# BaratiLab/GAMD

Hardware: AMD Instinct MI355X
Metric: atom-steps/sec (force eval + integrate), 10k-atom LJ box (higher is better)
Workload: dtype f32; 1 GPU; C2: 10 000-atom LJ box, rho*=0.5, L=92.29 A, cutoff 3.0 sigma=10.2 A, fp32, 4 conv layers x 128, random-init weights (seed 0), 1 box per GPU; n_atoms=10000, boxes=1, launch=single process

## Files before the change

gamd_amd/csrc/gamd_api.hip:

```cpp
#include "gamd_host.h"

#include <algorithm>
#include <cmath>
#include <cstddef>
#include <cstdlib>
#include <cstring>
#include <deque>

static_assert(sizeof(gamd_config) == 96 && offsetof(gamd_config, n_boxes) == 88 && offsetof(gamd_config, edge_capacity) == 40,
              "gamd_config layout is part of the C ABI (gamd_amd/_lib.py mirrors it)");

namespace {

bool small_path(const gamd_handle* h) { return h->use_small; }

int fill_com(gamd_handle* h, int enabled, MdCom* c) {
    c->enabled = enabled ? 1 : 0;
    c->blocks = std::max(1, std::min(16, (h->n_per_box + 1023) / 1024));
    c->partial = nullptr;
    if (!c->enabled) return 0;
    if (h->com_partial.ensure(sizeof(double) * 4 * (size_t)c->blocks * (size_t)h->n_boxes, true)) return fail(-12, "allocation failed");
    c->partial = h->com_partial.as<double>();
    return 0;
}
// ... 127 lines not shown
        a.cand_stride = (int)std::max<long long>(1, std::min<long long>(h->cand_cap / h->n, 1 << 20));
    }
    return a;
}

void pack128(const float* W, float* out, int ld = 128) {
    for (int tp = 0; tp < 4; ++tp)
        for (int t = 0; t < 4; ++t)
            for (int q = 0; q < 4; ++q)
                for (int lane = 0; lane < 64; ++lane)
                    for (int j = 0; j < 4; ++j) {
                        const int n = 32 * tp + (lane & 31), k = 32 * t + 8 * q + 4 * (lane >> 5) + j;
                        out[((((tp * 4 + t) * 4 + q) * 64 + lane) * 4) + j] = W[(size_t)n * ld + k];
                    }
}
void pack16(const float* W, float* out, int ld = 128) {
    for (int ob = 0; ob < 8; ++ob)
        for (int blk = 0; blk < 8; ++blk)
            for (int lane = 0; lane < 64; ++lane)
                for (int r = 0; r < 4; ++r)
                    out[(((ob * 8 + blk) * 64 + lane) * 4) + r] = W[(size_t)(16 * ob + (lane & 15)) * ld + 16 * blk + 4 * (lane >> 4) + r];
}
void split_f16(float w, uint16_t* hi, uint16_t* lo);
void pack16_f16x3(const float* W, uint16_t* out) {
    for (int ob = 0; ob < 8; ++ob)
        for (int m = 0; m < 4; ++m)
            for (int lane = 0; lane < 64; ++lane)
                for (int j = 0; j < 8; ++j) {
                    const int k = 32 * m + 16 * (j >> 2) + 4 * (lane >> 4) + (j & 3);
                    const size_t hi = ((((size_t)(ob * 4 + m) * 2 + 0) * 64 + lane) * 8) + j, lo = ((((size_t)(ob * 4 + m) * 2 + 1) * 64 + lane) * 8) + j;
                    split_f16(W[(size_t)(16 * ob + (lane & 15)) * 128 + k], out + hi, out + lo);
                }
}
void pack_enc1(const float* W, int n_feat, float* out) {
    for (int tp = 0; tp < 4; ++tp)
        for (int g = 0; g < 6; ++g)
            for (int lane = 0; lane < 64; ++lane)
                for (int j = 0; j < 4; ++j) {
                    const int n = 32 * tp + (lane & 31), k = 2 * (4 * g + j) + (lane >> 5);
                    out[(((tp * 6 + g) * 64 + lane) * 4) + j] = k < n_feat ? W[n * n_feat + k] : 0.f;
                }
}

int kfeat16x(int m, int g) { return 32 * (m >> 3) + 8 * ((m >> 1) & 3) + 4 * (g & 1) + (g >> 1) + 2 * (m & 1); }
void pack16x(const float* W, float* out, int ld, bool chained) {
    for (int ob = 0; ob < 8; ++ob)
        for (int m4 = 0; m4 < 8; ++m4)
            for (int lane = 0; lane < 64; ++lane) {
                const int i = lane & 15, g = lane >> 4;
                const int row = chained ? kfeat16x(4 * ob + (i & 3), i >> 2) : 64 * (ob >> 2) + 4 * i + (ob & 3);
                for (int c = 0; c < 4; ++c)
                    out[(((size_t)ob * 8 + m4) * 64 + lane) * 4 + c] = W[(size_t)row * ld + kfeat16x(4 * m4 + c, g)];
            }
}

uint16_t f2bf(float x) {
    uint32_t u; memcpy(&u, &x, 4);
    if ((u & 0x7f800000u) == 0x7f800000u) return (uint16_t)(u >> 16);
    u += 0x7fffu + ((u >> 16) & 1u);
    return (uint16_t)(u >> 16);
}
void pack128_bf16(const float* W, uint16_t* out, int ld = 128) {
    for (int tp = 0; tp < 4; ++tp)
        for (int t = 0; t < 4; ++t)
            for (int u = 0; u < 2; ++u)
                for (int lane = 0; lane < 64; ++lane)
                    for (int j = 0; j < 8; ++j) {
                        const int r = 8 * u + j, half = lane >> 5;
                        const int n = 32 * tp + (lane & 31), k = 32 * t + (r & 3) + 8 * (r >> 2) + 4 * half;
                        out[((((tp * 4 + t) * 2 + u) * 64 + lane) * 8) + j] = f2bf(W[(size_t)n * ld + k]);
                    }
}
void pack_enc1_bf16(const float* W, int n_feat, uint16_t* out) {
    for (int tp = 0; tp < 4; ++tp)
        for (int s = 0; s < 3; ++s)
            for (int lane = 0; lane < 64; ++lane)
                for (int j = 0; j < 8; ++j) {
                    const int n = 32 * tp + (lane & 31), k = 16 * s + 8 * (lane >> 5) + j;
                    out[(((tp * 3 + s) * 64 + lane) * 8) + j] = k < n_feat ? f2bf(W[n * n_feat + k]) : (uint16_t)0;
                }
}

void split_f16(float w, uint16_t* hi, uint16_t* lo) {
    const _Float16 h = (_Float16)w;
    const _Float16 l = (_Float16)(w - (float)h);
    memcpy(hi, &h, 2); memcpy(lo, &l, 2);
}
void pack128_f16x3(const float* W, uint16_t* out, int ld = 128) {
    for (int tp = 0; tp < 4; ++tp)
        for (int t = 0; t < 4; ++t)
            for (int u = 0; u < 2; ++u)
                for (int lane = 0; lane < 64; ++lane)
                    for (int j = 0; j < 8; ++j) {
                        const int r = 8 * u + j, half = lane >> 5;
                        const int n = 32 * tp + (lane & 31), k = 32 * t + (r & 3) + 8 * (r >> 2) + 4 * half;
                        const size_t at = ((((tp * 4 + t) * 2 + u) * 64 + lane) * 8) + j;
                        split_f16(W[(size_t)n * ld + k], out + at, out + 16384 + at);
                    }
}
void pack_enc1_f16x3(const float* W, int n_feat, uint16_t* out) {
    for (int tp = 0; tp < 4; ++tp)
        for (int s = 0; s < 3; ++s)
            for (int lane = 0; lane < 64; ++lane)
                for (int j = 0; j < 8; ++j) {
                    const int n = 32 * tp + (lane & 31), k = 16 * s + 8 * (lane >> 5) + j;
                    const size_t at = (((tp * 3 + s) * 64 + lane) * 8) + j;
                    split_f16(k < n_feat ? W[n * n_feat + k] : 0.f, out + at, out + 6144 + at);
                }
}

struct BlobBuilder {
    std::vector<float> host;
    size_t add(size_t n_floats) {
        const size_t off = host.size();
        host.resize(off + ((n_floats + 63) & ~(size_t)63), 0.f);
        return off;
    }
};

const HostTensor* find_w(gamd_handle* h, const std::string& name, std::initializer_list<int64_t> shape) {
    auto it = h->host_w.find(name);
    if (it == h->host_w.end()) { fail(-2, "missing weight '%s'", name.c_str()); return nullptr; }
    if (it->second.shape != std::vector<int64_t>(shape)) {
        std::string got;
        for (auto d : it->second.shape) got += std::to_string(d) + ",";
        std::string want;
        for (auto d : shape) want += std::to_string(d) + ",";
        fail(-22, "weight '%s' has shape (%s), expected (%s) for this configuration", name.c_str(), got.c_str(),
             want.c_str());
        return nullptr;
    }
    return &it->second;
}

struct EdgeList { const int* centre; const int* neigh; long long n; };

int fill_rigid(const gamd_handle* h, int rigid_water, float mass_o, float mass_h, float r_oh, float r_hh,
               int* use_rigid, RigidWater* g) {
    *use_rigid = 0;
    if (!rigid_water) return 0;
    if (h->n_per_box % 3 != 0) return fail(-22, "rigid_water needs O,H,H triples: n_atoms = %d is not a multiple of 3", h->n_per_box);
    if (!(mass_h > 0.f) || !(mass_o > 0.f)) return fail(-22, "rigid_water needs mass_amu (O) and mass_h_amu (H)");
    if (!(r_oh > 0.f) || !(r_hh > 0.f) || !(r_hh < 2.f * r_oh)) return fail(-22, "rigid_water needs 0 < r_hh < 2 r_oh");
    const double rc = 0.5 * (double)r_hh, t = std::sqrt((double)r_oh * r_oh - rc * rc);
    const double ra = t * 2.0 * mass_h / ((double)mass_o + 2.0 * mass_h);
    g->m_o = mass_o; g->m_h = mass_h;
    g->rc = (float)rc; g->ra = (float)ra; g->rb = (float)(t - ra);
    *use_rigid = 1;
    return 0;
}

int enqueue_forward(gamd_handle* h, const float* pos_dev, const uint8_t* species_dev, float* out_norm_dev,
                    float* out_denorm_dev, hipStream_t st, hipEvent_t* evs, int* n_ev, std::vector<std::string>* labels,
                    const EdgeList* el = nullptr, const MdFuse* fuse = nullptr, bool copy_counters = true, bool l0_reuse = false) {
    auto mark = [&](const char* label) {
        if (evs) { (void)hipEventRecord(evs[*n_ev], st); ++*n_ev; labels->push_back(label); }
    };
    int r;
    mark("begin");
    const bool pingpong = !el && h->skin > 0.f;
    int* counters_next = nullptr;
    if (pingpong) {
        h->cnt_parity ^= 1;
        h->cur_counters = h->cnt2.as<int>() + h->cnt_parity * CNT_COUNT;
        counters_next = h->cnt2.as<int>() + (1 - h->cnt_parity) * CNT_COUNT;
    } else {
        h->cur_counters = h->counters.as<int>();
    }
    NbrArgs na = nbr_args(h, pos_dev, species_dev);
    na.counters_next = counters_next;
    if (el) {
        if ((r = launch_csr_from_edges(na, el->centre, el->neigh, el->n, h->tmp_eid.as<int>(), st)))
            return fail(-1, "edge-list CSR launch failed (%d)", r);
        h->cand_valid = false;
    } else if (h->skin > 0.f) {
        na.ref_pos = h->ref_pos.as<float4>();
        na.force_rebuild = h->cand_valid ? 0 : 1;
        ++h->skin_calls;
        na.cells_one_wg = (h->skin_calls < 32 || 6ll * h->sticky_host[STICKY_REBUILDS] < h->skin_calls) ? 1 : 0;
        if (fuse && !pingpong) return fail(-1, "internal: integrator halves can only be fused into the skin path");
        if ((r = launch_neighbor_skin(na, st, fuse))) return fail(-1, "neighbor (skin) launch failed (%d)", r);
        h->cand_valid = true;
    } else if ((r = launch_neighbor_build(na, st))) return fail(-1, "neighbor build launch failed (%d)", r);
    mark("neighbor_build");

    EncArgs ea{};
    ea.counters = h->cur_counters;
    ea.devflags = h->devflags.as<int>();
    ea.pos_s = h->pos_s.as<float4>();
    ea.col = h->col.as<int>();
    ea.erow = h->erow.as<int>();
    ea.bond_nbr = h->has_bonds ? h->bond_nbr.as<int>() : nullptr;
    ea.perm = h->perm.as<int>();
    ea.row_ptr = h->row_ptr.as<int>();
    ea.self_loop = na.self_loop;
    ea.zero_row = h->n;
    for (int d = 0; d < 3; ++d) { ea.box[d] = h->box[d]; ea.half[d] = 0.5f * h->box[d]; }
    ea.bx = box_ref(h);
    ea.length_mean = h->length_mean;
    ea.length_std = h->length_std;
    ea.gamma = (float)(1.0 / 0.025);
    ea.ln_inv_width = 1.0f / (float)h->Eh_true;
    ea.ln_n_pad = (float)(h->Eh - h->Eh_true);
    ea.n_feat = h->n_feat;
    ea.n_ksteps = (h->n_feat + 1) / 2;
    ea.centers = h->centers;
    ea.rbf = h->rbf;
    ea.w1p = h->enc_w1p; ea.w2p = h->enc_w2p; ea.w3p = h->enc_w3p;
    ea.b1 = h->enc_b1; ea.b2 = h->enc_b2; ea.b3 = h->enc_b3;
    ea.ln_g = h->enc_lng; ea.ln_b = h->enc_lnb;
    ea.e_format = !h->wide_enc ? 0 : h->cfg.edge_dtype == GAMD_EDGE_F16X3 ? 2 : h->cfg.edge_dtype == GAMD_EDGE_BF16 ? 1 : 0;
    ea.e_frag = h->e_frag.as<float>();
    ea.e_cap = h->e_cap;
    ea.sticky = h->sticky_dev;
    ea.feat_dbg = h->cfg.keep_stages ? h->feat_dbg.as<float>() : nullptr;
    int small_tiles = 0;
    if (h->cfg.edge_dtype == GAMD_EDGE_F32) {
        const long long e_est = el ? el->n + (na.self_loop ? h->n : 0)
                                   : (h->counters_host[CNT_E] > 0 ? (long long)h->counters_host[CNT_E] : (long long)((double)h->e_cap / 1.5));
        const long long tiles = (e_est + GAMD_TILE - 1) / GAMD_TILE;
        if (tiles <= h->small_tile_limit) small_tiles = (int)std::max<long long>(1, std::min<long long>(tiles + tiles / 8 + 1, 4096));
    }
    const bool half_quantum = h->wide_conv && h->cfg.edge_dtype == GAMD_EDGE_F32 && (h->cfg.kernel_select & GAMD_KSEL_FORCE_HALF_QUANTUM) != 0;
    bool tev_full = false;
    auto tev_begin = [&](int kind) -> int {
        if (!h->timing) return 0;
        if (h->tev_used + 2 > h->tev.size()) {
            if (h->tev.size() >= 8 * gamd_handle::EVENT_POOL_CAP) { tev_full = true; return 0; }
            for (int k = 0; k < 256; ++k) { hipEvent_t e; HIP_TRY(hipEventCreate(&e)); h->tev.push_back(e); h->tev_kind.push_back(0); }
        }
        h->tev_kind[h->tev_used] = kind;
        HIP_TRY(hipEventRecord(h->tev[h->tev_used], st));
        return 0;
    };
    auto tev_end = [&]() -> int {
        if (!h->timing || tev_full) return 0;
        HIP_TRY(hipEventRecord(h->tev[h->tev_used + 1], st));
        h->tev_used += 2;
        return 0;
    };
    if ((r = tev_begin(100))) return r;
    r = h->DT > 1 ? launch_edge_encode_wide_d(ea, h->EHT, h->DT, h->n_cu, st)
        : h->wide_enc ? launch_edge_encode_wide(ea, h->EHT, h->n_cu, st)
        : h->cfg.edge_dtype == GAMD_EDGE_BF16 ? launch_edge_encode_bf16(ea, h->n_cu, st)
        : h->cfg.edge_dtype == GAMD_EDGE_F16X3 ? launch_edge_encode_f16x3(ea, h->n_cu, st)
        : small_tiles > 0 ? launch_edge_encode_small(ea, small_tiles, st) : launch_edge_encode(ea, h->n_cu, st);
    if (r) return fail(-1, "edge encode launch failed (%d)", r);
    if ((r = tev_end())) return r;
    mark("edge_encode");

    const size_t nh = (size_t)h->n * (size_t)h->H;
    auto node = [&](const NodeArgs& na_) {
        return h->DT > 1 ? launch_node_wide_d(na_, h->HT, h->DT, st) : h->wide_conv ? launch_node_wide(na_, h->HT, st) : launch_node(na_, st);
    };
    auto hptr = [&](int l) { return h->hbuf.as<float>() + (h->cfg.keep_stages ? (size_t)l * nh : (size_t)(l & 1) * nh); };

    NodeArgs no{};
#ifdef GAMD_PROFILING
    { static const bool node_time = getenv("GAMD_NODE_TIME") != nullptr; if (node_time) no.tdbg = h->tdbg.as<long long>(); }
#endif
    no.counters = h->cur_counters;
    no.devflags = h->devflags.as<int>();
    no.sticky = h->sticky_dev;
    no.n = h->n;
    no.pos_s = h->pos_s.as<float4>();
    no.node_emb = h->node_emb; no.enc_w = h->nenc_w; no.enc_b = h->nenc_b;
    no.row_ptr = h->row_ptr.as<int>(); no.na_excl = h->na_excl.as<int>(); no.deg = h->deg.as<int>();
    no.col = (h->l0_hoist && h->n_boxes > 1) ? h->col.as<int>() : nullptr;
    no.partial = h->partial.as<float>();
    no.piece_cap = h->piece_cap;
    no.P_in = h->P.as<float>();
    no.hn_perm = (!h->wide_conv && h->cfg.edge_dtype == GAMD_EDGE_F16X3) ? 1 : 0;
    no.tab16 = (!h->wide_conv && h->cfg.edge_dtype == GAMD_EDGE_BF16) ? 1 : 0;
    no.hn_out = h->hn.as<float>(); no.S_out = h->S.as<float>(); no.D_out = h->D.as<float>(); no.P_out = h->P.as<float>();
    no.dec_w1p = h->dec_w1p; no.dec_b1 = h->dec_b1; no.dec_w2 = h->dec_w2; no.dec_b2 = h->dec_b2;
    no.ln_inv_width = 1.0f / (float)h->H_true;
    no.ln_n_pad = (float)(h->H - h->H_true);
    no.norm_bn = h->norm_bn;
    no.f16x3 = h->node_f16 ? 1 : 0;
    no.scale = (float)std::sqrt(h->scaler_var);
    no.shift = (float)h->scaler_mean;
    no.perm = h->perm.as<int>();
    no.forces_norm = out_norm_dev ? out_norm_dev : h->f_norm.as<float>();
    no.forces = out_denorm_dev;

    const bool l0 = h->skin > 0.f && !el;
    float* const h0 = (l0 && !h->cfg.keep_stages) ? h->l0_h.as<float>() : hptr(0);
    no.mode = 0;
    no.pre = h->layers[0].node;
    no.h_out = h0;
    if (l0) { no.hn_out = h->l0_hn.as<float>(); no.S_out = h->l0_S.as<float>(); no.D_out = h->l0_D.as<float>(); no.P_out = h->l0_P.as<float>(); }
    no.l0_gate = (l0 && l0_reuse) ? 1 : 0;
    if ((r = node(no))) return fail(-1, "node(0) launch failed (%d)", r);
    no.l0_gate = 0;
    no.hn_out = h->hn.as<float>(); no.S_out = h->S.as<float>(); no.D_out = h->D.as<float>(); no.P_out = h->P.as<float>();
    mark("node_first");


    for (int l = 0; l < h->L; ++l) {
        ConvEdgeArgs ca{};
        ca.counters = h->cur_counters;
        ca.devflags = h->devflags.as<int>();
        ca.col = h->col.as<int>(); ca.erow = h->erow.as<int>();
        ca.chunk_piece = h->chunk_piece.as<int>(); ca.chunk_mask = h->chunk_mask.as<unsigned>();
        ca.e_frag = (h->update_edge && l > 0) ? h->e_frag2.as<float>() : h->e_frag.as<float>();
        ca.emb_out = (h->update_edge && l + 1 < h->L) ? h->e_emb.as<float>() : nullptr;
        ca.hn = h->hn.as<float>(); ca.S = h->S.as<float>(); ca.D = h->D.as<float>();
        if (l0 && l == 0) { ca.hn = h->l0_hn.as<float>(); ca.S = h->l0_S.as<float>(); ca.D = h->l0_D.as<float>(); }
        const LayerDev& ld = h->layers[l];
        ca.w1p = ld.w1p; ca.w2p = ld.w2p; ca.w3p = ld.w3p; ca.w4p = ld.w4p; ca.w16p = ld.w16p;
        ca.b1 = ld.b1; ca.b3 = ld.b3; ca.b4 = ld.b4;
        const bool hoist = l == 0 && h->l0_hoist;
        if (hoist) { ca.w3p = ld.w3p_l0; ca.b3 = ld.b3_l0; }
        ca.partial = h->partial.as<float>();
        ca.piece_cap = h->piece_cap;
        ca.sticky = h->sticky_dev;
        ca.e_cap = h->e_cap;
        ca.zero_row = h->n;
#ifdef GAMD_CHECKED
        { static const bool inject = getenv("GAMD_CHK_INJECT") != nullptr; if (inject) ca.zero_row = 0; }
#endif
        ca.tdbg = h->tdbg.as<long long>();
        if ((r = tev_begin(l))) return r;
        r = h->DT > 1 ? launch_conv_edge_wide_d(ca, h->EHT, h->HT, h->DT, h->n_cu, st)
            : h->wide_conv ? (h->cfg.edge_dtype == GAMD_EDGE_F16X3 ? launch_conv_edge_f16x3_wide(ca, h->EHT, h->HT, h->n_cu, st)
                            : h->cfg.edge_dtype == GAMD_EDGE_BF16 ? launch_conv_edge_bf16_wide(ca, h->EHT, h->HT, h->n_cu, st)
                            : (half_quantum && ca.w16p && !ca.emb_out) ? launch_conv_edge_wide16(ca, h->EHT, h->HT, h->n_cu, st)
                            : small_tiles > 0 ? launch_conv_edge_small_wide(ca, h->EHT, h->HT, small_tiles, st)
                                              : launch_conv_edge_wide(ca, h->EHT, h->HT, h->n_cu, st))
            : h->cfg.edge_dtype == GAMD_EDGE_BF16 ? launch_conv_edge_bf16(ca, h->n_cu, st)
            : h->cfg.edge_dtype == GAMD_EDGE_F16X3 ? launch_conv_edge_f16x3(ca, h->n_cu, st)
            : hoist ? (small_tiles > 0 ? launch_conv_edge_small_l0(ca, small_tiles, st) : launch_conv_edge_l0(ca, h->n_cu, st))
            : small_tiles > 0 ? launch_conv_edge_small(ca, small_tiles, st) : launch_conv_edge(ca, h->n_cu, st);
        if (r) return fail(-1, "conv edge launch failed (%d)", r);
        if ((r = tev_end())) return r;
        mark("conv_edge");
        if (ca.emb_out) {
            EdgeUpdateArgs ua{};
            ua.counters = h->cur_counters; ua.devflags = h->devflags.as<int>(); ua.e_cap = h->e_cap;
            ua.emb = ca.emb_out; ua.ln_g = ld.e_ln_g; ua.ln_b = ld.e_ln_b;
            ua.ln_inv_width = 1.0f / (float)h->Eh_true;
            ua.ln_n_pad = (float)(h->Eh - h->Eh_true);
            ua.e_frag_out = h->e_frag2.as<float>();
            if ((r = launch_edge_update(ua, h->HT, small_tiles > 0 ? std::max(1, small_tiles / 4) : 2 * h->n_cu, st)))
                return fail(-1, "edge update launch failed (%d)", r);
            mark("edge_update");
        }

        no.mode = (l == h->L - 1) ? 2 : 1;
        no.post = ld.node;
        if (l + 1 < h->L) no.pre = h->layers[l + 1].node;
        no.h_in = l == 0 ? h0 : hptr(l);
        no.P_in = (l0 && l == 0) ? h->l0_P.as<float>() : h->P.as<float>();
        no.h_out = hptr(l + 1);
        if ((r = node(no))) return fail(-1, "node launch failed (%d)", r);
        mark(no.mode == 2 ? "node_last_decode" : "node_mid");
    }
    if (copy_counters)
        HIP_TRY(hipMemcpyAsync(h->counters_host, h->cur_counters, sizeof(int) * CNT_COUNT, hipMemcpyDeviceToHost, st));
    return 0;
}

int check_ready(gamd_handle* h) {
    if (!h) return fail(-22, "null handle");
    if (!h->finalized) return fail(-22, "weights not finalized (call gamd_finalize_weights)");
    return 0;
}

int check_model_inputs(gamd_handle* h, const uint8_t* species_dev) {
    if (h->cfg.kind == GAMD_KIND_WATER && !species_dev && !h->feat_dev)
        return fail(-22, "water model needs species (or gamd_set_node_features)");
    if (h->cfg.use_bond && !h->has_bonds) return fail(-22, "use_bond set but no bonds given (gamd_set_bonds)");
    return 0;
}

int check_rigid_layout(gamd_handle* h, const uint8_t* species_dev, hipStream_t st) {
    if (!species_dev) return fail(-22, "rigid_water needs species (O = 1, H = 0, atoms ordered O,H,H)");
    if (h->rigid_checked == species_dev) return 0;
    std::vector<uint8_t> sp((size_t)h->n);
    HIP_TRY(hipMemcpyAsync(sp.data(), species_dev, sp.size(), hipMemcpyDeviceToHost, st));
    HIP_TRY(hipStreamSynchronize(st));
    for (int i = 0; i < h->n; ++i)
        if ((sp[(size_t)i] != 0) != (i % 3 == 0))
            return fail(-22, "rigid_water needs atoms ordered O,H,H per molecule: species[%d] = %d", i, (int)sp[(size_t)i]);
    h->rigid_checked = species_dev;
    return 0;
}

int clear_devflags(gamd_handle* h) {
    const int init[2] = {0, -1};
    HIP_TRY(init_upload(h->devflags.p, init, sizeof(init)));
    return 0;
}

int step_event(gamd_handle* h, hipStream_t st, bool closes = false) {
    if (!h->timing) return 0;
    if (h->sev_used == h->sev.size()) {
        if (h->sev.size() >= gamd_handle::EVENT_POOL_CAP) return 0;
        for (int k = 0; k < 256; ++k) { hipEvent_t e; HIP_TRY(hipEventCreate(&e)); h->sev.push_back(e); h->sev_closes.push_back(0); }
    }
    h->sev_closes[h->sev_used] = closes ? 1 : 0;
    HIP_TRY(hipEventRecord(h->sev[h->sev_used++], st));
    return 0;
}

int enqueue_md_steps(gamd_handle* h, long long s_begin, bool skip_first) {
    MdPending& p = h->pending;
    int r;
    if (p.kind == 0 && h->skin > 0.f) {
        for (long long s = s_begin; s < p.n_steps; ++s) {
            if ((r = step_event(h, p.st))) return r;
            p.m.step = p.first_step + (unsigned long long)s;
            p.m.step_index = (int)s;
            int do_second = (s > s_begin && !observers_sampled(h, s - 1)) ? 1 : 0;
            const int do_first = (skip_first && s == s_begin) ? 0 : 1;
            if (p.m.com.enabled) {
                if (do_second && do_first) {
                    MdArgs prev = p.m;
                    prev.step_index = (int)(s - 1);
                    if ((r = launch_baoab_second_com(prev, p.st))) return fail(-1, "integrator launch failed (%d)", r);
                    do_second = 0;
                } else {
                    if (do_second) {
                        MdArgs prev = p.m;
                        prev.step_index = (int)(s - 1);
                        if ((r = launch_baoab_second(prev, p.st))) return fail(-1, "integrator launch failed (%d)", r);
                        do_second = 0;
                    }
                    if (do_first && (r = launch_com_partial(p.m.com, p.m.v, p.m.species, p.m.inv_mass, p.m.inv_mass_h, p.m.n, p.m.bx,
                                                            p.m.devflags, p.m.use_rigid, p.st)))
                        return fail(-1, "integrator launch failed (%d)", r);
                }
            }
            const MdFuse fuse{&p.m, do_second, do_first};
            if ((r = enqueue_forward(h, p.x, p.species, nullptr, p.f, p.st, nullptr, nullptr, nullptr, nullptr, &fuse,
                                     s + 1 == p.n_steps, s > s_begin)))
                return r;
            if (s + 1 < p.n_steps && observers_sampled(h, s)) {
                if ((r = launch_baoab_second(p.m, p.st))) return fail(-1, "integrator launch failed (%d)", r);
                if ((r = observers_enqueue(h, s))) return r;
            }
        }
        if (p.n_steps > s_begin) {
            p.m.step_index = (int)(p.n_steps - 1);
            if ((r = launch_baoab_second(p.m, p.st))) return fail(-1, "integrator launch failed (%d)", r);
            if ((r = observers_enqueue(h, p.n_steps - 1))) return r;
        }
        return step_event(h, p.st, true);
    }
    for (long long s = s_begin; s < p.n_steps; ++s) {
        if ((r = step_event(h, p.st))) return r;
        const bool first = !(skip_first && s == s_begin);
        const bool last = s + 1 == p.n_steps;
        if (p.kind == 0) {
            p.m.step = p.first_step + (unsigned long long)s;
            p.m.step_index = (int)s;
            if (first && (r = launch_baoab_first(p.m, p.st))) return fail(-1, "integrator launch failed (%d)", r);
            if ((r = enqueue_forward(h, p.x, p.species, nullptr, p.f, p.st, nullptr, nullptr, nullptr, nullptr, nullptr, last, s > s_begin))) return r;
            if ((r = launch_baoab_second(p.m, p.st))) return fail(-1, "integrator launch failed (%d)", r);
        } else {
            p.a.step_index = (int)s;
            if (first && (r = launch_nhc_first(p.a, p.st))) return fail(-1, "integrator launch failed (%d)", r);
            if ((r = enqueue_forward(h, p.x, p.species, nullptr, p.f, p.st, nullptr, nullptr, nullptr, nullptr, nullptr, last, s > s_begin))) return r;
            if ((r = launch_nhc_second(p.a, p.st))) return fail(-1, "integrator launch failed (%d)", r);
        }
        if ((r = observers_enqueue(h, s))) return r;
    }
    return step_event(h, p.st, true);
}

template <typename Params, typename Args>
int fill_run_args(gamd_handle* h, const Params* p, const float* box, const uint8_t* species_dev, hipStream_t st, Args* a) {
    int r;
    a->n = h->n; a->species = species_dev; a->dt = p->dt_ps;
    a->len = p->length_per_nm > 0.f ? p->length_per_nm : 10.0f;
    if ((r = fill_rigid(h, p->rigid_water, p->mass_amu, p->mass_h_amu, p->r_oh, p->r_hh, &a->use_rigid, &a->rigid))) return r;
    if (a->use_rigid && (r = check_rigid_layout(h, species_dev, st))) return r;
    for (int d = 0; d < 3; ++d) a->box[d] = box[d];
    a->bx = box_ref(h);
    if ((r = fill_com(h, p->remove_cm_motion, &a->com))) return r;
    a->devflags = h->devflags.as<int>();
    return 0;
}

int start_run(gamd_handle* h, float* x_dev, float* f_dev, const uint8_t* species_dev, const float* box, long long n_steps, hipStream_t st) {
    MdPending& pd = h->pending;
    pd.active = true; pd.n_steps = n_steps;
    pd.x = x_dev; pd.f = f_dev; pd.species = species_dev; pd.st = st;
    observers_begin_run(h, box, species_dev, n_steps);
    return enqueue_md_steps(h, 0, false);
}

}

extern "C" {

#ifdef GAMD_CHECKED
const char* gamd_version(void) { return "gamd_hip 0.1 (gfx950) checked"; }
#else
const char* gamd_version(void) { return "gamd_hip 0.1 (gfx950)"; }
#endif
const char* gamd_last_error(void) { return g_err; }

int32_t gamd_create(const gamd_config* cfg, gamd_handle** out) {
    if (!cfg || !out) return fail(-22, "null argument");
    if (cfg->n_atoms <= 0) return fail(-22, "n_atoms must be positive");
    if (cfg->n_boxes < 0 || cfg->n_boxes > (1 << 20)) return fail(-22, "n_boxes out of range");
    const int n_boxes = cfg->n_boxes > 1 ? cfg->n_boxes : 1;
    if ((long long)cfg->n_atoms * n_boxes >= (1 << 23) - 1)
        return fail(-22, "n_atoms x n_boxes = %lld: at most %d atoms per handle", (long long)cfg->n_atoms * n_boxes, (1 << 23) - 2);
    if (cfg->n_layers <= 0 || cfg->n_layers > 16) return fail(-22, "n_layers out of range");
    if (!(cfg->cutoff > 0.f)) return fail(-22, "cutoff must be positive");
    if (cfg->edge_dtype != GAMD_EDGE_F32 && cfg->edge_dtype != GAMD_EDGE_BF16 && cfg->edge_dtype != GAMD_EDGE_F16X3)
        return fail(-22, "unknown edge_dtype");
    if (!(cfg->neighbor_skin >= 0.f)) return fail(-22, "neighbor_skin must be >= 0");
    if (cfg->self_loop_mode != GAMD_SELF_LOOP_DGL07_NOOP && cfg->self_loop_mode != GAMD_SELF_LOOP_APPEND_ZERO_FEATURE)
        return fail(-22, "unknown self_loop_mode %d", cfg->self_loop_mode);
    if (cfg->self_loop_mode != GAMD_SELF_LOOP_DGL07_NOOP && cfg->edge_dtype != GAMD_EDGE_F32)
        return fail(-22, "self_loop_mode 1 is built for the fp32 edge dtype only");
    if (cfg->kernel_select & ~(GAMD_KSEL_FORCE_GENERIC_WIDTH | GAMD_KSEL_FORCE_HALF_QUANTUM | GAMD_KSEL_NO_LAYER0_HOIST))
        return fail(-22, "unknown kernel_select bits 0x%x", cfg->kernel_select);
    int ndev = 0;
    if (hipGetDeviceCount(&ndev) != hipSuccess || ndev <= 0)
        return fail(-19, "no HIP device available: libgamd_hip has no CPU fallback");
    if (cfg->device < 0 || cfg->device >= ndev) return fail(-22, "device %d out of range (%d visible)", cfg->device, ndev);
    DeviceGuard guard(cfg->device);
    hipDeviceProp_t prop;
    HIP_TRY(hipGetDeviceProperties(&prop, cfg->device));
    const int H_true = cfg->encoding_size ? cfg->encoding_size : 128, Eh_true = cfg->edge_embedding_dim ? cfg->edge_embedding_dim : 128;
    const int D_true = cfg->hidden_dim ? cfg->hidden_dim : 128;
    if (H_true < 1 || H_true > 256 || Eh_true < 1 || Eh_true > 256)
        return fail(-22, "encoding_size and edge_embedding_dim must be in [1, 256] (got %d, %d)", H_true, Eh_true);
    if (D_true < 1 || D_true > 256) return fail(-22, "hidden_dim must be in [1, 256] (got %d)", D_true);
    const int Dp = D_true <= 128 ? 128 : 256;
    if (Dp > 128 && cfg->edge_dtype != GAMD_EDGE_F32)
        return fail(-22, "hidden_dim above 128 is built for edge_dtype f32 only (got hidden_dim %d)", D_true);
    const int H = H_true <= 128 ? 128 : 256, Eh = Eh_true <= 128 ? 128 : 256;
    const bool exact128 = H_true == 128 && Eh_true == 128 && D_true == 128;
    const bool generic = H != 128 || Eh != 128 || cfg->no_expand_edge;
    if (cfg->edge_dtype != GAMD_EDGE_F32 && H == 256 && (long long)cfg->n_atoms * n_boxes > (1ll << 22) - 2)
        return fail(-22, "bf16 / split-fp16 with encoding_size > 128: at most 2^22 - 2 atoms per handle (32-bit byte offsets into hn)");
    gamd_handle* h = new gamd_handle();
    h->obs = observers_new();
    h->cfg = *cfg;
    h->dev = cfg->device;
    if (hipStreamCreateWithFlags(&h->init_stream, hipStreamNonBlocking) != hipSuccess) {
        h->init_stream = nullptr;
        gamd_destroy(h);
        return fail(-12, "stream creation failed");
    }
    InitStream init(h->init_stream);
    h->n_boxes = n_boxes;
    h->n_per_box = cfg->n_atoms;
    h->n = cfg->n_atoms * n_boxes;
    h->L = cfg->n_layers;
    h->H = H; h->Eh = Eh; h->HT = H / 128; h->EHT = Eh / 128;
    h->H_true = H_true; h->Eh_true = Eh_true; h->D_true = D_true;
    h->Dp = Dp; h->DT = Dp / 128;
    h->skin = cfg->neighbor_skin;
    if (cfg->small_tile_limit != 0) h->small_tile_limit = cfg->small_tile_limit < 0 ? -1 : cfg->small_tile_limit;
    const bool forced = (cfg->kernel_select & GAMD_KSEL_FORCE_GENERIC_WIDTH) && cfg->edge_dtype == GAMD_EDGE_F32;
    const bool lp_generic = cfg->edge_dtype != GAMD_EDGE_F32 && (generic || !exact128);
    h->wide_enc = generic || forced || lp_generic || Dp > 128;
    h->wide_conv = H != 128 || Eh != 128 || forced || lp_generic || Dp > 128;
    h->n_feat = (cfg->no_expand_edge ? 4 : 44) + (cfg->use_bond ? 1 : 0);
    h->n_cu = prop.multiProcessorCount > 0 ? prop.multiProcessorCount : 256;
    const size_t n = (size_t)h->n;
    int r = 0;
    r |= h->pos_w.ensure(sizeof(float4) * n, true);
    r |= h->pos_s.ensure(sizeof(float4) * (n + 1), true);
    r |= h->cell_of.ensure(sizeof(int) * n, true);
    r |= h->perm.ensure(sizeof(int) * (n + 1), true);
    if (n_boxes > 1) {
        r |= h->boxes_dev.ensure(sizeof(float) * 12 * (size_t)n_boxes, true);
        r |= h->box_shift.ensure(sizeof(int) * ((size_t)n_boxes + 2), true);
    }
    r |= h->inv_perm.ensure(sizeof(int) * n, true);
    r |= h->deg.ensure(sizeof(int) * n, true);
    r |= h->row_ptr.ensure(sizeof(int) * (n + 1), true);
    r |= h->na_excl.ensure(sizeof(int) * (n + 1), true);
    const size_t nh = n * (size_t)H * sizeof(float), nd = n * (size_t)Dp * sizeof(float), zd = (size_t)Dp * sizeof(float);
    r |= h->hbuf.ensure(nh * (cfg->keep_stages ? (size_t)h->L + 1 : 2), true);
    r |= h->hn.ensure(nh + (size_t)H * sizeof(float), true);
    r |= h->S.ensure(nd + zd, true);
    r |= h->D.ensure(nd + zd, true);
    r |= h->P.ensure(nd, true);
    if (cfg->neighbor_skin > 0.f) {
        r |= h->l0_hn.ensure(nh + (size_t)H * sizeof(float), true);
        r |= h->l0_S.ensure(nd + zd, true);
        r |= h->l0_D.ensure(nd + zd, true);
        r |= h->l0_P.ensure(nd, true);
        if (!cfg->keep_stages) r |= h->l0_h.ensure(nh, true);
    }
    r |= h->f_norm.ensure(sizeof(float) * 3 * n, true);
    r |= h->f_den.ensure(sizeof(float) * 3 * n, true);
    r |= h->tdbg.ensure(sizeof(long long) * 16 * 8 * 1024, true);
    r |= h->devflags.ensure(sizeof(int) * DEVFLAG_COUNT, true);
    r |= h->cnt2.ensure(sizeof(int) * 2 * CNT_COUNT, true);
    if (r) { gamd_destroy(h); return fail(-12, "device allocation failed"); }
    {
        const int no_atom = -2;
        if (init_upload(h->perm.as<int>() + n, &no_atom, sizeof(int)) != hipSuccess) {
            gamd_destroy(h);
            return fail(-1, "device copy failed");
        }
    }
    if ((r = clear_devflags(h))) { gamd_destroy(h); return r; }
    if (hipHostMalloc((void**)&h->counters_host, sizeof(int) * CNT_COUNT) != hipSuccess) {
        gamd_destroy(h);
        return fail(-12, "pinned allocation failed");
    }
    memset(h->counters_host, 0, sizeof(int) * CNT_COUNT);
    if (hipHostMalloc((void**)&h->sticky_host, sizeof(int) * STICKY_COUNT, hipHostMallocMapped) != hipSuccess ||
        hipHostGetDevicePointer((void**)&h->sticky_dev, h->sticky_host, 0) != hipSuccess) {
        gamd_destroy(h);
        return fail(-12, "mapped host allocation failed");
    }
    memset(h->sticky_host, 0, sizeof(int) * STICKY_COUNT);
    if (h->skin > 0.f) {
        int rr = 0;
        rr |= h->ref_pos.ensure(sizeof(float4) * n, true);
        rr |= h->cand_deg.ensure(sizeof(int) * n, true);
        rr |= h->cand_ptr.ensure(sizeof(int) * (n + 1), true);
        if (rr) { gamd_destroy(h); return fail(-12, "device allocation failed"); }
    }
    {
        std::vector<float> all((size_t)n_boxes * 3);
        for (int b = 0; b < n_boxes; ++b)
            for (int d = 0; d < 3; ++d) all[(size_t)3 * b + d] = cfg->box[d];
        if ((r = set_box(h, all.data()))) { gamd_destroy(h); return r; }
    }
    {
        const double per_atom = std::min<double>(h->n, 27.0 * h->n / std::max(1, h->ncell));
        h->use_small = h->n <= 1024 && n_boxes <= 1 && (double)h->n * per_atom <= 3.0e5 && h->ncell <= 4096;
    }
    long long ecap = cfg->edge_capacity;
    if (ecap <= 0) {
        const double vol = (double)cfg->box[0] * cfg->box[1] * cfg->box[2];
        const double per_atom = 4.18879 * std::pow((double)cfg->cutoff, 3) * (double)h->n_per_box / vol + 1.0;
        ecap = (long long)(1.5 * per_atom * (double)h->n) + 1024 + 16ll * n_boxes;
    }
    if (cfg->self_loop_mode) ecap += h->n;
    if ((r = alloc_edges(h, ecap))) { gamd_destroy(h); return r; }
    if (hipStreamSynchronize(h->init_stream) != hipSuccess) { gamd_destroy(h); return fail(-1, "device synchronisation failed"); }
    *out = h;
    return 0;
}

int32_t gamd_destroy(gamd_handle* h) {
    if (!h) return 0;
    DeviceGuard guard(h->dev);
    InitStream init(h->init_stream);
    h->devflags.release();
    h->cnt2.release();
    DevBuf* bufs[] = {&h->boxes_dev, &h->box_shift, &h->wblob, &h->pos_w, &h->pos_s, &h->cell_of, &h->perm, &h->inv_perm, &h->deg, &h->row_ptr,
                      &h->na_excl, &h->bond_nbr, &h->hbuf, &h->hn, &h->S, &h->D, &h->P, &h->l0_h, &h->l0_hn, &h->l0_S, &h->l0_D, &h->l0_P, &h->f_norm, &h->f_den,
                      &h->cell_cnt, &h->cell_fill, &h->cell_start, &h->col, &h->erow, &h->chunk_piece,
                      &h->chunk_mask, &h->e_frag, &h->e_emb, &h->e_frag2, &h->partial, &h->feat_dbg, &h->counters, &h->tdbg, &h->tmp_eid, &h->ke_partial, &h->com_partial,
                      &h->ref_pos, &h->cand_deg, &h->cand_ptr, &h->cand_col};
    for (DevBuf* b : bufs) b->release();
    observers_free(h);
    h->pos_in.release();
    if (h->host_in) (void)hipHostFree(h->host_in);
    if (h->host_out) (void)hipHostFree(h->host_out);
    if (h->counters_host) (void)hipHostFree(h->counters_host);
    if (h->sticky_host) (void)hipHostFree(h->sticky_host);
    for (hipEvent_t e : h->tev) (void)hipEventDestroy(e);
    for (hipEvent_t e : h->sev) (void)hipEventDestroy(e);
    if (h->init_stream) (void)hipStreamDestroy(h->init_stream);
    delete h;
    return 0;
}

int32_t gamd_load_weight(gamd_handle* h, const char* name, const float* data, const int64_t* shape, int32_t ndim) {
    if (!h || !name || !data || !shape || ndim < 1 || ndim > 2) return fail(-22, "bad argument to gamd_load_weight");
    HostTensor t;
    size_t cnt = 1;
    for (int i = 0; i < ndim; ++i) { t.shape.push_back(shape[i]); cnt *= (size_t)shape[i]; }
    t.data.assign(data, data + cnt);
    h->host_w[name] = std::move(t);
    h->finalized = false;
    return 0;
}

int32_t gamd_finalize_weights(gamd_handle* h) {
    if (!h) return fail(-22, "null handle");
    DeviceGuard guard(h->dev);
    InitStream init(h->init_stream);
    const int F = h->n_feat, L = h->L;
    const int64_t H = h->H, Eh = h->Eh, HT = h->HT, EHT = h->EHT;
    const int64_t Ht = h->H_true, Et = h->Eh_true, Dt = h->D_true;
    const int64_t Dp = h->Dp, DT = h->DT;
    const bool expand = !h->cfg.no_expand_edge;
    BlobBuilder bb;
    struct Off { size_t w1p, w2p, w3p, w4p, w16p = 0, b1, b3, b4, elng = 0, elnb = 0, lng, lnb, wsp, wdp, wpdp, bS, bP, wpep, wphip, bphi;
                 size_t w3p_l0 = 0, b3_l0 = 0, m0 = 0, c0 = 0; };
    std::vector<Off> lo(L);
    std::deque<HostTensor> padded;
    auto get = [&](const std::string& nm, std::initializer_list<int64_t> shp, std::initializer_list<int64_t> pad) -> const HostTensor* {
        const HostTensor* t = find_w(h, nm, shp);
        if (!t) return nullptr;
        const std::vector<int64_t> ps(pad);
        if (t->shape == ps) return t;
        HostTensor o;
        o.shape = ps;
        const int64_t r = ps.size() == 2 ? t->shape[0] : 1, c = ps.size() == 2 ? t->shape[1] : t->shape[0];
        const int64_t cp = ps.size() == 2 ? ps[1] : ps[0], rp = ps.size() == 2 ? ps[0] : 1;
        o.data.assign((size_t)(rp * cp), 0.f);
        for (int64_t i = 0; i < r; ++i) std::copy(t->data.begin() + i * c, t->data.begin() + (i + 1) * c, o.data.begin() + i * cp);
        padded.push_back(std::move(o));
        return &padded.back();
    };
    auto put_vec = [&](const HostTensor* t) { size_t o = bb.add(t->data.size()); std::copy(t->data.begin(), t->data.end(), bb.host.begin() + o); return o; };
    auto put_blocks = [&](const HostTensor* t, int OB, int KB) {
        size_t o = bb.add((size_t)OB * KB * GAMD_WFRAG_FLOATS);
        for (int ob = 0; ob < OB; ++ob)
            for (int kb = 0; kb < KB; ++kb)
                pack128(t->data.data() + (size_t)128 * ob * 128 * KB + 128 * kb,
                        bb.host.data() + o + (size_t)(ob * KB + kb) * GAMD_WFRAG_FLOATS, 128 * KB);
        return o;
    };
    auto put_blocks_f16x3_fn = [&](const HostTensor* t, int OB, int KB) {
        size_t o = bb.add((size_t)OB * KB * GAMD_WFRAG_FLOATS);
        for (int ob = 0; ob < OB; ++ob)
            for (int kb = 0; kb < KB; ++kb)
                pack128_f16x3(t->data.data() + (size_t)128 * ob * 128 * KB + 128 * kb,
                              reinterpret_cast<uint16_t*>(bb.host.data() + o + (size_t)(ob * KB + kb) * GAMD_WFRAG_FLOATS), 128 * KB);
        return o;
    };
    h->node_f16 = h->cfg.edge_dtype != GAMD_EDGE_F32;
    auto put_node = [&](const HostTensor* t, int OB, int KB) {
        if (h->wide_conv) return h->node_f16 ? put_blocks_f16x3_fn(t, OB, KB) : put_blocks(t, OB, KB);
        size_t o = bb.add(GAMD_WFRAG_FLOATS);
        if (h->node_f16) pack16_f16x3(t->data.data(), reinterpret_cast<uint16_t*>(bb.host.data() + o));
        else pack16(t->data.data(), bb.host.data() + o);
        return o;
    };
    const bool bf16_edges = h->cfg.edge_dtype == GAMD_EDGE_BF16 && !h->wide_conv;
    const bool bf16_wide = h->cfg.edge_dtype == GAMD_EDGE_BF16 && h->wide_conv;
    const bool f16x3_edges = h->cfg.edge_dtype == GAMD_EDGE_F16X3 && !h->wide_conv;
    const bool f16x3_wide = h->cfg.edge_dtype == GAMD_EDGE_F16X3 && h->wide_conv;
    auto put_edge_f16x3 = [&](const HostTensor* t) {
        size_t o = bb.add(GAMD_WFRAG_FLOATS);
        pack128_f16x3(t->data.data(), reinterpret_cast<uint16_t*>(bb.host.data() + o));
        return o;
    };
    auto put_blocks_f16x3 = put_blocks_f16x3_fn;
    auto put_edge_bf16 = [&](const HostTensor* t) {
        size_t o = bb.add(GAMD_WFRAG_FLOATS / 2);
        pack128_bf16(t->data.data(), reinterpret_cast<uint16_t*>(bb.host.data() + o));
        return o;
    };

    const bool update_edge = h->host_w.count("graph_conv.conv.0.edge_layer_norm.weight") != 0;
    if (update_edge) {
        if (Ht != Et)
            return fail(-22, "update_edge_emb needs encoding_size == edge_embedding_dim (got %d, %d)", (int)Ht, (int)Et);
        if (h->cfg.edge_dtype != GAMD_EDGE_F32 || h->cfg.self_loop_mode)
            return fail(-22, "update_edge_emb is built for the fp32 edge MLP without appended self loops");
        h->wide_enc = h->wide_conv = true;
    }
    if (update_edge != h->update_edge) {
        h->update_edge = update_edge;
        if (alloc_edges(h, h->e_cap)) return -12;
    }
    const bool norm_bn = h->host_w.count("graph_conv.norm_layers.0.running_mean") != 0;
    h->norm_bn = norm_bn ? 1 : 0;
    h->l0_hoist = h->cfg.kind == GAMD_KIND_LJ && h->cfg.edge_dtype == GAMD_EDGE_F32 && !h->wide_conv && DT == 1 && !update_edge &&
                  !(h->cfg.kernel_select & GAMD_KSEL_NO_LAYER0_HOIST);
    const HostTensor* emb0 = h->l0_hoist ? get("node_emb", {1, Ht}, {1, H}) : nullptr;
    if (h->l0_hoist && !emb0) return -2;
    auto permute_f2 = [](const HostTensor& w, const HostTensor& b, HostTensor& wo, HostTensor& bo) {
        wo = w;
        bo = b;
        for (int q = 0; q < 4; ++q)
            for (int s = 0; s < 32; ++s) {
                std::copy(w.data.begin() + (size_t)(4 * s + q) * 128, w.data.begin() + (size_t)(4 * s + q + 1) * 128,
                          wo.data.begin() + (size_t)(32 * q + s) * 128);
                bo.data[32 * q + s] = b.data[4 * s + q];
            }
    };
    for (int l = 0; l < L; ++l) {
        const std::string p = "graph_conv.conv." + std::to_string(l);
        const HostTensor *ea0w = get(p + ".edge_affine.mlp_layer.0.weight", {128, Et}, {128, Eh}), *ea0b = get(p + ".edge_affine.mlp_layer.0.bias", {128}, {128});
        const HostTensor *ea2w = get(p + ".edge_affine.mlp_layer.2.weight", {Dt, 128}, {Dp, 128}), *ea2b = get(p + ".edge_affine.mlp_layer.2.bias", {Dt}, {Dp});
        const HostTensor *sw = get(p + ".src_affine.weight", {Dt, Ht}, {Dp, H}), *sb = get(p + ".src_affine.bias", {Dt}, {Dp});
        const HostTensor *dw = get(p + ".dst_affine.weight", {Dt, Ht}, {Dp, H}), *db = get(p + ".dst_affine.bias", {Dt}, {Dp});
        const HostTensor *t1w = get(p + ".theta_edge.mlp_layer.1.weight", {Dt, Dt}, {Dp, Dp}), *t1b = get(p + ".theta_edge.mlp_layer.1.bias", {Dt}, {Dp});
        const HostTensor *t3w = get(p + ".theta_edge.mlp_layer.3.weight", {Ht, Dt}, {H, Dp}), *t3b = get(p + ".theta_edge.mlp_layer.3.bias", {Ht}, {H});
        const HostTensor *pdw = get(p + ".phi_dst.weight", {Dt, Ht}, {Dp, H}), *pdb = get(p + ".phi_dst.bias", {Dt}, {Dp});
        const HostTensor *pew = get(p + ".phi_edge.weight", {Dt, Ht}, {Dp, H}), *peb = get(p + ".phi_edge.bias", {Dt}, {Dp});
        const HostTensor *phw = get(p + ".phi.mlp_layer.1.weight", {Ht, Dt}, {H, Dp}), *phb = get(p + ".phi.mlp_layer.1.bias", {Ht}, {H});
        const HostTensor *ng = get("graph_conv.norm_layers." + std::to_string(l) + ".weight", {Ht}, {H});
        const HostTensor *nb = get("graph_conv.norm_layers." + std::to_string(l) + ".bias", {Ht}, {H});
        if (!ea0w || !ea0b || !ea2w || !ea2b || !sw || !sb || !dw || !db || !t1w || !t1b || !t3w || !t3b || !pdw ||
            !pdb || !pew || !peb || !phw || !phb || !ng || !nb)
            return -2;
        if (norm_bn) {
            const std::string np_ = "graph_conv.norm_layers." + std::to_string(l);
            const HostTensor *rm = get(np_ + ".running_mean", {Ht}, {H}), *rv = get(np_ + ".running_var", {Ht}, {H});
            if (!rm || !rv) return -2;
            HostTensor al, be;
            al.shape = be.shape = {H};
            al.data.assign((size_t)H, 0.f);
            be.data.assign((size_t)H, 0.f);
            for (int64_t i = 0; i < Ht; ++i) {
                const float invstd = 1.0f / std::sqrt(rv->data[i] + 1e-5f);
                al.data[i] = ng->data[i] * invstd;
                be.data[i] = nb->data[i] - rm->data[i] * al.data[i];
            }
            padded.push_back(std::move(al)); ng = &padded.back();
            padded.push_back(std::move(be)); nb = &padded.back();
        }
        if (bf16_edges) {
            auto scaled = [&](const HostTensor* t, double f) -> const HostTensor* {
                HostTensor o = *t;
                for (float& v : o.data) v = (float)((double)v * f);
                padded.push_back(std::move(o));
                return &padded.back();
            };
            const double LOG2E = 1.4426950408889634, LN2 = 0.6931471805599453;
            ea0w = scaled(ea0w, LOG2E); ea0b = scaled(ea0b, LOG2E); t1b = scaled(t1b, LOG2E); t3w = scaled(t3w, LN2);
            sw = scaled(sw, LOG2E); dw = scaled(dw, LOG2E);
            sb = scaled(sb, LOG2E); db = scaled(db, LOG2E); ea2b = scaled(ea2b, LOG2E);
        }
        Off& o = lo[l];
        if (l == 0 && h->l0_hoist) {
            std::vector<double> hn0((size_t)H, 0.0);
            if (norm_bn) {
                for (int64_t i = 0; i < H; ++i) hn0[i] = (double)emb0->data[i] * ng->data[i] + nb->data[i];
            } else {
                double mean = 0.0, var = 0.0;
                for (int64_t i = 0; i < Ht; ++i) mean += emb0->data[i];
                mean /= (double)Ht;
                for (int64_t i = 0; i < Ht; ++i) var += ((double)emb0->data[i] - mean) * ((double)emb0->data[i] - mean);
                var /= (double)Ht;
                const double rstd = 1.0 / std::sqrt(var + 1e-5);
                for (int64_t i = 0; i < Ht; ++i) hn0[i] = ((double)emb0->data[i] - mean) * rstd * ng->data[i] + nb->data[i];
            }
            HostTensor m0, c0;
            m0.shape = {Dp, Dp};
            m0.data.assign((size_t)(Dp * Dp), 0.f);
// ... 620 lines not shown
```

gamd_amd/csrc/gamd_host.h:

```cpp
#pragma once
#include "../../include/gamd_hip.h"
#include "gamd_common.h"
#include "gamd_internal.h"

#include <cstdarg>
#include <cstdio>
#include <map>
#include <string>
#include <vector>

#pragma GCC visibility push(hidden)

inline thread_local char g_err[512] = "";

inline int fail(int code, const char* fmt, ...) {
    va_list ap;
    va_start(ap, fmt);
    vsnprintf(g_err, sizeof(g_err), fmt, ap);
    va_end(ap);
    return code;
}

#define HIP_TRY(expr)                                                                              \
    do {                                                                                           \
        hipError_t e__ = (expr);                                                                   \
        if (e__ != hipSuccess) return fail(-1000 - (int)e__, "%s: %s", #expr, hipGetErrorString(e__)); \
    } while (0)

struct HostTensor {
    std::vector<int64_t> shape;
    std::vector<float> data;
};

inline thread_local hipStream_t tl_init_stream = nullptr;
struct InitStream {
    hipStream_t prev;
    explicit InitStream(hipStream_t st) : prev(tl_init_stream) { tl_init_stream = st; }
    ~InitStream() { tl_init_stream = prev; }
    InitStream(const InitStream&) = delete;
    InitStream& operator=(const InitStream&) = delete;
};
inline hipError_t init_upload(void* dst, const void* src, size_t bytes) {
    hipError_t e = hipMemcpyAsync(dst, src, bytes, hipMemcpyHostToDevice, tl_init_stream);
    return e != hipSuccess ? e : hipStreamSynchronize(tl_init_stream);
}

struct DevBuf {
    void* p = nullptr;
    size_t bytes = 0;
    int ensure(size_t want, bool zero) {
        if (want <= bytes && p) return 0;
        if (p) { hipError_t e = hipFree(p); if (e != hipSuccess) return (int)e; p = nullptr; bytes = 0; }
        hipError_t e = hipMalloc(&p, want);
        if (e != hipSuccess) return (int)e;
        bytes = want;
        if (zero) {
            e = hipMemsetAsync(p, 0, want, tl_init_stream);
            if (e == hipSuccess) e = hipStreamSynchronize(tl_init_stream);
            if (e != hipSuccess) return (int)e;
        }
        return 0;
    }
    void release() { if (p) (void)hipFree(p); p = nullptr; bytes = 0; }
    template <typename T> T* as() const { return reinterpret_cast<T*>(p); }
};

struct LayerDev {
    const float *w1p, *w2p, *w3p, *w4p, *b1, *b3, *b4;
    const float *w16p = nullptr;
    const float *e_ln_g = nullptr, *e_ln_b = nullptr;
    const float *w3p_l0 = nullptr, *b3_l0 = nullptr;
    NodeLayerW node;
};

struct DeviceGuard {
    int prev = -1;
    bool changed = false;
    explicit DeviceGuard(int dev) {
        if (hipGetDevice(&prev) == hipSuccess && prev != dev) changed = hipSetDevice(dev) == hipSuccess;
    }
    ~DeviceGuard() { if (changed) (void)hipSetDevice(prev); }
    DeviceGuard(const DeviceGuard&) = delete;
    DeviceGuard& operator=(const DeviceGuard&) = delete;
};

struct MdPending {
    bool active = false;
    int kind = 0;
    MdArgs m{};
    NhcArgs a{};
    unsigned long long first_step = 0;
    float mass = 0.f, mass_h = 0.f;
    long long n_steps = 0;
    float* x = nullptr;
    float* f = nullptr;
    const uint8_t* species = nullptr;
    hipStream_t st = nullptr;
};

struct Observers;
Observers* observers_new();
void observers_free(gamd_handle* h);
int observers_check_run(gamd_handle* h, const float* box, const uint8_t* species_dev);
void observers_begin_run(gamd_handle* h, const float* box, const uint8_t* species_dev, long long n_steps);
bool observers_sampled(const gamd_handle* h, long long s);
int observers_enqueue(gamd_handle* h, long long s);

struct gamd_handle {
    gamd_config cfg{};
    int dev = 0;
    int n = 0, L = 0, n_feat = 44, n_cu = 256;
    int n_boxes = 1, n_per_box = 0;
    bool use_small = false;
    DevBuf boxes_dev, box_shift;
    std::vector<float> boxes_host;
    int H = 128, Eh = 128, HT = 1, EHT = 1;
    int H_true = 128, Eh_true = 128, D_true = 128;
    int Dp = 128, DT = 1;
    int norm_bn = 0;
    bool update_edge = false;
    bool node_f16 = false;
    bool wide_enc = false, wide_conv = false;
    bool l0_hoist = false;
    long long small_tile_limit = 512;
    std::map<std::string, HostTensor> host_w;
    bool finalized = false;
    double scaler_mean = 0.0, scaler_var = 1.0;

    DevBuf wblob;
    std::vector<LayerDev> layers;
    const float *enc_w1p = nullptr, *enc_w2p = nullptr, *enc_w3p = nullptr, *enc_b1 = nullptr, *enc_b2 = nullptr,
                *enc_b3 = nullptr, *enc_lng = nullptr, *enc_lnb = nullptr, *centers = nullptr;
    const float *node_emb = nullptr, *nenc_w = nullptr, *nenc_b = nullptr;
    const float *dec_w1p = nullptr, *dec_b1 = nullptr, *dec_w2 = nullptr, *dec_b2 = nullptr;
    float length_mean = 0.f, length_std = 1.f;
    RbfGrid rbf{};

    DevBuf pos_w, pos_s, cell_of, perm, inv_perm, deg, row_ptr, na_excl, bond_nbr;
    DevBuf hbuf, hn, S, D, P, f_norm, f_den;
    DevBuf l0_h, l0_hn, l0_S, l0_D, l0_P;
    DevBuf cell_cnt, cell_fill, cell_start;
    int ncell_cap = 0;
    long long e_cap = 0;
    long long piece_cap = 0;
    DevBuf col, erow, chunk_piece, chunk_mask, e_frag, partial, feat_dbg, e_emb, e_frag2;
    DevBuf counters, tdbg, tmp_eid, ke_partial, com_partial;
    DevBuf cnt2;
    int cnt_parity = 0;
    long long skin_calls = 0;
    int* cur_counters = nullptr;
    int* counters_host = nullptr;
    float* host_in = nullptr;
    float* host_out = nullptr;
    DevBuf pos_in;
    int* sticky_host = nullptr;
    int* sticky_dev = nullptr;
    hipStream_t init_stream = nullptr;
    DevBuf devflags;
    const float* feat_dev = nullptr;
    const uint8_t* rigid_checked = nullptr;
    MdPending pending;
    Observers* obs = nullptr;
    bool has_bonds = false;

    float skin = 0.f;
    DevBuf ref_pos, cand_deg, cand_ptr, cand_col;
    long long cand_cap = 0;
    bool cand_valid = false;

    float box[3] = {0, 0, 0};
    int nc[3] = {1, 1, 1};
    int ncell = 1;

    bool timing = false;
    std::vector<hipEvent_t> tev;
    std::vector<int> tev_kind;
    size_t tev_used = 0;
    std::vector<hipEvent_t> sev;
    std::vector<uint8_t> sev_closes;
    size_t sev_used = 0;
    static constexpr size_t EVENT_POOL_CAP = 1u << 16;
};

inline BoxRef box_ref(const gamd_handle* h) {
    BoxRef r{};
    r.n_boxes = h->n_boxes;
    r.n_per_box = h->n_per_box;
    r.inv_npb = 1.0f / (float)h->n_per_box;
    r.boxes = h->n_boxes > 1 ? h->boxes_dev.as<float4>() : nullptr;
    return r;
}

inline int check_traps(gamd_handle* h) {
    const int code = h->sticky_host[STICKY_CHECK_CODE];
    if (!code) return 0;
    const int value = h->sticky_host[STICKY_CHECK_VALUE], line = h->sticky_host[STICKY_CHECK_LINE];
    h->sticky_host[STICKY_CHECK_CODE] = 0;
    return fail(-35, "checked build: device-side range check %d failed (value %d, source line %d)", code, value, line);
}

#pragma GCC visibility pop
```

gamd_amd/csrc/gamd_internal.h:

```cpp
#pragma once
#include <hip/hip_runtime.h>
#include <stdint.h>
#include <atomic>
#include "gamd_common.h"

enum { CNT_E = 0, CNT_PIECES = 1, CNT_OVERFLOW = 2, CNT_TILES = 3, CNT_REBUILD = 4, CNT_NCAND = 5,
       CNT_CAND_MAX = 6,
       CNT_COUNT = 8 };
enum { STICKY_EDGE_OVERFLOW = 0, STICKY_CAND_OVERFLOW = 1, STICKY_REBUILDS = 2, STICKY_NCAND = 3,
       STICKY_NONFINITE = 4,
       STICKY_CHECK_CODE = 5, STICKY_CHECK_VALUE = 6, STICKY_CHECK_LINE = 7,
       STICKY_COUNT = 8 };
enum { GAMD_CHK_CELL = 101, GAMD_CHK_CAND = 102, GAMD_CHK_EDGE_POS = 103, GAMD_CHK_PERM = 104, GAMD_CHK_ENC_SRC = 111, GAMD_CHK_ENC_DST = 112,
       GAMD_CHK_CONV_SRC = 121, GAMD_CHK_CONV_DST = 122, GAMD_CHK_PIECE = 123, GAMD_CHK_NODE_PIECES = 131, GAMD_CHK_INJECTED = 199 };
#ifdef GAMD_CHECKED
template <typename T>
__device__ __forceinline__ T gamd_chk_range(int* sticky, T v, long long lo, long long hi, int code, int line) {
    if ((long long)v >= lo && (long long)v <= hi) return v;
    if (sticky && sticky[STICKY_CHECK_CODE] == 0) {
        sticky[STICKY_CHECK_VALUE] = (int)v;
        sticky[STICKY_CHECK_LINE] = line;
        __threadfence_system();
        sticky[STICKY_CHECK_CODE] = code;
    }
    return (T)lo;
}
#define GAMD_CHK_RANGE(sticky, v, lo, hi, code) gamd_chk_range((sticky), (v), (long long)(lo), (long long)(hi), (code), __LINE__)
#else
#define GAMD_CHK_RANGE(sticky, v, lo, hi, code) (v)
#endif
enum { DEVFLAG_FROZEN = 0, DEVFLAG_FROZEN_AT = 1, DEVFLAG_REBUILDS = 2, DEVFLAG_COUNT = 4 };

constexpr int GAMD_MAX_DEVICES = 64;
struct PerDeviceOnce { std::atomic<bool> done[GAMD_MAX_DEVICES] = {}; };
template <typename... Fn>
inline int gamd_allow_dynamic_lds(PerDeviceOnce& once, int bytes, Fn... fns) {
    int dev = 0;
    hipError_t e = hipGetDevice(&dev);
    if (e != hipSuccess) return (int)e;
    if (dev >= 0 && dev < GAMD_MAX_DEVICES && once.done[dev].load(std::memory_order_relaxed)) return 0;
    const void* list[] = {(const void*)fns...};
    for (const void* fn : list) {
        e = hipFuncSetAttribute(fn, hipFuncAttributeMaxDynamicSharedMemorySize, bytes);
        if (e != hipSuccess) return (int)e;
    }
    if (dev >= 0 && dev < GAMD_MAX_DEVICES) once.done[dev].store(true, std::memory_order_relaxed);
    return 0;
}

struct BoxRef {
    int n_boxes, n_per_box;
    float inv_npb;
    const float4* boxes;
};
__device__ __forceinline__ int gamd_box_of(const BoxRef& r, int i) {
    int q = (int)(((float)i + 0.5f) * r.inv_npb);
    const int rem = i - q * r.n_per_box;
    q += rem >= r.n_per_box ? 1 : (rem < 0 ? -1 : 0);
    return q;
}
struct BoxDims { float bx, by, bz, hx, hy, hz; };
__device__ __forceinline__ BoxDims gamd_box_dims(const BoxRef& r, const float (&box)[3], const float (&half)[3], int box_id) {
    if (r.n_boxes <= 1) return BoxDims{box[0], box[1], box[2], half[0], half[1], half[2]};
    const float4 b = r.boxes[3 * box_id], h = r.boxes[3 * box_id + 1];
    return BoxDims{b.x, b.y, b.z, h.x, h.y, h.z};
}

constexpr int GAMD_HIST_MAX_BINS = 1024;
constexpr int GAMD_HIST_MAX_PAIRS = 3;
__device__ __forceinline__ void gamd_hist_add(unsigned* bins, float4 p, float4 q, const BoxDims& B, float r_max, float bin_scale,
                                              int n_bins, int n_pairs, int accept_all, unsigned inc) {
    float r;
    {
#pragma clang fp contract(off)
        const float rx = gamd_min_image_wrapped(p.x - q.x, B.bx, B.hx);
        const float ry = gamd_min_image_wrapped(p.y - q.y, B.by, B.hy);
        const float rz = gamd_min_image_wrapped(p.z - q.z, B.bz, B.hz);
        r = sqrtf((rx * rx + ry * ry) + rz * rz);
    }
    if (!(accept_all || r < r_max)) return;
    int bin = (int)(r * bin_scale / r_max);
    bin = bin < n_bins - 1 ? bin : n_bins - 1;
    bin = bin < 0 ? 0 : bin;
    int pair = 0;
    if (n_pairs == 3) {
        const bool po = p.w != 0.f, qo = q.w != 0.f;
        pair = (po && qo) ? 0 : ((po || qo) ? 1 : 2);
    }
    atomicAdd(&bins[pair * n_bins + bin], inc);
}
__device__ __forceinline__ void gamd_hist_zero(unsigned* bins, int n_slots) { for (int k = threadIdx.x; k < n_slots; k += blockDim.x) bins[k] = 0u; }
__device__ __forceinline__ void gamd_hist_flush(const unsigned* bins, unsigned long long* out, int n_slots) {
    for (int k = threadIdx.x; k < n_slots; k += blockDim.x) {
        const unsigned c = bins[k];
        if (c) atomicAdd(&out[k], (unsigned long long)c);
    }
}

struct NbrArgs {
    int n;
    BoxRef bx;
    int* box_shift;
    int flavour;
    float box[3], half[3];
    float rc, rc2;
    int nc[3], ncell;
    int ncell_cap;
    long long e_cap;
    const float* pos;
    const uint8_t* species;
    const float* feat;
    int self_loop;
    int* devflags;
    float4* pos_w;
    float4* pos_s;
    int* cell_of;
    int* cell_cnt;
    int* cell_fill;
    int* cell_start;
    int* perm;
    int* inv_perm;
    int* deg;
    int* row_ptr;
    int* na_excl;
    int* col;
    int* erow;
    int* chunk_piece;
    unsigned* chunk_mask;
    int* counters;
    int* counters_next;
    int* sticky;
    const int* gate;
    float skin_half2;
    int force_rebuild;
    float4* ref_pos;
    int* cand_deg;
    int* cand_ptr;
    int* cand_col;
    long long cand_cap;
    int cand_stride;
    int use_small;
    int cells_one_wg;
    float rc_build, rc2_build;
};
struct MdArgs;
struct MdFuse { const MdArgs* md; int do_second, do_first; };
int launch_neighbor_build(const NbrArgs& a, hipStream_t st);
int launch_neighbor_skin(const NbrArgs& a, hipStream_t st, const MdFuse* fuse = nullptr);
int launch_csr_from_edges(const NbrArgs& a, const int* centre, const int* neigh, long long n_edges, int* tmp_eid,
                          hipStream_t st);

struct EncArgs {
    const int* counters;
    const int* devflags;
    const float4* pos_s;
    const int* col;
    const int* erow;
    const int* bond_nbr;
    const int* perm;
    const int* row_ptr;
    int self_loop;
    int zero_row;
    float box[3], half[3];
    BoxRef bx;
    float length_mean, length_std, gamma;
    float ln_inv_width, ln_n_pad;
    int n_feat;
    int n_ksteps;
    const float* centers;
    RbfGrid rbf;
    const float* w1p;
    const float* w2p;
    const float* w3p;
    const float* b1; const float* b2; const float* b3;
    const float* ln_g; const float* ln_b;
    float* e_frag;
    long long e_cap;
    float* feat_dbg;
    int* sticky;
    int e_format;
};
__device__ __forceinline__ bool gamd_is_appended_loop(const EncArgs& a, long long x, int src, int dst) {
    if (!a.self_loop || src == a.zero_row) return false;
    const long long row_end = a.row_ptr[dst + 1];
    return x == row_end - 1 || (x + 1 < row_end && a.col[x + 1] == a.zero_row);
}

__device__ __forceinline__ BoxDims gamd_edge_box(const EncArgs& a, int dst) {
    return gamd_box_dims(a.bx, a.box, a.half, a.bx.n_boxes > 1 ? gamd_box_of(a.bx, dst) : 0);
}
int launch_edge_encode(const EncArgs& a, int n_blocks, hipStream_t st);
int launch_edge_encode_small(const EncArgs& a, int n_blocks, hipStream_t st);
int launch_edge_encode_bf16(const EncArgs& a, int n_blocks, hipStream_t st);
int launch_edge_encode_f16x3(const EncArgs& a, int n_blocks, hipStream_t st);
int launch_edge_encode_wide(const EncArgs& a, int eht, int n_blocks, hipStream_t st);
int launch_edge_encode_wide_d(const EncArgs& a, int eht, int dt, int n_blocks, hipStream_t st);

struct ConvEdgeArgs {
    const int* counters;
    const int* devflags;
    const int* col;
    const int* erow;
    const int* chunk_piece;
    const unsigned* chunk_mask;
    const float* e_frag;
    const float* hn;
    const float* S;
    const float* D;
    const float* w1p; const float* w2p; const float* w3p; const float* w4p;
    const float* w16p;
    const float* b1; const float* b3; const float* b4;
    float* partial;
    long long e_cap;
    int zero_row;
    long long* tdbg;
    int* sticky;
    long long piece_cap;
    float* emb_out;
};
int launch_conv_edge(const ConvEdgeArgs& a, int n_blocks, hipStream_t st);
int launch_conv_edge_l0(const ConvEdgeArgs& a, int n_blocks, hipStream_t st);
int launch_conv_edge_bf16(const ConvEdgeArgs& a, int n_blocks, hipStream_t st);
int launch_conv_edge_small(const ConvEdgeArgs& a, int n_blocks, hipStream_t st);
int launch_conv_edge_small_l0(const ConvEdgeArgs& a, int n_blocks, hipStream_t st);
int launch_conv_edge_small_wide(const ConvEdgeArgs& a, int eht, int ht, int n_blocks, hipStream_t st);
int launch_conv_edge_f16x3(const ConvEdgeArgs& a, int n_blocks, hipStream_t st);
int launch_conv_edge_wide(const ConvEdgeArgs& a, int eht, int ht, int n_blocks, hipStream_t st);
int launch_conv_edge_wide16(const ConvEdgeArgs& a, int eht, int ht, int n_blocks, hipStream_t st);
int launch_conv_edge_wide_d(const ConvEdgeArgs& a, int eht, int ht, int dt, int n_blocks, hipStream_t st);
int launch_conv_edge_f16x3_wide(const ConvEdgeArgs& a, int eht, int ht, int n_blocks, hipStream_t st);
int launch_conv_edge_bf16_wide(const ConvEdgeArgs& a, int eht, int ht, int n_blocks, hipStream_t st);

struct EdgeUpdateArgs {
    const int* counters;
    const int* devflags;
    long long e_cap;
    const float* emb;
    const float* ln_g; const float* ln_b;
    float ln_inv_width, ln_n_pad;
    float* e_frag_out;
};
int launch_edge_update(const EdgeUpdateArgs& a, int ht, int n_blocks, hipStream_t st);

struct NodeLayerW {
    const float* ln_g; const float* ln_b;
    const float* wsp; const float* wdp; const float* wpdp;
    const float* bS;
    const float* bP;
    const float* wpep;
    const float* c0;
    const float* wphip;
    const float* bphi;
};
struct NodeArgs {
    const int* counters;
    const int* devflags;
    int* sticky;
    int n;
    int mode;
    int l0_gate;
    const float4* pos_s;
    const float* node_emb;
    const float* enc_w; const float* enc_b;
    const int* row_ptr; const int* na_excl; const int* deg;
    const int* col;
    const float* partial;
    long long piece_cap;
    const float* h_in;
    const float* P_in;
    NodeLayerW post;
    NodeLayerW pre;
    const float* dec_w1p; const float* dec_b1; const float* dec_w2; const float* dec_b2;
    float scale, shift;
    float ln_inv_width, ln_n_pad;
    int norm_bn;
    int f16x3;
    const int* perm;
    float* h_out;
    float* hn_out; float* S_out; float* D_out; float* P_out;
    int hn_perm;
    int tab16;
    float* forces_norm;
    float* forces;
    long long* tdbg;
};
int launch_node(const NodeArgs& a, hipStream_t st);
int launch_node_wide(const NodeArgs& a, int ht, hipStream_t st);
int launch_node_wide_d(const NodeArgs& a, int ht, int dt, hipStream_t st);

struct RigidWater { float m_o, m_h, ra, rb, rc; };
struct MdCom {
    int enabled;
    int blocks;
    double* partial;
};
struct MdArgs {
    int n;
    float* x; float* v;
    const float* f;
    const uint8_t* species;
    float inv_mass, inv_mass_h;
    float len;
    float dt;
    float a, b_len_kT;
    float box[3];
    BoxRef bx;
    int use_rigid;
    RigidWater rigid;
    unsigned long long seed; unsigned long long step;
    int* devflags;
    int step_index;
    MdCom com;
};
int launch_baoab_first(const MdArgs& a, hipStream_t st);
int launch_baoab_second(const MdArgs& a, hipStream_t st);
int launch_baoab_second_com(const MdArgs& a, hipStream_t st);

struct NhcArgs {
    int n;
    float* x; float* v;
    const float* f;
    const uint8_t* species;
    float mass, mass_h;
    float len;
    float dt;
    float box[3];
    BoxRef bx;
    int use_rigid;
    RigidWater rigid;
    double kT, freq, ndf;
    int M, n_c, n_ys;
    double w[5];
    double* state;
    double* partial;
    int n_blocks;
    int* devflags;
    int step_index;
    MdCom com;
};
int launch_com_partial(const MdCom& com, const float* v, const uint8_t* species, float inv_mass, float inv_mass_h, int n,
                       const BoxRef& bx, const int* devflags, int by_molecule, hipStream_t st);
int launch_nhc_first(const NhcArgs& a, hipStream_t st);
int launch_nhc_second(const NhcArgs& a, hipStream_t st);

enum { GAMD_CHK_REPORT_SRC = 141, GAMD_CHK_REPORT_DST = 142, GAMD_CHK_REPORT_PERM = 143, GAMD_CHK_REPORT_ROW = 144 };
struct ReportArgs {
    int n;
    BoxRef bx;
    const int* devflags;
    int* sticky;
    const float* v;
    const uint8_t* species;
    double mass, mass_h;
    double len;
    double* partial;
    int blocks;
    long long* steps;
    double* ke;
    long long slot;
    long long g;
    const int* counters;
    const float4* pos_s;
    const int* col; const int* erow; const int* row_ptr; const int* perm;
    long long e_cap;
    float box[3], half[3];
    int n_bins, n_pairs;
    float r_max, bin_scale;
    int all_edges;
    int exclude_same_molecule;
    unsigned long long* counts;
    int rdf_blocks;
};
int launch_report_ke(const ReportArgs& a, hipStream_t st);
int launch_report_rdf(const ReportArgs& a, hipStream_t st);

struct TrajArgs {
    int n;
    BoxRef bx;
    float box[3];
    const int* devflags;
    const float* x; const float* v; const float* f;
    const uint8_t* species;
    double mass, mass_h;
    long long q;
    long long g;
    long long frame;
    long long* steps;
    float* fx; float* fv; float* ff; int* fimg;
    float* x_prev;
    int* image;
    unsigned long long* ambiguous;
    int n_lags;
    int slot;
    int active;
    int classes;
    int subtract_com;
    float* ring_x; int* ring_img; float* ring_v;
    double* ring_com;
    double* com_partial;
    int com_blocks;
    double* corr_partial;
    int corr_blocks;
    double* msd; double* vacf;
    long long* class_atoms;
};
int launch_traj_sample(const TrajArgs& a, hipStream_t st);

enum { GAMD_CHK_STRUCT_PERM_I = 145, GAMD_CHK_STRUCT_PERM_J = 146 };
struct StructArgs {
    int n;
    BoxRef bx;
    const int* devflags;
    int* sticky;
    float box[3], half[3];
    const float4* pos_s;
    const int* perm;
    int n_bins, n_pairs;
    float r_max, bin_scale;
    int exclude_same_molecule;
    int tiles;
    unsigned long long* counts;
    const float* x;
    const uint8_t* species;
    int n_k;
    const int* kvec;
    int classes;
    int rho_blocks;
    double* rho_partial;
    double* sk_sum;
};
int launch_struct_pairs(const StructArgs& a, hipStream_t st);
int launch_struct_sk(const StructArgs& a, hipStream_t st);
```

gamd_amd/csrc/gamd_md_dev.h:

```cpp
#pragma once
#include "gamd_common.h"
#include "gamd_internal.h"

#pragma clang fp contract(off)

__device__ __forceinline__ void philox_round(uint32_t (&c)[4], uint32_t k0, uint32_t k1) {
    const uint32_t M0 = 0xD2511F53u, M1 = 0xCD9E8D57u;
    const uint32_t hi0 = __umulhi(M0, c[0]), lo0 = M0 * c[0];
    const uint32_t hi1 = __umulhi(M1, c[2]), lo1 = M1 * c[2];
    const uint32_t n0 = hi1 ^ c[1] ^ k0, n2 = hi0 ^ c[3] ^ k1;
    c[0] = n0; c[1] = lo1; c[2] = n2; c[3] = lo0;
}

__device__ __forceinline__ void philox4x32_10(uint32_t (&c)[4], uint32_t k0, uint32_t k1) {
#pragma unroll
    for (int i = 0; i < 10; ++i) {
        philox_round(c, k0, k1);
        k0 += 0x9E3779B9u; k1 += 0xBB67AE85u;
    }
}

__device__ __forceinline__ float u01(uint32_t x) { return ((float)(x >> 8) + 0.5f) * (1.0f / 16777216.0f); }

__device__ __forceinline__ void atom_noise(unsigned long long seed, unsigned long long step, int i, float (&xi)[3]) {
// ... 28 lines not shown
    out[0] = (float)(px * inv); out[1] = (float)(py * inv); out[2] = (float)(pz * inv);
}

__device__ __forceinline__ void d_baoab_first_atom(const MdArgs& a, int i) {
    float xi[3], box[3], com[3] = {0.f, 0.f, 0.f};
    const BoxAtom ba = md_box_atom(a.bx, i);
    md_box(a.bx, a.box, ba.box, box);
    if (a.com.enabled) md_com_velocity(a.com, ba.box, com);
    atom_noise(a.seed + (unsigned long long)ba.box, a.step, ba.local, xi);
    const float w = atom_inv_mass(a.species, a.inv_mass, a.inv_mass_h, i);
    const float hdt = 0.5f * a.dt, kick = hdt * a.len * w, bs = a.b_len_kT * sqrtf(w);
#pragma unroll
    for (int d = 0; d < 3; ++d) {
        float v = a.v[3 * i + d] - com[d], x = a.x[3 * i + d];
        v += kick * a.f[3 * i + d];
        x += hdt * v;
        v = a.a * v + bs * xi[d];
        x += hdt * v;
        a.v[3 * i + d] = v;
        a.x[3 * i + d] = gamd_remainder(x, box[d]);
    }
}

__device__ __forceinline__ void d_baoab_second_dof(const MdArgs& a, int i) {
    a.v[i] += 0.5f * a.dt * a.len * atom_inv_mass(a.species, a.inv_mass, a.inv_mass_h, i / 3) * a.f[i];
}

namespace gamd_md {

struct Vec3 { float x, y, z; };
__device__ __forceinline__ Vec3 operator+(Vec3 a, Vec3 b) { return {a.x + b.x, a.y + b.y, a.z + b.z}; }
__device__ __forceinline__ Vec3 operator-(Vec3 a, Vec3 b) { return {a.x - b.x, a.y - b.y, a.z - b.z}; }
__device__ __forceinline__ Vec3 operator*(float s, Vec3 a) { return {s * a.x, s * a.y, s * a.z}; }
__device__ __forceinline__ float dot(Vec3 a, Vec3 b) { return (a.x * b.x + a.y * b.y) + a.z * b.z; }
__device__ __forceinline__ Vec3 cross(Vec3 a, Vec3 b) { return {a.y * b.z - a.z * b.y, a.z * b.x - a.x * b.z, a.x * b.y - a.y * b.x}; }
__device__ __forceinline__ Vec3 unit(Vec3 a) { return (1.0f / sqrtf(dot(a, a))) * a; }

__device__ __forceinline__ void settle_positions(const Vec3 (&x0)[3], Vec3 (&x1)[3], const RigidWater& g) {
    const Vec3 b0 = x0[1] - x0[0], c0 = x0[2] - x0[0];
    const Vec3 A1 = x1[0] - x0[0], B1 = x1[1] - x0[0], C1 = x1[2] - x0[0];
    const float inv_m = 1.0f / (g.m_o + 2.0f * g.m_h);
    const Vec3 d0 = inv_m * ((g.m_o * A1) + (g.m_h * (B1 + C1)));
    const Vec3 a1 = A1 - d0, b1 = B1 - d0, c1 = C1 - d0;
    Vec3 n0 = cross(b0, c0), n1 = cross(a1, n0), n2 = cross(n0, n1);
    n0 = unit(n0); n1 = unit(n1); n2 = unit(n2);
    const float b0x = dot(b0, n1), b0y = dot(b0, n2), c0x = dot(c0, n1), c0y = dot(c0, n2);
    const float a1z = dot(a1, n0);
    const float b1x = dot(b1, n1), b1y = dot(b1, n2), b1z = dot(b1, n0);
    const float c1x = dot(c1, n1), c1y = dot(c1, n2), c1z = dot(c1, n0);
    const float sinphi = a1z / g.ra, cosphi = sqrtf(1.0f - sinphi * sinphi);
    const float sinpsi = (b1z - c1z) / (2.0f * g.rc * cosphi), cospsi = sqrtf(1.0f - sinpsi * sinpsi);
    const float a2y = g.ra * cosphi, a2z = g.ra * sinphi;
    const float b2x = -g.rc * cospsi, b2y = -g.rb * cosphi - g.rc * sinpsi * sinphi, b2z = -g.rb * sinphi + g.rc * sinpsi * cosphi;
    const float c2x = g.rc * cospsi, c2y = -g.rb * cosphi + g.rc * sinpsi * sinphi, c2z = -g.rb * sinphi - g.rc * sinpsi * cosphi;
    const float alpha = b2x * (b0x - c0x) + b0y * b2y + c0y * c2y;
    const float beta = b2x * (c0y - b0y) + b0x * b2y + c0x * c2y;
    const float gamma = (b0x * b1y - b1x * b0y) + (c0x * c1y - c1x * c0y);
    const float a2b2 = alpha * alpha + beta * beta;
    const float sint = (alpha * gamma - beta * sqrtf(a2b2 - gamma * gamma)) / a2b2, cost = sqrtf(1.0f - sint * sint);
    const float a3x = -a2y * sint, a3y = a2y * cost;
    const float b3x = b2x * cost - b2y * sint, b3y = b2x * sint + b2y * cost;
    const float c3x = c2x * cost - c2y * sint, c3y = c2x * sint + c2y * cost;
    const Vec3 base = x0[0] + d0;
    x1[0] = base + ((a3x * n1) + (a3y * n2)) + (a2z * n0);
    x1[1] = base + ((b3x * n1) + (b3y * n2)) + (b2z * n0);
    x1[2] = base + ((c3x * n1) + (c3y * n2)) + (c2z * n0);
}

__device__ __forceinline__ void settle_velocities(const Vec3 (&x)[3], Vec3 (&v)[3], const RigidWater& g) {
    const float wo = 1.0f / g.m_o, wh = 1.0f / g.m_h;
    const Vec3 r0 = x[0] - x[1], r1 = x[0] - x[2], r2 = x[1] - x[2];
    const float y0 = -dot(r0, v[0] - v[1]), y1 = -dot(r1, v[0] - v[2]), y2 = -dot(r2, v[1] - v[2]);
    const float a00 = (wo + wh) * dot(r0, r0), a01 = wo * dot(r0, r1), a02 = -wh * dot(r0, r2);
    const float a11 = (wo + wh) * dot(r1, r1), a12 = wh * dot(r1, r2), a22 = 2.0f * wh * dot(r2, r2);
    const float c00 = a11 * a22 - a12 * a12, c01 = a02 * a12 - a01 * a22, c02 = a01 * a12 - a02 * a11;
    const float c11 = a00 * a22 - a02 * a02, c12 = a01 * a02 - a00 * a12, c22 = a00 * a11 - a01 * a01;
    const float inv_det = 1.0f / ((a00 * c00 + a01 * c01) + a02 * c02);
    const float g0 = ((c00 * y0 + c01 * y1) + c02 * y2) * inv_det;
    const float g1 = ((c01 * y0 + c11 * y1) + c12 * y2) * inv_det;
    const float g2 = ((c02 * y0 + c12 * y1) + c22 * y2) * inv_det;
    v[0] = v[0] + (wo * ((g0 * r0) + (g1 * r1)));
    v[1] = v[1] + (wh * ((g2 * r2) - (g0 * r0)));
    v[2] = v[2] - (wh * ((g1 * r1) + (g2 * r2)));
}

__device__ __forceinline__ void load_mol(const float* p, int m, Vec3 (&o)[3]) {
#pragma unroll
    for (int k = 0; k < 3; ++k) o[k] = {p[9 * m + 3 * k], p[9 * m + 3 * k + 1], p[9 * m + 3 * k + 2]};
}
__device__ __forceinline__ void store_mol(float* p, int m, const Vec3 (&o)[3]) {
#pragma unroll
    for (int k = 0; k < 3; ++k) { p[9 * m + 3 * k] = o[k].x; p[9 * m + 3 * k + 1] = o[k].y; p[9 * m + 3 * k + 2] = o[k].z; }
}
__device__ __forceinline__ void wrap_mol(Vec3 (&x)[3], const float (&box)[3]) {
    const Vec3 s = {floorf(x[0].x / box[0]) * box[0], floorf(x[0].y / box[1]) * box[1], floorf(x[0].z / box[2]) * box[2]};
#pragma unroll
    for (int k = 0; k < 3; ++k) x[k] = x[k] - s;
}

__device__ __forceinline__ void d_baoab_first_mol(const MdArgs& a, int m) {
    Vec3 x[3], v[3], f[3];
    load_mol(a.x, m, x); load_mol(a.v, m, v); load_mol(a.f, m, f);
    const float w[3] = {1.0f / a.rigid.m_o, 1.0f / a.rigid.m_h, 1.0f / a.rigid.m_h};
    const float hdt = 0.5f * a.dt;
    const BoxAtom ba = md_box_atom(a.bx, 3 * m);
    float box[3];
    md_box(a.bx, a.box, ba.box, box);
    if (a.com.enabled) {
        float com[3];
        md_com_velocity(a.com, ba.box, com);
#pragma unroll
        for (int k = 0; k < 3; ++k) v[k] = v[k] - Vec3{com[0], com[1], com[2]};
    }
#pragma unroll
    for (int k = 0; k < 3; ++k) v[k] = v[k] + ((hdt * a.len * w[k]) * f[k]);
    settle_velocities(x, v, a.rigid);
#pragma unroll
    for (int stage = 0; stage < 2; ++stage) {
        Vec3 x1[3], xc[3];
#pragma unroll
        for (int k = 0; k < 3; ++k) { x1[k] = x[k] + (hdt * v[k]); xc[k] = x1[k]; }
        settle_positions(x, xc, a.rigid);
#pragma unroll
        for (int k = 0; k < 3; ++k) { v[k] = v[k] + ((1.0f / hdt) * (xc[k] - x1[k])); x[k] = xc[k]; }
        settle_velocities(x, v, a.rigid);
        if (stage == 0) {
#pragma unroll
            for (int k = 0; k < 3; ++k) {
                float xi[3];
                atom_noise(a.seed + (unsigned long long)ba.box, a.step, ba.local + k, xi);
                const float bs = a.b_len_kT * sqrtf(w[k]);
                v[k] = (a.a * v[k]) + Vec3{bs * xi[0], bs * xi[1], bs * xi[2]};
            }
            settle_velocities(x, v, a.rigid);
        }
    }
    wrap_mol(x, box);
    store_mol(a.x, m, x); store_mol(a.v, m, v);
}

__device__ __forceinline__ void d_baoab_second_mol(const MdArgs& a, int m) {
    Vec3 x[3], v[3], f[3];
    load_mol(a.x, m, x); load_mol(a.v, m, v); load_mol(a.f, m, f);
    const float w[3] = {1.0f / a.rigid.m_o, 1.0f / a.rigid.m_h, 1.0f / a.rigid.m_h};
#pragma unroll
    for (int k = 0; k < 3; ++k) v[k] = v[k] + ((0.5f * a.dt * a.len * w[k]) * f[k]);
    settle_velocities(x, v, a.rigid);
    store_mol(a.v, m, v);
}

}

#pragma clang fp contract(fast)
```

gamd_amd/csrc/neighbor.hip:

```cpp
#include "gamd_common.h"
#include "gamd_internal.h"
#include "gamd_md_dev.h"

namespace {

__device__ __forceinline__ int cell_coord(float p, float box, int nc) {
    int c = (int)floorf(p * ((float)nc / box));
    return c < 0 ? 0 : (c >= nc ? nc - 1 : c);
}

#define GAMD_GATE() do { if (a.gate && *a.gate == 0) return; } while (0)

__device__ __forceinline__ float node_feature(const NbrArgs& a, int v) {
    return a.feat ? a.feat[v] : (a.species ? (float)a.species[v] : 0.f);
}

__device__ __forceinline__ int box_id(const NbrArgs& a, int i) { return a.bx.n_boxes > 1 ? gamd_box_of(a.bx, i) : 0; }
__device__ __forceinline__ BoxDims box_dims(const NbrArgs& a, int b) {
    if (a.bx.n_boxes <= 1) {
        float bx = a.box[0], by = a.box[1], bz = a.box[2], hx = a.half[0], hy = a.half[1], hz = a.half[2];
        asm volatile("" : "+r"(bx), "+r"(by), "+r"(bz), "+r"(hx), "+r"(hy), "+r"(hz));
        return BoxDims{bx, by, bz, hx, hy, hz};
    }
    const float4 B = a.bx.boxes[3 * b], H = a.bx.boxes[3 * b + 1];
    return BoxDims{B.x, B.y, B.z, H.x, H.y, H.z};
}
struct BoxCells { int nx, ny, nz, base; };
__device__ __forceinline__ BoxCells box_cells(const NbrArgs& a, int b) {
    if (a.bx.n_boxes <= 1) {
        int nx = a.nc[0], ny = a.nc[1], nz = a.nc[2];
        asm volatile("" : "+r"(nx), "+r"(ny), "+r"(nz));
        return BoxCells{nx, ny, nz, 0};
    }
    const int4 c = reinterpret_cast<const int4*>(a.bx.boxes)[3 * b + 2];
    return BoxCells{c.x, c.y, c.z, c.w};
}

__device__ __forceinline__ void d_bin(const NbrArgs& a, int i) {
    const int bi = box_id(a, i);
    const BoxDims B = box_dims(a, bi);
    float4 p;
    p.x = gamd_remainder(a.pos[3 * i + 0], B.bx);
    p.y = gamd_remainder(a.pos[3 * i + 1], B.by);
    p.z = gamd_remainder(a.pos[3 * i + 2], B.bz);
    p.w = 0.f;
    a.pos_w[i] = p;
    if (a.ref_pos) a.ref_pos[i] = p;
    const BoxCells G = box_cells(a, bi);
    const int c = G.base + (cell_coord(p.x, B.bx, G.nx) * G.ny + cell_coord(p.y, B.by, G.ny)) * G.nz + cell_coord(p.z, B.bz, G.nz);
    (void)GAMD_CHK_RANGE(a.sticky, c, 0, a.ncell - 1, GAMD_CHK_CELL);
    a.cell_of[i] = c;
    atomicAdd(&a.cell_cnt[c], 1);
}

__global__ void k_bin(NbrArgs a) {
    GAMD_GATE();
    const int i = blockIdx.x * blockDim.x + threadIdx.x;
    if (i < a.n) d_bin(a, i);
}

template <typename F>
__device__ __forceinline__ void block_exclusive_scan(int n, F load, int* __restrict__ out) {
    constexpr int IPT = 4;
    __shared__ int wave_tot[16];
    __shared__ int carry_s;
    const int tid = threadIdx.x, lane = tid & 63, wv = tid >> 6;
    if (tid == 0) carry_s = 0;
    __syncthreads();
    for (int base = 0; base < n; base += 1024 * IPT) {
        const int i0 = base + tid * IPT;
        int v[IPT];
        int mine = 0;
#pragma unroll
        for (int k = 0; k < IPT; ++k) { v[k] = (i0 + k < n) ? load(i0 + k) : 0; mine += v[k]; }
        int x = mine;
#pragma unroll
        for (int d = 1; d < 64; d <<= 1) {
            const int y = __shfl_up(x, d, 64);
            if (lane >= d) x += y;
        }
        if (lane == 63) wave_tot[wv] = x;
        __syncthreads();
        int woff = 0;
        for (int w = 0; w < wv; ++w) woff += wave_tot[w];
        const int carry = carry_s;
        int run = carry + woff + x - mine;
#pragma unroll
        for (int k = 0; k < IPT; ++k) {
            if (i0 + k < n) out[i0 + k] = run;
            run += v[k];
        }
        __syncthreads();
        if (tid == 1023) carry_s = run;
        __syncthreads();
    }
    if (tid == 0) out[n] = carry_s;
}

__global__ void __launch_bounds__(1024) k_scan_cells(NbrArgs a) {
    GAMD_GATE();
    block_exclusive_scan(a.ncell, [&](int i) { return a.cell_cnt[i]; }, a.cell_start);
}

__device__ __forceinline__ void d_fill_cells(const NbrArgs& a, int i) {
    const int c = GAMD_CHK_RANGE(a.sticky, a.cell_of[i], 0, a.ncell - 1, GAMD_CHK_CELL);
    const int s = atomicAdd(&a.cell_fill[c], 1);
    a.perm[GAMD_CHK_RANGE(a.sticky, a.cell_start[c] + s, 0, a.n - 1, GAMD_CHK_PERM)] = i;
}

__global__ void k_fill_cells(NbrArgs a) {
    GAMD_GATE();
    const int i = blockIdx.x * blockDim.x + threadIdx.x;
    if (i < a.n) d_fill_cells(a, i);
}

__device__ __forceinline__ void d_sort_gather(const NbrArgs& a, int c, int lane) {
    const int s = a.cell_start[c], e = a.cell_start[c + 1], cnt = e - s;
    if (cnt <= 64) {
        const int v = lane < cnt ? a.perm[s + lane] : 0x7fffffff;
        int rank = 0;
        for (int j = 0; j < cnt; ++j) rank += (__shfl(v, j, 64) < v) ? 1 : 0;
        if (lane < cnt) {
            a.perm[s + rank] = v;
            float4 p = a.pos_w[v];
            p.w = node_feature(a, v);
            a.pos_s[s + rank] = p;
            a.inv_perm[v] = s + rank;
        }
    } else {
        if (lane == 0) {
            for (int i = s + 1; i < e; ++i) {
                const int v = a.perm[i];
                int j = i - 1;
                while (j >= s && a.perm[j] > v) { a.perm[j + 1] = a.perm[j]; --j; }
                a.perm[j + 1] = v;
            }
        }
        __builtin_amdgcn_fence(__ATOMIC_RELEASE, "workgroup");
        __builtin_amdgcn_wave_barrier();
        __builtin_amdgcn_fence(__ATOMIC_ACQUIRE, "workgroup");
        for (int i = s + lane; i < e; i += 64) {
            const int v = ((volatile int*)a.perm)[i];
            float4 p = a.pos_w[v];
            p.w = node_feature(a, v);
            a.pos_s[i] = p;
            a.inv_perm[v] = i;
        }
    }
}

__global__ void __launch_bounds__(256) k_sort_gather(NbrArgs a) {
    GAMD_GATE();
    const int c = (blockIdx.x * blockDim.x + threadIdx.x) >> 6;
    if (c < a.ncell) d_sort_gather(a, c, threadIdx.x & 63);
}

__device__ __forceinline__ float gamd_mask_d2(const float4& pc, const float4& pb, const BoxDims& B) {
#pragma clang fp contract(off)
    const float rx = gamd_min_image_wrapped(pc.x - pb.x, B.bx, B.hx);
    const float ry = gamd_min_image_wrapped(pc.y - pb.y, B.by, B.hy);
    const float rz = gamd_min_image_wrapped(pc.z - pb.z, B.bz, B.hz);
    const float xx = rx * rx, yy = ry * ry, zz = rz * rz;
    return (xx + yy) + zz;
}

typedef __attribute__((address_space(3))) const f32x4* LdsPos;
typedef __attribute__((address_space(3))) const int* LdsCells;
__device__ __forceinline__ float4 pos_at(const float4* p, int i) { return p[i]; }
__device__ __forceinline__ float4 pos_at(LdsPos p, int i) { const f32x4 v = p[i]; return make_float4(v[0], v[1], v[2], v[3]); }

template <typename V, typename PosPtr, typename CellPtr>
__device__ __forceinline__ void sweep_d2(const NbrArgs& a, int ctr, int l, V visit, PosPtr pos_s, CellPtr cell_start) {
    const float4 pc = pos_at(pos_s, ctr);
    const int bi = box_id(a, ctr);
    const BoxDims B = box_dims(a, bi);
    const BoxCells G = box_cells(a, bi);
    const int cx = cell_coord(pc.x, B.bx, G.nx);
    const int cy = cell_coord(pc.y, B.by, G.ny);
    const int cz = cell_coord(pc.z, B.bz, G.nz);
    const int lx = G.nx >= 3 ? -1 : -cx, hx = G.nx >= 3 ? 1 : G.nx - 1 - cx;
    const int ly = G.ny >= 3 ? -1 : -cy, hy = G.ny >= 3 ? 1 : G.ny - 1 - cy;
    const int lz = G.nz >= 3 ? -1 : -cz, hz = G.nz >= 3 ? 1 : G.nz - 1 - cz;
    for (int dx = lx; dx <= hx; ++dx) {
        int x = cx + dx; x += x < 0 ? G.nx : 0; x -= x >= G.nx ? G.nx : 0;
        for (int dy = ly; dy <= hy; ++dy) {
            int y = cy + dy; y += y < 0 ? G.ny : 0; y -= y >= G.ny ? G.ny : 0;
            for (int dz = lz; dz <= hz; ++dz) {
                int z = cz + dz; z += z < 0 ? G.nz : 0; z -= z >= G.nz ? G.nz : 0;
                const int c = G.base + (x * G.ny + y) * G.nz + z;
                const int s = cell_start[c], e = cell_start[c + 1];
                for (int b0 = s; b0 < e; b0 += 32) {
                    const int b = b0 + l;
                    float d2 = 0.f;
                    if (b < e) { const float4 pb = pos_at(pos_s, b); d2 = gamd_mask_d2(pc, pb, B); }
                    visit(b < e, d2, b);
                }
            }
        }
    }
}
template <typename V>
__device__ __forceinline__ void sweep_d2(const NbrArgs& a, int ctr, int l, V visit) { sweep_d2(a, ctr, l, visit, a.pos_s, a.cell_start); }
__device__ __forceinline__ bool in_range(int flavour, float d2, float rc, float rc2, bool is_self) {
    return flavour == 0 ? d2 < rc2
                        : (sqrtf(d2) <= rc) && !is_self;
}
template <typename V, typename PosPtr, typename CellPtr>
__device__ __forceinline__ void sweep(const NbrArgs& a, int ctr, int l, V visit, PosPtr pos_s, CellPtr cell_start) {
// ... 232 lines not shown
template <typename PosPtr, typename CellPtr>
__device__ __forceinline__ void d_fill(const NbrArgs& a, int ctr, int l, PosPtr pos_s, CellPtr cell_start) {
    const bool live = ctr < a.n;
    const int c = live ? ctr : a.n - 1;
    long long w = a.row_ptr[c];
    sweep(a, c, l, [&](bool ok, int b) {
        const unsigned m = half_ballot(ok);
        if (ok && live) {
            const long long at = w + __popc(m & ((1u << l) - 1u));
            if (at < a.e_cap) { a.col[at] = b; if (a.erow) a.erow[at] = c; }
        }
        w += __popc(m);
    }, pos_s, cell_start);
    if (a.self_loop && live && l == 0 && w < a.e_cap) { a.col[w] = c; if (a.erow) a.erow[w] = c; }
    if (live) d_fill_padding(a, c, l, w + (a.self_loop ? 1 : 0));
}
__device__ __forceinline__ void d_fill(const NbrArgs& a, int ctr, int l) { d_fill(a, ctr, l, a.pos_s, a.cell_start); }

__global__ void __launch_bounds__(256) k_fill(NbrArgs a) {
    GAMD_GATE();
    d_fill(a, (blockIdx.x * blockDim.x + threadIdx.x) >> 5, threadIdx.x & 31);
    for (int k = blockIdx.x * blockDim.x + threadIdx.x; k < a.ncell; k += gridDim.x * blockDim.x) { a.cell_cnt[k] = 0; a.cell_fill[k] = 0; }
}

__global__ void k_chunk_meta(NbrArgs a) {
    const int c = blockIdx.x * blockDim.x + threadIdx.x;
    long long E = a.counters[CNT_E];
    if (E > a.e_cap) E = a.e_cap;
    const long long x0 = (long long)c * GAMD_CHUNK;
    if (x0 >= E) {
        if (x0 < a.e_cap + GAMD_TILE) { a.chunk_piece[c] = 0; a.chunk_mask[c] = 0; }
        return;
    }
    const int first_atom = a.erow[x0];
    const int na_incl = a.na_excl[first_atom] +
                        ((a.deg[first_atom] > 0 && (a.row_ptr[first_atom] % GAMD_CHUNK) != 0) ? 1 : 0);
    a.chunk_piece[c] = c + na_incl;
    unsigned mask = 0;
    int prev = first_atom;
    for (int r = 0; r < GAMD_CHUNK; ++r) {
        const long long x = x0 + r;
        if (x >= E) break;
        const int nxt = (x + 1 < E) ? a.erow[x + 1] : -1;
        if (nxt != prev) mask |= 1u << r;
        prev = nxt;
    }
    a.chunk_mask[c] = mask;
}

__device__ __forceinline__ NbrArgs cand_args(const NbrArgs& a) {
    NbrArgs c = a;
    c.rc = a.rc_build; c.rc2 = a.rc2_build;
    c.deg = a.cand_deg; c.row_ptr = a.cand_ptr; c.col = a.cand_col; c.erow = nullptr; c.e_cap = a.cand_cap;
    c.self_loop = 0;
    c.gate = nullptr;
    return c;
}

constexpr int CELL_BATCH = 8;

__device__ void d_bin_batch(const NbrArgs& a, int tid) {
    for (int base = tid; base < a.n; base += 1024 * CELL_BATCH) {
        float px[CELL_BATCH], py[CELL_BATCH], pz[CELL_BATCH];
#pragma unroll
        for (int b = 0; b < CELL_BATCH; ++b) {
            const int i = base + 1024 * b;
            if (i < a.n) { px[b] = a.pos[3 * i + 0]; py[b] = a.pos[3 * i + 1]; pz[b] = a.pos[3 * i + 2]; }
        }
#pragma unroll
        for (int b = 0; b < CELL_BATCH; ++b) {
            const int i = base + 1024 * b;
            if (i < a.n) {
                const int bi = box_id(a, i);
                const BoxDims B = box_dims(a, bi);
                float4 p;
                p.x = gamd_remainder(px[b], B.bx);
                p.y = gamd_remainder(py[b], B.by);
                p.z = gamd_remainder(pz[b], B.bz);
                p.w = 0.f;
                a.pos_w[i] = p;
                if (a.ref_pos) a.ref_pos[i] = p;
                const BoxCells G = box_cells(a, bi);
                const int c = G.base + (cell_coord(p.x, B.bx, G.nx) * G.ny + cell_coord(p.y, B.by, G.ny)) * G.nz + cell_coord(p.z, B.bz, G.nz);
                a.cell_of[i] = c;
                atomicAdd(&a.cell_cnt[c], 1);
            }
        }
    }
}

__device__ void d_fill_cells_batch(const NbrArgs& a, int tid) {
    for (int base = tid; base < a.n; base += 1024 * CELL_BATCH) {
        int c[CELL_BATCH], s[CELL_BATCH], st[CELL_BATCH];
#pragma unroll
        for (int b = 0; b < CELL_BATCH; ++b) { const int i = base + 1024 * b; c[b] = i < a.n ? a.cell_of[i] : -1; }
#pragma unroll
        for (int b = 0; b < CELL_BATCH; ++b)
            if (c[b] >= 0) { s[b] = atomicAdd(&a.cell_fill[c[b]], 1); st[b] = a.cell_start[c[b]]; }
#pragma unroll
        for (int b = 0; b < CELL_BATCH; ++b)
            if (c[b] >= 0) a.perm[st[b] + s[b]] = base + 1024 * b;
    }
}

__device__ void d_sort_gather_batch(const NbrArgs& a, int wave, int lane, int c_begin, int c_end) {
    for (int k0 = c_begin + wave; k0 < c_end; k0 += 16 * CELL_BATCH) {
        int s[CELL_BATCH], cnt[CELL_BATCH], v[CELL_BATCH], rank[CELL_BATCH];
#pragma unroll
        for (int b = 0; b < CELL_BATCH; ++b) {
            const int k = k0 + 16 * b;
            s[b] = k < c_end ? a.cell_start[k] : 0;
            cnt[b] = k < c_end ? a.cell_start[k + 1] - s[b] : 0;
        }
#pragma unroll
        for (int b = 0; b < CELL_BATCH; ++b) v[b] = (cnt[b] <= 64 && lane < cnt[b]) ? a.perm[s[b] + lane] : 0x7fffffff;
        int maxc = 0;
#pragma unroll
        for (int b = 0; b < CELL_BATCH; ++b) { rank[b] = 0; if (cnt[b] <= 64 && cnt[b] > maxc) maxc = cnt[b]; }
        for (int j = 0; j < maxc; ++j) {
#pragma unroll
            for (int b = 0; b < CELL_BATCH; ++b) rank[b] += (__shfl(v[b], j, 64) < v[b]) ? 1 : 0;
        }
        float4 p[CELL_BATCH];
        float f[CELL_BATCH];
#pragma unroll
        for (int b = 0; b < CELL_BATCH; ++b)
            if (cnt[b] <= 64 && lane < cnt[b]) { p[b] = a.pos_w[v[b]]; f[b] = node_feature(a, v[b]); }
#pragma unroll
        for (int b = 0; b < CELL_BATCH; ++b)
            if (cnt[b] <= 64 && lane < cnt[b]) {
                a.perm[s[b] + rank[b]] = v[b];
                a.pos_s[s[b] + rank[b]] = make_float4(p[b].x, p[b].y, p[b].z, f[b]);
                a.inv_perm[v[b]] = s[b] + rank[b];
            }
        unsigned over = 0;
#pragma unroll
        for (int b = 0; b < CELL_BATCH; ++b) over |= cnt[b] > 64 ? 1u << b : 0u;
        for (int b = 0; over >> b; ++b)
            if ((over >> b) & 1u) d_sort_gather(a, k0 + 16 * b, lane);
    }
}

__device__ void d_cells_one_wg(const NbrArgs& c) {
    const int tid = threadIdx.x;
    d_bin_batch(c, tid);
    __syncthreads();
    block_exclusive_scan(c.ncell, [&](int i) { return c.cell_cnt[i]; }, c.cell_start);
    __syncthreads();
    d_fill_cells_batch(c, tid);
    __syncthreads();
    d_sort_gather_batch(c, tid >> 6, tid & 63, 0, c.ncell);
}

__device__ __forceinline__ bool d_moved_beyond(const float4& p, const float4& r, const BoxDims& B, float skin_half2) {
#pragma clang fp contract(off)
    const float dx = gamd_min_image_wrapped(p.x - r.x, B.bx, B.hx);
    const float dy = gamd_min_image_wrapped(p.y - r.y, B.by, B.hy);
    const float dz = gamd_min_image_wrapped(p.z - r.z, B.bz, B.hz);
    return !(((dx * dx + dy * dy) + dz * dz) <= skin_half2);
}

__device__ __forceinline__ bool d_skin_check(const NbrArgs& a, int i) {
    const BoxDims B = box_dims(a, box_id(a, i));
    float4 p;
    p.x = gamd_remainder(a.pos[3 * i + 0], B.bx);
    p.y = gamd_remainder(a.pos[3 * i + 1], B.by);
    p.z = gamd_remainder(a.pos[3 * i + 2], B.bz);
    p.w = 0.f;
    a.pos_w[i] = p;
    bool moved = a.force_rebuild != 0;
    if (!moved) {
        moved = d_moved_beyond(p, a.ref_pos[i], B, a.skin_half2);
    }
    p.w = node_feature(a, i);
    a.pos_s[a.inv_perm[i]] = p;
    return moved;
}

__device__ __forceinline__ bool d_skin_check_mol(const NbrArgs& a, int i0) {
    float px[3][3];
    float4 r[3];
    int ip[3];
    float w[3];
#pragma unroll
    for (int k = 0; k < 3; ++k) {
        const int i = i0 + k < a.n ? i0 + k : a.n - 1;
        px[k][0] = a.pos[3 * i + 0]; px[k][1] = a.pos[3 * i + 1]; px[k][2] = a.pos[3 * i + 2];
        r[k] = a.ref_pos[i];
        ip[k] = a.inv_perm[i];
        w[k] = node_feature(a, i);
    }
    bool moved = a.force_rebuild != 0;
#pragma unroll
    for (int k = 0; k < 3; ++k) {
        const int i = i0 + k;
        if (i < a.n) {
            const BoxDims B = box_dims(a, box_id(a, i));
            float4 p;
            p.x = gamd_remainder(px[k][0], B.bx);
            p.y = gamd_remainder(px[k][1], B.by);
            p.z = gamd_remainder(px[k][2], B.bz);
            p.w = 0.f;
            a.pos_w[i] = p;
            if (!a.force_rebuild) moved |= d_moved_beyond(p, r[k], B, a.skin_half2);
            p.w = w[k];
            a.pos_s[ip[k]] = p;
        }
    }
    return moved;
}

__global__ void k_skin_check(NbrArgs a, MdArgs md, int do_second, int do_first) {
    const int i = blockIdx.x * blockDim.x + threadIdx.x;
    if (a.counters_next && i < CNT_COUNT) a.counters_next[i] = 0;
    if (do_second | do_first) {
        if (md.devflags[DEVFLAG_FROZEN]) {
            if (i == 0 && md.devflags[DEVFLAG_FROZEN_AT] < 0)
                md.devflags[DEVFLAG_FROZEN_AT] = do_second ? 2 * (md.step_index - 1) + 1 : 2 * md.step_index;
        } else if (md.use_rigid) {
            if (3 * i < a.n) {
                if (do_second) gamd_md::d_baoab_second_mol(md, i);
                if (do_first) gamd_md::d_baoab_first_mol(md, i);
            }
        } else if (i < a.n) {
            if (do_second) {
#pragma unroll
                for (int d = 0; d < 3; ++d) d_baoab_second_dof(md, 3 * i + d);
            }
            if (do_first) d_baoab_first_atom(md, i);
        }
    }
    bool moved = false;
    if ((do_second | do_first) && md.use_rigid) {
        if (3 * i < a.n) moved = d_skin_check_mol(a, 3 * i);
    } else if (i < a.n) {
        moved = d_skin_check(a, i);
    }
    if (moved) a.counters[CNT_REBUILD] = 1;
}

__global__ void __launch_bounds__(1024) k_cells_one_wg(NbrArgs a) {
    if (a.counters[CNT_REBUILD] == 0) return;
    d_cells_one_wg(cand_args(a));
}

constexpr int CELLS_SL_MAXCELL = 4096;
constexpr int CELLS_SL_WGS = 32;

struct BinOut { float4 p; int c; };
__device__ __forceinline__ BinOut d_wrap_cell(const NbrArgs& a, int i, float px, float py, float pz) {
    const int bi = box_id(a, i);
    const BoxDims B = box_dims(a, bi);
    BinOut o;
    o.p.x = gamd_remainder(px, B.bx);
    o.p.y = gamd_remainder(py, B.by);
    o.p.z = gamd_remainder(pz, B.bz);
    o.p.w = 0.f;
    const BoxCells G = box_cells(a, bi);
    o.c = G.base + (cell_coord(o.p.x, B.bx, G.nx) * G.ny + cell_coord(o.p.y, B.by, G.ny)) * G.nz + cell_coord(o.p.z, B.bz, G.nz);
    return o;
}

__global__ void __launch_bounds__(1024) k_cells_sliced(NbrArgs a0) {
    if (a0.counters[CNT_REBUILD] == 0) return;
    __shared__ int s_cnt[CELLS_SL_MAXCELL];
    __shared__ int s_start[CELLS_SL_MAXCELL + 1];
    __shared__ int s_range[2];
    const NbrArgs a = cand_args(a0);
    const int tid = threadIdx.x, w = blockIdx.x, nwg = gridDim.x;
    for (int k = tid; k < a.ncell; k += 1024) s_cnt[k] = 0;
    __syncthreads();
    for (int base = tid; base < a.n; base += 1024 * CELL_BATCH) {
        float px[CELL_BATCH], py[CELL_BATCH], pz[CELL_BATCH];
#pragma unroll
        for (int b = 0; b < CELL_BATCH; ++b) {
            const int i = base + 1024 * b;
            if (i < a.n) { px[b] = a.pos[3 * i + 0]; py[b] = a.pos[3 * i + 1]; pz[b] = a.pos[3 * i + 2]; }
        }
#pragma unroll
        for (int b = 0; b < CELL_BATCH; ++b) {
            const int i = base + 1024 * b;
            if (i < a.n) atomicAdd(&s_cnt[d_wrap_cell(a, i, px[b], py[b], pz[b]).c], 1);
        }
    }
    __syncthreads();
    block_exclusive_scan(a.ncell, [&](int i) { return s_cnt[i]; }, s_start);
    __syncthreads();
    if (tid < 2) {
        const int which = w + tid;
        int c;
        if (which == 0) c = 0;
        else if (which >= nwg) c = a.ncell;
        else {
            const int chunk = (a.n + nwg - 1) / nwg;
            const int target = which * chunk < a.n ? which * chunk : a.n;
            int lo = 0, hi = a.ncell;
            while (lo < hi) { const int mid = (lo + hi) >> 1; if (s_start[mid] >= target) hi = mid; else lo = mid + 1; }
            c = lo;
        }
        s_range[tid] = c;
    }
    for (int k = tid; k < a.ncell; k += 1024) s_cnt[k] = 0;
    __syncthreads();
    const int c0 = s_range[0], c1 = s_range[1];
    for (int k = c0 + tid; k <= c1; k += 1024) a.cell_start[k] = s_start[k];
    for (int base = tid; base < a.n; base += 1024 * CELL_BATCH) {
        float px[CELL_BATCH], py[CELL_BATCH], pz[CELL_BATCH];
#pragma unroll
        for (int b = 0; b < CELL_BATCH; ++b) {
            const int i = base + 1024 * b;
            if (i < a.n) { px[b] = a.pos[3 * i + 0]; py[b] = a.pos[3 * i + 1]; pz[b] = a.pos[3 * i + 2]; }
        }
#pragma unroll
        for (int b = 0; b < CELL_BATCH; ++b) {
            const int i = base + 1024 * b;
            if (i < a.n) {
                const BinOut o = d_wrap_cell(a, i, px[b], py[b], pz[b]);
                if (o.c >= c0 && o.c < c1) {
                    a.pos_w[i] = o.p;
                    if (a.ref_pos) a.ref_pos[i] = o.p;
                    a.cell_of[i] = o.c;
                    a.perm[s_start[o.c] + atomicAdd(&s_cnt[o.c], 1)] = i;
                }
            }
        }
    }
    __syncthreads();
    d_sort_gather_batch(a, tid >> 6, tid & 63, c0, c1);
}

__global__ void __launch_bounds__(1024) k_step_small(NbrArgs a, MdArgs md, int do_second, int do_first) {
    const int tid = threadIdx.x;
    if (do_second | do_first) {
        if (md.devflags[DEVFLAG_FROZEN]) {
            if (tid == 0 && md.devflags[DEVFLAG_FROZEN_AT] < 0)
                md.devflags[DEVFLAG_FROZEN_AT] = do_second ? 2 * (md.step_index - 1) + 1 : 2 * md.step_index;
        } else if (md.use_rigid) {
            if (3 * tid < a.n) {
                if (do_second) gamd_md::d_baoab_second_mol(md, tid);
                if (do_first) gamd_md::d_baoab_first_mol(md, tid);
            }
        } else if (tid < a.n) {
            if (do_second) {
#pragma unroll
                for (int d = 0; d < 3; ++d) d_baoab_second_dof(md, 3 * tid + d);
            }
            if (do_first) d_baoab_first_atom(md, tid);
        }
    }
    bool moved = false;
    if ((do_second | do_first) && md.use_rigid) {
        if (3 * tid < a.n) moved = d_skin_check_mol(a, 3 * tid);
    } else if (tid < a.n) {
        moved = d_skin_check(a, tid);
    }
    if (tid < CNT_COUNT) a.counters_next[tid] = 0;
    if (!__syncthreads_or(moved ? 1 : 0)) return;
    if (tid == 0) a.counters[CNT_REBUILD] = 1;
    NbrArgs c = cand_args(a);
    for (int k = tid; k < c.ncell; k += 1024) { c.cell_cnt[k] = 0; c.cell_fill[k] = 0; }
    __syncthreads();
    if (tid < c.n) d_bin(c, tid);
    __syncthreads();
    block_exclusive_scan(c.ncell, [&](int i) { return c.cell_cnt[i]; }, c.cell_start);
    __syncthreads();
    if (tid < c.n) d_fill_cells(c, tid);
    __syncthreads();
    for (int k = tid >> 6; k < c.ncell; k += 16) d_sort_gather(c, k, tid & 63);
    __syncthreads();
}

template <bool FILL, typename RowPtr>
__device__ __forceinline__ void d_filter(const NbrArgs& a, int ctr, int l, RowPtr row_ptr) {
    const bool live = ctr < a.n;
    const int c = live ? ctr : a.n - 1;
    const float4 pc = a.pos_s[c];
    const BoxDims B = box_dims(a, box_id(a, c));
    long long s, e;
    if (a.cand_stride > 0) {
        const int dgc = a.cand_deg[c];
        s = (long long)c * a.cand_stride;
        e = s + (dgc < a.cand_stride ? dgc : a.cand_stride);
    } else {
        s = a.cand_ptr[c]; e = a.cand_ptr[c + 1];
        if (e > a.cand_cap) e = a.cand_cap;
        if (s > e) s = e;
    }
    long long w = FILL ? (long long)row_ptr[c] : 0;
    int cnt = 0;
    for (long long b0 = s; b0 < e; b0 += 32) {
        bool ok = false;
        int b = 0;
        if (b0 + l < e) {
            b = GAMD_CHK_RANGE(a.sticky, a.cand_col[b0 + l], 0, a.n, GAMD_CHK_CAND);
            const float4 pb = a.pos_s[b];
            const float d2 = gamd_mask_d2(pc, pb, B);
            if (a.flavour == 0) ok = d2 < a.rc2;
            else ok = (sqrtf(d2) <= a.rc) && (b != c);
        }
        const unsigned m = half_ballot(ok);
        if (FILL) {
            if (ok && live) {
                const long long at = w + __popc(m & ((1u << l) - 1u));
                if (at < a.e_cap) { a.col[at] = b; a.erow[at] = c; }
            }
            w += __popc(m);
        } else {
            cnt += __popc(m);
        }
    }
    if (FILL && a.self_loop && live && l == 0 && w < a.e_cap) { a.col[w] = c; a.erow[w] = c; }
    if (FILL && live) d_fill_padding(a, c, l, w + (a.self_loop ? 1 : 0));
    if (!FILL && live && l == 0) a.deg[ctr] = cnt + (a.self_loop ? 1 : 0);
}

template <bool FILL>
// ... 196 lines not shown
#pragma unroll
    for (int k = 0; k < 4; ++k) {
        if (i0 + k <= a.n) s_na[i0 + k] = run2;
        run2 += f[k];
    }
    if (tid == 255 && a.n == 1024) s_na[1024] = run2;
    __syncthreads();
    const int E_all = s_rp[a.n];
    long long E = E_all;
    if (E > a.e_cap) E = a.e_cap;
    if (blockIdx.x == 0) {
        if (a.cand_stride > 0 && a.counters[CNT_REBUILD]) d_publish_candidates<256>(a);
        for (int i = tid; i <= a.n; i += 256) { a.row_ptr[i] = s_rp[i]; a.na_excl[i] = s_na[i]; }
        if (tid == 0) {
            a.counters[CNT_E] = E_all;
            a.counters[CNT_PIECES] = (E_all + GAMD_CHUNK - 1) / GAMD_CHUNK + s_na[a.n];
            if ((long long)E_all > a.e_cap) {
                a.counters[CNT_OVERFLOW] = 1; a.sticky[STICKY_EDGE_OVERFLOW] = 1; a.devflags[DEVFLAG_FROZEN] = 1;
            }
            a.counters[CNT_TILES] = (E_all + GAMD_TILE - 1) / GAMD_TILE;
        }
    }
    d_filter<true>(a, (blockIdx.x * 256 + tid) >> 5, tid & 31, s_rp);
    const int n_chunks = 2 * (int)((E + GAMD_TILE - 1) / GAMD_TILE);
    for (int c = blockIdx.x * 256 + tid; c < n_chunks; c += gridDim.x * 256) {
        const long long x0 = (long long)c * GAMD_CHUNK;
        if (x0 >= E) { a.chunk_piece[c] = 0; a.chunk_mask[c] = 0; continue; }
        int lo = 0, hi = a.n - 1;
        while (lo < hi) { const int mid = (lo + hi + 1) >> 1; if (s_rp[mid] <= x0) lo = mid; else hi = mid - 1; }
        int at = lo;
        while (s_rp[at + 1] <= x0) ++at;
        const int na_incl = s_na[at] + ((s_rp[at + 1] > s_rp[at] && (s_rp[at] % GAMD_CHUNK) != 0) ? 1 : 0);
        a.chunk_piece[c] = c + na_incl;
        unsigned mask = 0;
        for (int r = 0; r < GAMD_CHUNK; ++r) {
            const long long xe = x0 + r;
            if (xe >= E) break;
            while (s_rp[at + 1] <= xe) ++at;
            if (xe == (long long)s_rp[at + 1] - 1 || xe == E - 1) mask |= 1u << r;
        }
        a.chunk_mask[c] = mask;
    }
}

__global__ void k_identity_sort(NbrArgs a) {
    const int i = blockIdx.x * blockDim.x + threadIdx.x;
    if (i >= a.n) return;
    const BoxDims B = box_dims(a, box_id(a, i));
    float4 p;
    p.x = gamd_remainder(a.pos[3 * i + 0], B.bx);
    p.y = gamd_remainder(a.pos[3 * i + 1], B.by);
    p.z = gamd_remainder(a.pos[3 * i + 2], B.bz);
    p.w = node_feature(a, i);
    a.pos_w[i] = p;
    a.pos_s[i] = p;
    a.perm[i] = i;
    a.inv_perm[i] = i;
    a.deg[i] = a.self_loop ? 1 : 0;
}

__global__ void k_edges_count(NbrArgs a, const int* __restrict__ centre, const int* __restrict__ neigh, long long ne) {
    const long long e = (long long)blockIdx.x * blockDim.x + threadIdx.x;
    if (e >= ne) return;
    const int c = centre[e], j = neigh[e];
    if (c >= 0 && c < a.n && j >= 0 && j < a.n) atomicAdd(&a.deg[c], 1);
    else a.counters[CNT_OVERFLOW] = 2;
}

__global__ void k_edges_fill(NbrArgs a, const int* __restrict__ centre, const int* __restrict__ neigh, long long ne,
                             int* __restrict__ tmp_eid) {
    const long long e = (long long)blockIdx.x * blockDim.x + threadIdx.x;
    if (e >= ne) return;
    const int c = centre[e], j = neigh[e];
    if (c < 0 || c >= a.n || j < 0 || j >= a.n) return;
    const int s = atomicAdd(&a.cell_of[c], 1);
    const long long at = (long long)a.row_ptr[c] + s;
    if (at < a.e_cap) tmp_eid[at] = (int)e;
}

__global__ void __launch_bounds__(256) k_edges_sort_rows(NbrArgs a, const int* __restrict__ neigh,
                                                         const int* __restrict__ tmp_eid) {
    const int row = (blockIdx.x * blockDim.x + threadIdx.x) >> 6;
    const int lane = threadIdx.x & 63;
    if (row >= a.n) return;
    const long long s = a.row_ptr[row];
    long long e = a.row_ptr[row + 1];
    if (e > a.e_cap) e = a.e_cap;
    const int total = (int)(e - s);
    int cnt = a.cell_of[row];
    if (cnt > total) cnt = total;
    int behind = cnt;
    if (a.self_loop && behind < total) {
        if (lane == 0) { a.col[s + behind] = row; a.erow[s + behind] = row; }
        ++behind;
    }
    for (int x = behind + lane; x < total; x += 64) { a.col[s + x] = a.n; a.erow[s + x] = row; }
    if (cnt <= 0) return;
    if (cnt <= 64) {
        const int v = lane < cnt ? tmp_eid[s + lane] : 0x7fffffff;
        int rank = 0;
        for (int j = 0; j < cnt; ++j) rank += (__shfl(v, j, 64) < v) ? 1 : 0;
        if (lane < cnt) { a.col[s + rank] = neigh[v]; a.erow[s + rank] = row; }
    } else {
        for (int i = lane; i < cnt; i += 64) {
            const int v = tmp_eid[s + i];
            int rank = 0;
            for (int j = 0; j < cnt; ++j) rank += (tmp_eid[s + j] < v) ? 1 : 0;
            a.col[s + rank] = neigh[v];
            a.erow[s + rank] = row;
        }
    }
}

}

int launch_csr_from_edges(const NbrArgs& a, const int* centre, const int* neigh, long long n_edges, int* tmp_eid,
                          hipStream_t st) {
    hipError_t e;
    e = hipMemsetAsync(a.counters, 0, sizeof(int) * CNT_COUNT, st); if (e) return (int)e;
    e = hipMemsetAsync(a.cell_of, 0, sizeof(int) * (size_t)a.n, st); if (e) return (int)e;
    const int tb = 256, gb = (a.n + tb - 1) / tb;
    hipLaunchKernelGGL(k_identity_sort, dim3(gb), dim3(tb), 0, st, a); GAMD_CHECK_LAUNCH();
    if (n_edges > 0) {
        const unsigned ge = (unsigned)((n_edges + tb - 1) / tb);
        hipLaunchKernelGGL(k_edges_count, dim3(ge), dim3(tb), 0, st, a, centre, neigh, n_edges); GAMD_CHECK_LAUNCH();
        hipLaunchKernelGGL(k_scan_deg, dim3(1), dim3(1024), 0, st, a); GAMD_CHECK_LAUNCH();
        hipLaunchKernelGGL(k_edges_fill, dim3(ge), dim3(tb), 0, st, a, centre, neigh, n_edges, tmp_eid); GAMD_CHECK_LAUNCH();
        hipLaunchKernelGGL(k_edges_sort_rows, dim3((a.n + 3) / 4), dim3(256), 0, st, a, neigh, tmp_eid); GAMD_CHECK_LAUNCH();
    } else {
        hipLaunchKernelGGL(k_scan_deg, dim3(1), dim3(1024), 0, st, a); GAMD_CHECK_LAUNCH();
    }
    const long long nchunk_cap = (a.e_cap + GAMD_TILE) / GAMD_CHUNK;
    hipLaunchKernelGGL(k_chunk_meta, dim3((unsigned)((nchunk_cap + 255) / 256)), dim3(256), 0, st, a);
    GAMD_CHECK_LAUNCH();
    return 0;
}

int launch_neighbor_skin(const NbrArgs& a, hipStream_t st, const MdFuse* fuse) {
    hipError_t e;
    const int tb = 256, gb = (a.n + tb - 1) / tb, ga = (a.n + 7) / 8;
    if (a.counters_next && a.use_small) {
        if (a.n > 1024) return -22;
        MdArgs md{};
        if (fuse) md = *fuse->md;
        hipLaunchKernelGGL(k_step_small, dim3(1), dim3(1024), 0, st, a, md, fuse ? fuse->do_second : 0, fuse ? fuse->do_first : 0);
        GAMD_CHECK_LAUNCH();
        NbrArgs x = a;
        x.ref_pos = nullptr;
        hipLaunchKernelGGL(k_filter_count, dim3(ga), dim3(256), 0, st, x); GAMD_CHECK_LAUNCH();
        hipLaunchKernelGGL(k_filter_fill_small, dim3(ga), dim3(256), 0, st, x); GAMD_CHECK_LAUNCH();
        return 0;
    }
    if (!a.counters_next) { e = hipMemsetAsync(a.counters, 0, sizeof(int) * CNT_COUNT, st); if (e) return (int)e; }
    {
        MdArgs md{};
        if (fuse) md = *fuse->md;
        hipLaunchKernelGGL(k_skin_check, dim3(gb), dim3(tb), 0, st, a, md, fuse ? fuse->do_second : 0, fuse ? fuse->do_first : 0);
        GAMD_CHECK_LAUNCH();
    }
    if (a.cells_one_wg && a.n <= 16 * 1024) {
        if (a.ncell <= CELLS_SL_MAXCELL) hipLaunchKernelGGL(k_cells_sliced, dim3(CELLS_SL_WGS), dim3(1024), 0, st, a);
        else hipLaunchKernelGGL(k_cells_one_wg, dim3(1), dim3(1024), 0, st, a);
        GAMD_CHECK_LAUNCH();
    } else {
        NbrArgs c = a;
        c.gate = a.counters + CNT_REBUILD;
        c.rc = a.rc_build; c.rc2 = a.rc2_build;
        c.deg = a.cand_deg; c.row_ptr = a.cand_ptr; c.col = a.cand_col; c.erow = nullptr; c.e_cap = a.cand_cap;
        c.self_loop = 0;
        hipLaunchKernelGGL(k_bin, dim3(gb), dim3(tb), 0, st, c); GAMD_CHECK_LAUNCH();
        hipLaunchKernelGGL(k_scan_cells, dim3(1), dim3(1024), 0, st, c); GAMD_CHECK_LAUNCH();
        hipLaunchKernelGGL(k_fill_cells, dim3(gb), dim3(tb), 0, st, c); GAMD_CHECK_LAUNCH();
        hipLaunchKernelGGL(k_sort_gather, dim3((a.ncell + 3) / 4), dim3(256), 0, st, c); GAMD_CHECK_LAUNCH();
    }
    NbrArgs x = a;
    x.ref_pos = nullptr;
    hipLaunchKernelGGL(k_filter_count, dim3(ga), dim3(256), 0, st, x); GAMD_CHECK_LAUNCH();
    if (a.bx.n_boxes <= 1 && a.n <= 16 * 1024 && a.cand_stride > 0) {
        hipLaunchKernelGGL(k_filter_fill_scan, dim3(ga), dim3(256), 0, st, x); GAMD_CHECK_LAUNCH();
        return 0;
    }
    hipLaunchKernelGGL(k_scan_deg, dim3(1), dim3(1024), 0, st, x); GAMD_CHECK_LAUNCH();
    hipLaunchKernelGGL(k_filter<true>, dim3(ga), dim3(256), 0, st, x); GAMD_CHECK_LAUNCH();
    return 0;
}

int launch_neighbor_build(const NbrArgs& a, hipStream_t st) {
    hipError_t e;
    e = hipMemsetAsync(a.counters, 0, sizeof(int) * (CNT_COUNT + 2 * (size_t)a.ncell_cap), st); if (e) return (int)e;
    const int tb = 256, gb = (a.n + tb - 1) / tb;
    hipLaunchKernelGGL(k_bin, dim3(gb), dim3(tb), 0, st, a); GAMD_CHECK_LAUNCH();
    hipLaunchKernelGGL(k_scan_cells, dim3(1), dim3(1024), 0, st, a); GAMD_CHECK_LAUNCH();
    hipLaunchKernelGGL(k_fill_cells, dim3(gb), dim3(tb), 0, st, a); GAMD_CHECK_LAUNCH();
    hipLaunchKernelGGL(k_sort_gather, dim3((a.ncell + 3) / 4), dim3(256), 0, st, a); GAMD_CHECK_LAUNCH();
    const int ga = (a.n + 7) / 8;
    hipLaunchKernelGGL(k_count, dim3(ga), dim3(256), 0, st, a); GAMD_CHECK_LAUNCH();
    hipLaunchKernelGGL(k_scan_deg, dim3(1), dim3(1024), 0, st, a); GAMD_CHECK_LAUNCH();
    hipLaunchKernelGGL(k_fill, dim3(ga), dim3(256), 0, st, a); GAMD_CHECK_LAUNCH();
    const long long nchunk_cap = (a.e_cap + GAMD_TILE) / GAMD_CHUNK;
    hipLaunchKernelGGL(k_chunk_meta, dim3((unsigned)((nchunk_cap + 255) / 256)), dim3(256), 0, st, a);
    GAMD_CHECK_LAUNCH();
    return 0;
}
```

gamd_amd/csrc/node.hip:

```cpp
#include "gamd_common.h"
#include "gamd_internal.h"

namespace {

typedef _Float16 nf16x8 __attribute__((ext_vector_type(8)));
typedef _Float16 nf16x2 __attribute__((ext_vector_type(2)));
typedef float nf32x2 __attribute__((ext_vector_type(2)));

constexpr int NT = 16;
constexpr int XLD = 136;

__device__ __forceinline__ f32x4 mfma16(float a, float b, f32x4 c) {
    return __builtin_amdgcn_mfma_f32_16x16x4f32(a, b, c, 0, 0, 0);
}

struct WHalf { f32x4 w[8]; };
__device__ __forceinline__ void load_whalf(const float* __restrict__ Wp, int w, int lane, int half, WHalf& h) {
    const f32x4* W = reinterpret_cast<const f32x4*>(Wp) + (size_t)w * 16 * 64 + lane;
#pragma unroll
    for (int o = 0; o < 2; ++o)
#pragma unroll
        for (int b = 0; b < 4; ++b) h.w[o * 4 + b] = W[(o * 8 + 4 * half + b) * 64];
}

__device__ __forceinline__ void gemm16_half(const WHalf& h, int half, const f32x4 (&XB)[8], f32x4 (&acc)[2]) {
#pragma unroll
    for (int b = 0; b < 4; ++b)
#pragma unroll
        for (int r = 0; r < 4; ++r) {
            acc[0] = mfma16(h.w[b][r], XB[4 * half + b][r], acc[0]);
            acc[1] = mfma16(h.w[4 + b][r], XB[4 * half + b][r], acc[1]);
        }
}

struct XSplit { nf16x8 h[4], l[4]; };
__device__ __forceinline__ void split16(const f32x4 (&XB)[8], XSplit& s) {
#pragma unroll
    for (int m = 0; m < 4; ++m)
#pragma unroll
        for (int j = 0; j < 8; j += 2) {
            const f32x4& q = XB[2 * m + (j >> 2)];
            const nf32x2 x = {q[j & 3], q[(j & 3) + 1]};
            const nf16x2 hi = __builtin_convertvector(x, nf16x2);
            const nf32x2 rem = x - __builtin_convertvector(hi, nf32x2);
            const nf16x2 lo = __builtin_convertvector(rem, nf16x2);
            s.h[m][j] = hi[0]; s.h[m][j + 1] = hi[1];
            s.l[m][j] = lo[0]; s.l[m][j + 1] = lo[1];
        }
}
__device__ __forceinline__ void gemm16_half_f16(const WHalf& h, int half, const XSplit& X, f32x4 (&acc)[2]) {
#pragma unroll
    for (int mm = 0; mm < 2; ++mm) {
        const int m = 2 * half + mm;
#pragma unroll
        for (int o = 0; o < 2; ++o) {
            const nf16x8 wh = __builtin_bit_cast(nf16x8, h.w[o * 4 + mm * 2]), wl = __builtin_bit_cast(nf16x8, h.w[o * 4 + mm * 2 + 1]);
            acc[o] = __builtin_amdgcn_mfma_f32_16x16x32_f16(wh, X.l[m], acc[o], 0, 0, 0);
            acc[o] = __builtin_amdgcn_mfma_f32_16x16x32_f16(wl, X.h[m], acc[o], 0, 0, 0);
            acc[o] = __builtin_amdgcn_mfma_f32_16x16x32_f16(wh, X.h[m], acc[o], 0, 0, 0);
        }
    }
}

template <bool NEXT, bool F16, typename XT>
__device__ __forceinline__ void gemm16(const float* W, const float* next, WHalf& wn, const XT& XB, f32x4 (&acc)[2], int w, int lane) {
    WHalf cur = wn;
    asm volatile("" ::: "memory");
    load_whalf(W, w, lane, 1, wn);
    asm volatile("" ::: "memory");
    if constexpr (F16) gemm16_half_f16(cur, 0, XB, acc); else gemm16_half(cur, 0, XB, acc);
    __builtin_amdgcn_sched_barrier(0);
    cur = wn;
    if (NEXT) {
        asm volatile("" ::: "memory");
        load_whalf(next, w, lane, 0, wn);
        asm volatile("" ::: "memory");
    }
    if constexpr (F16) gemm16_half_f16(cur, 1, XB, acc); else gemm16_half(cur, 1, XB, acc);
    __builtin_amdgcn_sched_barrier(0);
}

__device__ __forceinline__ void load16(const float* __restrict__ row, int w, int g, f32x4 (&v)[2]) {
    v[0] = *reinterpret_cast<const f32x4*>(row + 32 * w + 4 * g);
    v[1] = *reinterpret_cast<const f32x4*>(row + 32 * w + 16 + 4 * g);
}
__device__ __forceinline__ void store16(float* __restrict__ row, int w, int g, const f32x4 (&v)[2]) {
    *reinterpret_cast<f32x4*>(row + 32 * w + 4 * g) = v[0];
    *reinterpret_cast<f32x4*>(row + 32 * w + 16 + 4 * g) = v[1];
}

__device__ __forceinline__ void exchange16(float* xbuf, int w, int a, int g, const f32x4 (&mine)[2], f32x4 (&XB)[8]) {
    __syncthreads();
    store16(xbuf + a * XLD, w, g, mine);
    __syncthreads();
#pragma unroll
    for (int blk = 0; blk < 8; ++blk) XB[blk] = *reinterpret_cast<const f32x4*>(xbuf + a * XLD + 16 * blk + 4 * g);
}

typedef _Float16 nf16x4 __attribute__((ext_vector_type(4)));
__device__ __forceinline__ nf16x4 cvt16x4(const f32x4& v) {
    const nf16x2 lo = __builtin_convertvector(nf32x2{v[0], v[1]}, nf16x2), hi = __builtin_convertvector(nf32x2{v[2], v[3]}, nf16x2);
    return nf16x4{lo[0], lo[1], hi[0], hi[1]};
}
__device__ __forceinline__ void store16_h(_Float16* __restrict__ row, int w, int g, const f32x4 (&v)[2]) {
    *reinterpret_cast<nf16x4*>(row + 32 * w + 4 * g) = cvt16x4(v[0]);
    *reinterpret_cast<nf16x4*>(row + 32 * w + 16 + 4 * g) = cvt16x4(v[1]);
}
__device__ __forceinline__ void store16_tab(_Float16* __restrict__ row, int w, int g, const f32x4 (&v)[2]) {
    *reinterpret_cast<nf16x4*>(row + 32 * w + 8 * (g & 1) + 4 * (g >> 1)) = cvt16x4(v[0]);
    *reinterpret_cast<nf16x4*>(row + 32 * w + 16 + 8 * (g & 1) + 4 * (g >> 1)) = cvt16x4(v[1]);
}

__device__ __forceinline__ float group_sum(float v) {
    v += __shfl_xor(v, 16, 64);
    return v + __shfl_xor(v, 32, 64);
}

template <bool F16>
__global__ void __launch_bounds__(256, 3) k_node(NodeArgs a) {
    __shared__ __attribute__((aligned(16))) float xbuf[NT * XLD];
    __shared__ float obuf[4][NT][3];
    __shared__ float red[2][4][NT];

    if (a.counters[CNT_OVERFLOW] || a.devflags[DEVFLAG_FROZEN]) return;
    if (a.mode == 0 && a.l0_gate && a.counters[CNT_REBUILD] == 0) return;

    const int lane = threadIdx.x & 63, la = lane & 15, g = lane >> 4;
    const int w = __builtin_amdgcn_readfirstlane(threadIdx.x >> 6);
    const int atom_raw = blockIdx.x * NT + la;
    const bool valid = atom_raw < a.n;
    const int atom = valid ? atom_raw : a.n - 1;
    const size_t row = (size_t)atom * GAMD_H;

#ifdef GAMD_PROFILING
    long long tm[16] = {0, 0, 0, 0, 0, 0, 0, 0, 0, 0, 0, 0, 0, 0, 0, 0};
#define NMARK(I) do { if (a.tdbg) tm[I] = (long long)__builtin_readcyclecounter(); } while (0)
#else
#define NMARK(I) do { } while (0)
#endif
    NMARK(0);
    f32x4 XB[8];
    XSplit XS;
#define GEMM16(NEXT, W, NXT) do { if constexpr (F16) gemm16<NEXT, true>(W, NXT, wn, XS, mine, w, lane); \
                                  else gemm16<NEXT, false>(W, NXT, wn, XB, mine, w, lane); } while (0)
#define SPLIT16() do { if constexpr (F16) split16(XB, XS); } while (0)
    f32x4 mine[2];
    WHalf wn;

    if (a.mode == 0) {
        if (a.node_emb) {
            load16(a.node_emb, w, g, mine);
        } else {
            const float f = a.pos_s[atom].w;
            f32x4 ww[2];
            load16(a.enc_w, w, g, ww);
            load16(a.enc_b, w, g, mine);
#pragma unroll
            for (int o = 0; o < 2; ++o)
#pragma unroll
                for (int r = 0; r < 4; ++r) mine[o][r] = f * ww[o][r] + mine[o][r];
        }
        if (valid) store16(a.h_out + row, w, g, mine);
        load_whalf(a.pre.wsp, w, lane, 0, wn);
    } else {
        const int rp0 = a.row_ptr[atom], dg = a.deg[atom];
        const int na_incl = a.na_excl[atom] + ((dg > 0 && (rp0 % GAMD_CHUNK) != 0) ? 1 : 0);
        const int p0 = rp0 / GAMD_CHUNK + na_incl;
        const int np = dg > 0 ? ((rp0 + dg - 1) / GAMD_CHUNK - rp0 / GAMD_CHUNK + 1) : 0;
        (void)GAMD_CHK_RANGE(a.sticky, (long long)p0 + np, 0, a.piece_cap, GAMD_CHK_NODE_PIECES);
        float n_real = 0.f;
        if (a.post.c0) {
            float n_pad = 0.f;
            if (a.col) {
#pragma unroll
                for (int k = 0; k < 4; ++k) {
                    const int j = g + 4 * k;
                    if (j < dg && a.col[rp0 + dg - 1 - j] == a.n) n_pad += 1.f;
                }
                n_pad = group_sum(n_pad);
            }
            n_real = (float)dg - n_pad;
        }
        mine[0] = f32x4{0.f, 0.f, 0.f, 0.f};
        mine[1] = mine[0];
        f32x4 p_in[2], h_res[2];
        load16(a.P_in + row, w, g, p_in);
        for (int k0 = 0; __any(k0 < np); k0 += 8) {
            f32x4 pc[8][2];
#pragma unroll
            for (int k = 0; k < 8; ++k) {
                const int kk = (k0 + k < np) ? k0 + k : (np > 0 ? np - 1 : 0);
                load16(a.partial + (size_t)(np > 0 ? p0 + kk : 0) * GAMD_H, w, g, pc[k]);
            }
#pragma unroll
            for (int k = 0; k < 8; ++k)
                if (k0 + k < np) { mine[0] += pc[k][0]; mine[1] += pc[k][1]; }
        }
        NMARK(1);
        asm volatile("" ::: "memory");
        load_whalf(a.post.wpep, w, lane, 0, wn);
        exchange16(xbuf, w, la, g, mine, XB);
        SPLIT16();
        NMARK(2);
        mine[0] = p_in[0]; mine[1] = p_in[1];
        GEMM16(true, a.post.wpep, a.post.wphip);
        if (a.post.c0) {
            f32x4 c[2];
            load16(a.post.c0, w, g, c);
#pragma unroll
            for (int o = 0; o < 2; ++o)
#pragma unroll
                for (int r = 0; r < 4; ++r) mine[o][r] = fmaf(n_real, c[o][r], mine[o][r]);
        }
        NMARK(3);
#pragma unroll
        for (int o = 0; o < 2; ++o)
#pragma unroll
            for (int r = 0; r < 4; ++r) mine[o][r] = gamd_silu_hw(mine[o][r]);
        exchange16(xbuf, w, la, g, mine, XB);
        SPLIT16();
        NMARK(4);
        load16(a.post.bphi, w, g, mine);
        load16(a.h_in + row, w, g, h_res);
        GEMM16(true, a.post.wphip, a.mode != 2 ? a.pre.wsp : a.dec_w1p);
        mine[0] += h_res[0]; mine[1] += h_res[1];
        if (valid) store16(a.h_out + row, w, g, mine);
        NMARK(5);
    }

    if (a.mode != 2) {
        float mean = 0.f, rstd = 1.0f;
        if (!a.norm_bn) {
            float ps = 0.f;
#pragma unroll
            for (int o = 0; o < 2; ++o)
#pragma unroll
                for (int r = 0; r < 4; ++r) ps += mine[o][r];
            ps = group_sum(ps);
            if (g == 0) red[0][w][la] = ps;
            __syncthreads();
            mean = ((red[0][0][la] + red[0][1][la]) + (red[0][2][la] + red[0][3][la])) * a.ln_inv_width;
            float pv = 0.f;
#pragma unroll
            for (int o = 0; o < 2; ++o)
#pragma unroll
                for (int r = 0; r < 4; ++r) { const float d = mine[o][r] - mean; pv += d * d; }
            pv = group_sum(pv);
            if (g == 0) red[1][w][la] = pv;
            __syncthreads();
            const float var = (((red[1][0][la] + red[1][1][la]) + (red[1][2][la] + red[1][3][la])) - a.ln_n_pad * (mean * mean)) * a.ln_inv_width;
            rstd = 1.0f / sqrtf(var + 1e-5f);
        }
        {
            f32x4 gg[2], bb[2];
            load16(a.pre.ln_g, w, g, gg);
            load16(a.pre.ln_b, w, g, bb);
#pragma unroll
            for (int o = 0; o < 2; ++o)
#pragma unroll
                for (int r = 0; r < 4; ++r) mine[o][r] = (mine[o][r] - mean) * rstd * gg[o][r] + bb[o][r];
        }
        if (valid && a.tab16) store16_h(reinterpret_cast<_Float16*>(a.hn_out) + row, w, g, mine);
        else if (valid && !a.hn_perm) store16(a.hn_out + row, w, g, mine);
        exchange16(xbuf, w, la, g, mine, XB);
        SPLIT16();
        NMARK(6);
        if (a.hn_perm) {
#pragma unroll
            for (int k = 0; k < 2; ++k) {
                const int idx = k * 256 + threadIdx.x, at = idx >> 5, c = idx & 31;
                const float* xr = xbuf + at * XLD + c;
                const f32x4 v = {xr[0], xr[32], xr[64], xr[96]};
                const int atom_k = blockIdx.x * NT + at;
                if (atom_k < a.n) *reinterpret_cast<f32x4*>(a.hn_out + (size_t)atom_k * GAMD_H + 4 * c) = v;
            }
        }
        load16(a.pre.bS, w, g, mine);
        GEMM16(true, a.pre.wsp, a.pre.wdp);
        if (valid && a.tab16) store16_tab(reinterpret_cast<_Float16*>(a.S_out) + row, w, g, mine);
        else if (valid) store16(a.S_out + row, w, g, mine);
        NMARK(7);
        mine[0] = f32x4{0.f, 0.f, 0.f, 0.f};
        mine[1] = mine[0];
        GEMM16(true, a.pre.wdp, a.pre.wpdp);
        if (valid && a.tab16) store16_tab(reinterpret_cast<_Float16*>(a.D_out) + row, w, g, mine);
        else if (valid) store16(a.D_out + row, w, g, mine);
        NMARK(8);
        load16(a.pre.bP, w, g, mine);
        GEMM16(false, a.pre.wpdp, nullptr);
        if (valid) store16(a.P_out + row, w, g, mine);
        NMARK(9);
#ifdef GAMD_PROFILING
        if (a.tdbg && a.mode == 1 && lane == 0 && blockIdx.x < 512) {
            long long* o = a.tdbg + ((size_t)blockIdx.x * 4 + w) * 16;
            for (int i = 0; i < 16; ++i) o[i] = tm[i];
        }
#endif
    } else {
        exchange16(xbuf, w, la, g, mine, XB);
        SPLIT16();
        load16(a.dec_b1, w, g, mine);
        GEMM16(false, a.dec_w1p, nullptr);
        float o3[3] = {0.f, 0.f, 0.f};
#pragma unroll
        for (int o = 0; o < 2; ++o) {
            const int f0 = 32 * w + 16 * o + 4 * g;
            f32x4 gl;
#pragma unroll
            for (int r = 0; r < 4; ++r) gl[r] = gamd_gelu_hw(mine[o][r]);
#pragma unroll
            for (int c = 0; c < 3; ++c) {
                const f32x4 ww = *reinterpret_cast<const f32x4*>(a.dec_w2 + c * GAMD_H + f0);
#pragma unroll
                for (int r = 0; r < 4; ++r) o3[c] += ww[r] * gl[r];
            }
        }
#pragma unroll
        for (int c = 0; c < 3; ++c) o3[c] = group_sum(o3[c]);
        if (g == 0) {
#pragma unroll
            for (int c = 0; c < 3; ++c) obuf[w][la][c] = o3[c];
        }
        __syncthreads();
        if (w == 0 && g == 0 && valid) {
            const int orig = a.perm[atom];
#pragma unroll
            for (int c = 0; c < 3; ++c) {
                const float v = ((obuf[0][la][c] + obuf[1][la][c]) + (obuf[2][la][c] + obuf[3][la][c])) + a.dec_b2[c];
                a.forces_norm[3 * (size_t)orig + c] = v;
                if (a.forces) a.forces[3 * (size_t)orig + c] = v * a.scale + a.shift;
                if (!(fabsf(v) <= 3.0e38f)) a.sticky[STICKY_NONFINITE] = 1;
            }
        }
    }
}

#undef NMARK
#undef GEMM16
#undef SPLIT16

}

int launch_node(const NodeArgs& a, hipStream_t st) {
    const int nb = (a.n + NT - 1) / NT;
    if (a.f16x3) hipLaunchKernelGGL((k_node<true>), dim3(nb), dim3(256), 0, st, a);
    else hipLaunchKernelGGL((k_node<false>), dim3(nb), dim3(256), 0, st, a);
    GAMD_CHECK_LAUNCH();
    return 0;
}
```

gamd_amd/engine.py:

```python
from __future__ import annotations

import ctypes as C
import os
from typing import Dict, Optional, Sequence, Tuple, Union

import numpy as np
import torch

from . import _lib
from ._lib import GamdReportParams, GamdStructParams, GamdTrajParams, GamdConfig, GamdMdParams, GamdNhcParams, TRAJ_FIELDS, check
from .weights import ModelConfig, infer_config, validate_state_dict

ArrayLike = Union[np.ndarray, torch.Tensor]

KIND = {"lj": 0, "water": 1, "dynbox": 1}
FLAVOUR = {"jaxmd": 0, "torch": 1}
SELF_LOOP = {"dgl07_noop": 0, "append_zero_feature_loops": 1}
KSEL_FORCE_GENERIC_WIDTH = 1
KSEL_NO_LAYER0_HOIST = 4


def _box3(box) -> np.ndarray:
    b = np.asarray(box, dtype=np.float64).reshape(-1)
    if b.size == 1:
        b = np.repeat(b, 3)
    if b.size != 3:
        raise ValueError("box must be a scalar or 3 values")
    return b.astype(np.float32)


def _boxes(box, n_boxes: int) -> np.ndarray:
    b = np.asarray(box, dtype=np.float64)
    if b.ndim == 0 or b.size == 1 or (b.ndim == 1 and b.size == 3):
        return np.tile(_box3(b), (n_boxes, 1))
    if b.ndim == 2 and b.shape == (n_boxes, 3):
        return b.astype(np.float32)
    if (b.ndim == 1 and b.size == n_boxes) or (b.ndim == 2 and b.shape == (n_boxes, 1)):
        return np.repeat(b.reshape(-1).astype(np.float32)[:, None], 3, axis=1)
    raise ValueError(f"box must be a scalar, 3 values, [{n_boxes}, 1] or [{n_boxes}, 3] ({n_boxes} boxes)")


def _rdf_from_counts(counts, frames: int, r_max: float, n_by_class, vol: float):
    c = np.asarray(counts).astype(np.float64)
    n_pairs, bins = c.shape
    if bins == 0 or frames == 0:
        raise ValueError("no histogram was recorded")
    nn = np.atleast_1d(np.asarray(n_by_class, dtype=np.float64))
    if n_pairs == 1:
        m = np.array([nn[0] ** 2])
    else:
        if nn.shape[0] != 2:
            raise ValueError("three pair classes need n_by_class = (N_O, N_H)")
        m = np.array([nn[0] ** 2, 2.0 * nn[0] * nn[1], nn[1] ** 2])
    edges = np.arange(bins + 1, dtype=np.float64) * (r_max / bins)
    shell = 4.0 / 3.0 * np.pi * (edges[1:] ** 3 - edges[:-1] ** 3)
    g = c / (frames * m[:, None] * shell[None, :] / vol)
    return 0.5 * (edges[1:] + edges[:-1]), g


def structure_kvectors(n2max: int) -> np.ndarray:
    n2max = int(n2max)
    if n2max <= 0:
        return np.zeros((0, 3), dtype=np.int32)
    m = int(np.floor(np.sqrt(n2max)))
    while (m + 1) * (m + 1) <= n2max:
        m += 1
    r = np.arange(-m, m + 1)
    n = np.stack(np.meshgrid(r, r, r, indexing="ij"), axis=-1).reshape(-1, 3)
    n2 = (n * n).sum(axis=1)
    lead = np.where(n[:, 0] != 0, n[:, 0], np.where(n[:, 1] != 0, n[:, 1], n[:, 2]))
    keep = (n2 > 0) & (n2 <= n2max) & (lead > 0)
    n, n2 = n[keep], n2[keep]
    order = np.lexsort((n[:, 2], n[:, 1], n[:, 0], n2))
    return n[order].astype(np.int32)


class RunStructure:

    def __init__(self, rdf_counts, sk_sum, kvectors, frames: int, r_max: float = 0.0, boxes=None):
        self.rdf_counts = np.asarray(rdf_counts, dtype=np.uint64)
        self.sk_sum = np.asarray(sk_sum, dtype=np.float64)
        self.kvectors = np.asarray(kvectors, dtype=np.int32).reshape(-1, 3)
        self.frames = int(frames)
        self.r_max = float(r_max)
        self.boxes = None if boxes is None else np.asarray(boxes, dtype=np.float64).reshape(-1, 3)

    def rdf(self, box: int, n_by_class, volume: Optional[float] = None):
        vol = float(volume) if volume is not None else float(np.prod(self.boxes[box]))
        return _rdf_from_counts(self.rdf_counts[box], self.frames, self.r_max, n_by_class, vol)

    def sk(self, box: int, n_by_class, shell_average: bool = False):
        s = self.sk_sum[box]
        n_pairs, K = s.shape
        if K == 0 or self.frames == 0:
            raise ValueError("no structure factor was sampled")
        nn = np.atleast_1d(np.asarray(n_by_class, dtype=np.float64))
        if n_pairs == 1:
            m = np.array([nn[0]])
        else:
            if nn.shape[0] != 2:
                raise ValueError("three pair classes need n_by_class = (N_O, N_H)")
            m = np.array([nn[0], np.sqrt(nn[0] * nn[1]), nn[1]])
        edges = self.boxes[box]
        kk = 2.0 * np.pi * np.sqrt(((self.kvectors.astype(np.float64) / edges[None, :]) ** 2).sum(axis=1))
        val = s / (self.frames * m[:, None])
        if not shell_average:
            return kk, val
        if not (edges[0] == edges[1] == edges[2]):
            raise ValueError("shell_average needs a cubic box")
        n2 = (self.kvectors.astype(np.int64) ** 2).sum(axis=1)
        shells, inv, cnt = np.unique(n2, return_inverse=True, return_counts=True)
        out = np.zeros((n_pairs, shells.shape[0]), dtype=np.float64)
        for c in range(n_pairs):
            out[c] = np.bincount(inv, weights=val[c], minlength=shells.shape[0]) / cnt
        return 2.0 * np.pi * np.sqrt(shells.astype(np.float64)) / edges[0], out


class RunReport:

    def __init__(self, steps, ke, temperature, rdf_counts, frames: int, dropped: int, r_max: float = 0.0, volumes=None):
        self.steps = np.asarray(steps, dtype=np.int64)
        self.ke = np.atleast_2d(np.asarray(ke, dtype=np.float64))
        self.temperature = np.atleast_2d(np.asarray(temperature, dtype=np.float64))
        self.rdf_counts = np.asarray(rdf_counts, dtype=np.uint64)
        self.frames, self.dropped = int(frames), int(dropped)
        self.r_max = float(r_max)
        self.volumes = None if volumes is None else np.asarray(volumes, dtype=np.float64).reshape(-1)

    def rdf(self, box: int, n_by_class, volume: Optional[float] = None):
        c = self.rdf_counts[box]
        if c.shape[1] == 0 or self.frames == 0:
            raise ValueError("no histogram was recorded")
        vol = float(volume) if volume is not None else float(self.volumes[box])
        return _rdf_from_counts(c, self.frames, self.r_max, n_by_class, vol)

    def write_state_data(self, path, dt_ps: float, separator: str = "\t", driver_step_convention: bool = False,
                         box: int = 0) -> None:
        k = 2 if driver_step_convention else 1
        head = ['"Step"', '"Time (ps)"', '"Kinetic Energy (kJ/mole)"', '"Temperature (K)"']
        with open(path, "w") as fh:
            fh.write("#" + separator.join(head) + "\n")
            for i, g in enumerate(self.steps):
                row = [str(k * int(g)), str(k * int(g) * float(dt_ps)), str(float(self.ke[i, box])),
                       str(float(self.temperature[i, box]))]
                fh.write(separator.join(row) + "\n")


class RunTrajectory:

    def __init__(self, steps=None, x=None, v=None, f=None, image=None, dropped: int = 0, ambiguous: int = 0,
                 n_samples: int = 0, class_atoms=None, msd_sum=None, vacf_sum=None, interval: int = 1):
        def arr(a, dt):
            return None if a is None else np.asarray(a, dtype=dt)
        self.steps = np.zeros(0, dtype=np.int64) if steps is None else np.asarray(steps, dtype=np.int64)
        self.x, self.v, self.f = arr(x, np.float32), arr(v, np.float32), arr(f, np.float32)
        self.image = arr(image, np.int32)
        self.dropped, self.ambiguous, self.n_samples = int(dropped), int(ambiguous), int(n_samples)
        self.class_atoms = None if class_atoms is None else np.atleast_2d(np.asarray(class_atoms, dtype=np.int64))
        self.msd_sum, self.vacf_sum = arr(msd_sum, np.float64), arr(vacf_sum, np.float64)
        self.interval = int(interval)

    @property
    def n_lags(self) -> int:
        return 0 if self.msd_sum is None else int(self.msd_sum.shape[-1])

    def unwrapped(self, box) -> np.ndarray:
        if self.x is None or self.image is None:
            raise ValueError("unwrapped needs the fields x and image")
        L = _boxes(box, self.x.shape[1]).astype(np.float64)
        return self.x.astype(np.float64) + self.image.astype(np.float64) * L[None, :, None, :]

    def _normalised(self, sums, box: int) -> np.ndarray:
        if sums is None or self.n_lags == 0:
            raise ValueError("no correlation functions were recorded (n_lags = 0)")
        origins = (self.n_samples - np.arange(self.n_lags)).astype(np.float64)
        den = np.where(origins > 0, origins, np.nan)[None, :] * self.class_atoms[box].astype(np.float64)[:, None]
        with np.errstate(divide="ignore", invalid="ignore"):
            return np.where(den > 0, sums[box] / den, np.nan)

    def msd(self, box: int = 0) -> np.ndarray:
        return self._normalised(self.msd_sum, box)

    def vacf(self, box: int = 0) -> np.ndarray:
        return self._normalised(self.vacf_sum, box)

    def lag_times(self, dt_ps: float) -> np.ndarray:
        return np.arange(self.n_lags, dtype=np.float64) * (self.interval * float(dt_ps))

    def diffusion_msd(self, box: int, cls: int, dt_ps: float, fit: Tuple[int, int], length_per_nm: float = 0.0) -> float:
        lo, hi = int(fit[0]), int(fit[1])
        if not 0 <= lo < hi < self.n_lags:
            raise ValueError(f"fit = ({lo}, {hi}) must satisfy 0 <= lo < hi < n_lags = {self.n_lags}")
        t = self.lag_times(dt_ps)[lo:hi + 1]
        y = self.msd(box)[cls, lo:hi + 1]
        tc = t - t.mean()
        d = float((tc * (y - y.mean())).sum() / (tc * tc).sum()) / 6.0
        return d / float(length_per_nm) ** 2 if length_per_nm else d

    def diffusion_green_kubo(self, box: int, cls: int, dt_ps: float, upto: int, length_per_nm: float = 0.0) -> float:
        upto = int(upto)
        if not 0 < upto < self.n_lags:
            raise ValueError(f"upto = {upto} must satisfy 0 < upto < n_lags = {self.n_lags}")
        c = self.vacf(box)[cls, :upto + 1]
        h = self.interval * float(dt_ps)
        d = float(h * (0.5 * c[0] + c[1:-1].sum() + 0.5 * c[-1])) / 3.0
        return d / float(length_per_nm) ** 2 if length_per_nm else d

    def write_dataset(self, dir, seed: int, prefix: str = "data_", length_per_nm: float = 0.0) -> list:
        if self.x is None:
            raise ValueError("write_dataset needs the field x")
        to_angstrom = np.float64(10.0) / np.float64(np.float32(length_per_nm)) if length_per_nm else np.float64(1.0)
        os.makedirs(dir, exist_ok=True)
        paths = []
        for t in range(self.x.shape[0]):
            out = {"pos": (self.x[t, 0].astype(np.float64) * to_angstrom).astype(np.float32)}
            if self.v is not None:
                out["vel"] = (self.v[t, 0].astype(np.float64) * (to_angstrom * 100.0)).astype(np.float32)
            if self.f is not None:
                out["forces"] = self.f[t, 0].astype(np.float32)
            paths.append(os.path.join(dir, f"{prefix}{seed}_{t}.npz"))
            np.savez(paths[-1], **out)
        return paths


class GamdForce:

    def __init__(self, state_dict: Dict[str, torch.Tensor], n_atoms: int, box, cutoff: float,
                 bond: Optional[np.ndarray] = None, scaler: Tuple[float, float] = (0.0, 1.0),
                 nbr_flavour: str = "jaxmd", device: int = 0, keep_stages: bool = False,
                 edge_capacity: int = 0, cfg: Optional[ModelConfig] = None, edge_dtype: str = "f32",
                 neighbor_skin: float = 0.0, self_loop_mode: str = "dgl07_noop", kernel_select: int = 0,
                 small_tile_limit: int = 0, n_boxes: int = 1):
        self._h = C.c_void_p()
        self._lib = _lib.load()
        if not torch.cuda.is_available():
            raise _lib.GamdError("GamdForce needs a HIP device (torch.cuda.is_available() is False); "
                                 "there is no CPU fallback")
        cfg = cfg or infer_config(state_dict)
        if (not 1 <= cfg.encoding_size <= 256 or not 1 <= cfg.edge_embedding_dim <= 256 or not 1 <= cfg.hidden_dim <= 256
                or cfg.n_rbf not in (0, 40)):
            raise ValueError("the gfx950 kernels cover encoding_size / edge_embedding_dim / hidden_dim up to 256 "
                             "and the RBF expansion on (40 centres) or off "
                             f"(got enc={cfg.encoding_size} hidden={cfg.hidden_dim} edge={cfg.edge_embedding_dim} "
                             f"n_rbf={cfg.n_rbf})")
        validate_state_dict(state_dict, cfg)
        self.cfg = cfg
        self.n = int(n_atoms)
        self.n_boxes = max(1, int(n_boxes))
        self.n_total = self.n * self.n_boxes
        self.device = torch.device("cuda", device)
        self.box = _box3(box)
        self.cutoff = float(cutoff)
        c = GamdConfig()
        c.n_boxes = self.n_boxes
        c.n_atoms, c.kind, c.n_layers = self.n, KIND[cfg.kind], cfg.conv_layer
        c.use_bond, c.nbr_flavour, c.device = int(cfg.use_bond), FLAVOUR[nbr_flavour], device
        c.cutoff = self.cutoff
        for d in range(3):
            c.box[d] = float(self.box[d])
        c.edge_capacity, c.keep_stages = int(edge_capacity), int(keep_stages)
        c.edge_dtype = {"f32": 0, "bf16": 1, "f16x3": 2}[edge_dtype]
        c.encoding_size, c.edge_embedding_dim, c.hidden_dim = cfg.encoding_size, cfg.edge_embedding_dim, cfg.hidden_dim
        c.no_expand_edge = int(cfg.n_rbf == 0)
        c.neighbor_skin = float(neighbor_skin)
        if self_loop_mode not in SELF_LOOP:
            raise ValueError(f"self_loop_mode must be one of {sorted(SELF_LOOP)}")
        c.self_loop_mode = SELF_LOOP[self_loop_mode]
        c.kernel_select, c.small_tile_limit = int(kernel_select), int(small_tile_limit)
        self.edge_dtype = edge_dtype
        check(self._lib.gamd_create(C.byref(c), C.byref(self._h)), "gamd_create")
        self.keep_stages = keep_stages
        for name, t in state_dict.items():
            if name.endswith("num_batches_tracked"):
                continue
            a = np.ascontiguousarray(t.detach().cpu().numpy().astype(np.float32))
            shape = (C.c_int64 * a.ndim)(*a.shape)
            check(self._lib.gamd_load_weight(self._h, name.encode(), a.ctypes.data_as(C.c_void_p), shape, a.ndim),
                  f"gamd_load_weight({name})")
        check(self._lib.gamd_finalize_weights(self._h), "gamd_finalize_weights")
        self.set_scaler(*scaler)
        if cfg.use_bond:
            if bond is None:
                raise ValueError("use_bond model needs the bond list")
            b = np.ascontiguousarray(np.asarray(bond, dtype=np.int32))
            check(self._lib.gamd_set_bonds(self._h, b.ctypes.data_as(C.c_void_p), b.shape[0]), "gamd_set_bonds")
        self._feat = None
        self._out = torch.empty((self.n_total, 3), dtype=torch.float32, device=self.device)
        self._out_den = torch.empty((self.n_total, 3), dtype=torch.float32, device=self.device)
        self.last_status = 0

    def close(self):
        if getattr(self, "_h", None) is not None and self._h.value:
            self._lib.gamd_destroy(self._h)
            self._h = C.c_void_p()

    def __del__(self):
        try:
            self.close()
        except Exception:
            pass

    def set_scaler(self, mean, var):
        self.scaler_mean = np.asarray(mean, dtype=np.float64).reshape(-1)[:1]
        self.scaler_var = np.asarray(var, dtype=np.float64).reshape(-1)[:1]
        check(self._lib.gamd_set_scaler(self._h, float(self.scaler_mean[0]), float(self.scaler_var[0])),
              "gamd_set_scaler")

    def _stream(self):
        return C.c_void_p(torch.cuda.current_stream(self.device).cuda_stream)

    def _dev_pos(self, pos: ArrayLike) -> torch.Tensor:
        if isinstance(pos, np.ndarray):
            pos = torch.from_numpy(np.ascontiguousarray(pos, dtype=np.float32))
        pos = pos.to(device=self.device, dtype=torch.float32).contiguous()
        if tuple(pos.shape) == (self.n_boxes, self.n, 3):
            pos = pos.view(self.n_total, 3)
        if tuple(pos.shape) != (self.n_total, 3):
            raise ValueError(f"pos must be [{self.n_total}, 3]" + (f" or [{self.n_boxes}, {self.n}, 3]" if self.n_boxes > 1 else "")
                             + f", got {tuple(pos.shape)}")
        return pos

    def _md_state(self, *ts):
        for t in ts:
            if not (t.is_cuda and t.dtype == torch.float32 and t.is_contiguous()
                    and tuple(t.shape) in ((self.n_total, 3), (self.n_boxes, self.n, 3))):
                raise ValueError(f"x, v, f must be contiguous float32 CUDA tensors of shape [{self.n_total}, 3]")

    def _dev_species(self, species) -> Optional[torch.Tensor]:
        if species is None:
            self._set_features(None)
            return None
        if isinstance(species, np.ndarray):
            species = torch.from_numpy(species)
        key = None
        if not species.is_cuda:
            c = species.detach().reshape(-1).contiguous()
            key = (str(c.dtype), c.numel(), hash(c.view(torch.uint8).numpy().tobytes()), torch.cuda.current_stream(self.device).cuda_stream)
            hit = getattr(self, "_species_cache", None)
            if hit is not None and hit[0] == key:
                self._set_features(hit[2])
                return hit[1]
        s = species.reshape(-1).to(device=self.device)
        if s.numel() == self.n and self.n_boxes > 1:
            s = s.repeat(self.n_boxes)
        if s.numel() != self.n_total:
            raise ValueError("species must have one entry per atom")
        feat = s.to(torch.float32).contiguous() if s.dtype.is_floating_point and self.cfg.kind != "lj" else None
        self._set_features(feat)
        flags = (s != 0).to(torch.uint8).contiguous()
        self._species_prev = getattr(self, "_species_cache", None)
        self._species_cache = (key, flags, feat)
        return flags

    def _set_features(self, feat: Optional[torch.Tensor]) -> None:
        if feat is None and self._feat is None:
            return
        self._feat = feat
        check(self._lib.gamd_set_node_features(self._h, C.c_void_p(feat.data_ptr()) if feat is not None else None),
              "gamd_set_node_features")

    def _box_arg(self, box):
        b = _boxes(self.box if box is None else box, self.n_boxes)
        return (C.c_float * (3 * self.n_boxes))(*[float(x) for x in b.reshape(-1)])

    def forward(self, pos: ArrayLike, box=None, species=None, denormalize: bool = False,
                inplace: bool = False) -> torch.Tensor:
        p = self._dev_pos(pos)
        s = self._dev_species(species)
        st = self._lib.gamd_forces(self._h, C.c_void_p(p.data_ptr()),
                                   C.c_void_p(s.data_ptr()) if s is not None else None,
                                   self._box_arg(box), C.c_void_p(self._out.data_ptr()),
                                   C.c_void_p(self._out_den.data_ptr()), self._stream())
        self.last_status = check(st, "gamd_forces")
        out = self._out_den if denormalize else self._out
        return out if inplace else out.clone()

    __call__ = forward

    def forward_host(self, pos: np.ndarray, box=None, species=None, denormalize: bool = False) -> np.ndarray:
        pos = np.asarray(pos)
        if pos.shape == (self.n_boxes, self.n, 3):
            pos = pos.reshape(self.n_total, 3)
        if pos.shape != (self.n_total, 3):
            raise ValueError(f"pos must be [{self.n_total}, 3], got {tuple(pos.shape)}")
        p32 = np.ascontiguousarray(pos, dtype=np.float32)
        if getattr(self, "_host_out", None) is None:
            self._host_out = np.empty((self.n_total, 3), dtype=np.float32)
        s = self._dev_species(species)
        st = self._lib.gamd_forces_host(self._h, p32.ctypes.data_as(C.c_void_p), C.c_void_p(s.data_ptr()) if s is not None else None,
                                        self._box_arg(box), self._host_out.ctypes.data_as(C.c_void_p), 1 if denormalize else 0,
                                        self._stream())
        self.last_status = check(st, "gamd_forces_host")
        return self._host_out

    def forward_edges(self, pos: ArrayLike, edge_idx, box=None, species=None, denormalize: bool = False,
                      inplace: bool = False) -> torch.Tensor:
        p = self._dev_pos(pos)
        s = self._dev_species(species)
        if isinstance(edge_idx, np.ndarray):
            edge_idx = torch.from_numpy(edge_idx)
        e = edge_idx.to(device=self.device, dtype=torch.int32).contiguous()
        if e.dim() != 2 or e.shape[0] != 2:
            raise ValueError("edge_idx must be [2, E]")
        st = self._lib.gamd_forces_edges(self._h, C.c_void_p(p.data_ptr()),
                                         C.c_void_p(s.data_ptr()) if s is not None else None, self._box_arg(box),
                                         C.c_void_p(e[0].data_ptr()), C.c_void_p(e[1].data_ptr()), int(e.shape[1]),
                                         C.c_void_p(self._out.data_ptr()), C.c_void_p(self._out_den.data_ptr()),
                                         self._stream())
        self.last_status = check(st, "gamd_forces_edges")
        out = self._out_den if denormalize else self._out
        return out if inplace else out.clone()

    def build_neighbors(self, pos: ArrayLike, box=None, species=None) -> int:
        p = self._dev_pos(pos)
        s = self._dev_species(species)
        st = self._lib.gamd_build_neighbors(self._h, C.c_void_p(p.data_ptr()),
                                            C.c_void_p(s.data_ptr()) if s is not None else None,
                                            self._box_arg(box), self._stream())
        return check(st, "gamd_build_neighbors")

    def counts(self) -> Tuple[int, int, int]:
        e, p, c = C.c_int64(), C.c_int64(), C.c_int64()
        check(self._lib.gamd_get_counts(self._h, C.byref(e), C.byref(p), C.byref(c)), "gamd_get_counts")
        return e.value, p.value, c.value

    def skin_stats(self) -> Tuple[int, int, int]:
        r, c, cap = C.c_int64(), C.c_int64(), C.c_int64()
        check(self._lib.gamd_get_skin_stats(self._h, C.byref(r), C.byref(c), C.byref(cap)), "gamd_get_skin_stats")
        return r.value, c.value, cap.value

    def _dbg(self, what: int, shape, dtype) -> np.ndarray:
        out = np.empty(shape, dtype=dtype)
        check(self._lib.gamd_debug_get(self._h, what, out.ctypes.data_as(C.c_void_p), out.nbytes), "gamd_debug_get")
        return out

    def debug_partial(self) -> np.ndarray:
        return self._dbg(6, (self.counts()[1], 128 * ((self.cfg.encoding_size + 127) // 128)), np.float32)

    def debug_perm(self) -> np.ndarray:
        return self._dbg(0, (self.n_total,), np.int32)

    def debug_csr(self) -> Tuple[np.ndarray, np.ndarray]:
        e = self.counts()[0]
        return self._dbg(1, (self.n_total + 1,), np.int32), self._dbg(2, (e,), np.int32)

    def debug_edges(self) -> np.ndarray:
        perm = self.debug_perm().astype(np.int64)
        row_ptr, col = self.debug_csr()
        dst = np.repeat(np.arange(self.n_total), np.diff(row_ptr))
        real = col < self.n_total
        return np.stack([perm[dst[real]], perm[col[real]]])

    def debug_edge_rows(self) -> np.ndarray:
# ... 244 lines not shown
```

include/gamd_hip.h:

```cpp
#ifndef GAMD_HIP_H
#define GAMD_HIP_H

#include <stdint.h>
#include <stddef.h>

#ifdef __cplusplus
extern "C" {
#endif

typedef struct gamd_handle gamd_handle;

enum { GAMD_EDGE_F32 = 0, GAMD_EDGE_BF16 = 1, GAMD_EDGE_F16X3 = 2 };

enum { GAMD_KIND_LJ = 0, GAMD_KIND_WATER = 1 };
enum { GAMD_NBR_JAXMD = 0, GAMD_NBR_TORCH = 1 };

typedef struct gamd_config {
    int32_t n_atoms;
    int32_t kind;
    int32_t n_layers;
    int32_t use_bond;
    int32_t nbr_flavour;
    int32_t device;
    float cutoff;
    float box[3];
    int64_t edge_capacity;
    int32_t keep_stages;
    int32_t edge_dtype;
    int32_t encoding_size;
    int32_t edge_embedding_dim;
    int32_t hidden_dim;
    int32_t no_expand_edge;
    float neighbor_skin;
    int32_t self_loop_mode;
    int32_t kernel_select;
    int32_t small_tile_limit;
    int32_t n_boxes;
} gamd_config;
enum { GAMD_SELF_LOOP_DGL07_NOOP = 0, GAMD_SELF_LOOP_APPEND_ZERO_FEATURE = 1 };
enum { GAMD_KSEL_FORCE_GENERIC_WIDTH = 1, GAMD_KSEL_FORCE_HALF_QUANTUM = 2, GAMD_KSEL_NO_LAYER0_HOIST = 4 };

const char* gamd_version(void);
const char* gamd_last_error(void);

int32_t gamd_create(const gamd_config* cfg, gamd_handle** out);
int32_t gamd_destroy(gamd_handle* h);

int32_t gamd_load_weight(gamd_handle* h, const char* name, const float* data, const int64_t* shape, int32_t ndim);
int32_t gamd_finalize_weights(gamd_handle* h);

int32_t gamd_set_scaler(gamd_handle* h, double mean, double var);

int32_t gamd_set_bonds(gamd_handle* h, const int32_t* bonds, int64_t n_bonds);

int32_t gamd_forces_async(gamd_handle* h, const float* pos_dev, const uint8_t* species_dev, const float* box,
                          float* out_norm_dev, float* out_denorm_dev, void* stream);

int32_t gamd_set_node_features(gamd_handle* h, const float* feat_dev);

int32_t gamd_sync_status(gamd_handle* h, void* stream);

int32_t gamd_get_device_flags(gamd_handle* h, int32_t flags[4]);

int32_t gamd_forces(gamd_handle* h, const float* pos_dev, const uint8_t* species_dev, const float* box,
                    float* out_norm_dev, float* out_denorm_dev, void* stream);

int32_t gamd_forces_host(gamd_handle* h, const float* pos_host, const uint8_t* species_dev, const float* box, float* out_host,
                         int32_t denormalize, void* stream);

int32_t gamd_forces_edges(gamd_handle* h, const float* pos_dev, const uint8_t* species_dev, const float* box,
                          const int32_t* centre_dev, const int32_t* neigh_dev, int64_t n_edges,
                          float* out_norm_dev, float* out_denorm_dev, void* stream);

int32_t gamd_build_neighbors(gamd_handle* h, const float* pos_dev, const uint8_t* species_dev, const float* box,
                             void* stream);

int32_t gamd_get_counts(gamd_handle* h, int64_t* n_edges, int64_t* n_pieces, int64_t* edge_capacity);

int32_t gamd_get_skin_stats(gamd_handle* h, int64_t* n_rebuilds, int64_t* n_candidates, int64_t* candidate_capacity);

enum {
    GAMD_DBG_PERM = 0,
    GAMD_DBG_ROWPTR = 1,
    GAMD_DBG_COL = 2,
    GAMD_DBG_EFRAG = 3,
    GAMD_DBG_FEAT = 4,
    GAMD_DBG_CYCLES = 5,
    GAMD_DBG_PARTIAL = 6,
    GAMD_DBG_H0 = 16
};
int32_t gamd_debug_get(gamd_handle* h, int32_t what, void* host_out, size_t bytes);

typedef struct gamd_md_params {
    float dt_ps;
    float mass_amu;
    float temperature_k;
    float gamma_per_ps;
    uint64_t seed;
    uint64_t first_step;
    float mass_h_amu;
    float length_per_nm;
    int32_t rigid_water;
    float r_oh, r_hh;
    int32_t remove_cm_motion;
} gamd_md_params;
int32_t gamd_md_run(gamd_handle* h, float* x_dev, float* v_dev, float* f_dev, const uint8_t* species_dev,
                    const float* box, const gamd_md_params* p, int64_t n_steps, void* stream);

typedef struct gamd_nhc_params {
    float dt_ps;
    float mass_amu;
    float temperature_k;
    float frequency_per_ps;
    int32_t chain_length;
    int32_t num_mts;
    int32_t num_yoshidasuzuki;
    int32_t reset;
    double ndf;
    float mass_h_amu;
    float length_per_nm;
    int32_t rigid_water;
    float r_oh, r_hh;
    int32_t remove_cm_motion;
} gamd_nhc_params;
int32_t gamd_md_run_nhc(gamd_handle* h, float* x_dev, float* v_dev, float* f_dev, const uint8_t* species_dev,
                        const float* box, const gamd_nhc_params* p, double* chain_state_dev, int64_t n_steps, void* stream);

typedef struct gamd_report_params {
    int64_t interval;
    int64_t max_samples;
    double ndf;
    int32_t rdf_bins;
    float rdf_rmax;
    int32_t exclude_same_molecule;
    int32_t reserved;
} gamd_report_params;
int32_t gamd_report_configure(gamd_handle* h, const gamd_report_params* p);
int32_t gamd_report_reset(gamd_handle* h);
int32_t gamd_report_read(gamd_handle* h, void* stream, int64_t* steps, double* ke, double* temperature, int64_t max_rows,
                         int64_t* n_rows, uint64_t* counts, int64_t count_elems, int64_t* frames, int64_t* dropped,
                         int32_t dims[3]);

enum { GAMD_TRAJ_X = 1, GAMD_TRAJ_V = 2, GAMD_TRAJ_F = 4, GAMD_TRAJ_IMAGE = 8 };
typedef struct gamd_traj_params {
    int64_t interval;
    int64_t max_frames;
    int32_t fields;
    int32_t n_lags;
    int32_t subtract_com;
    int32_t reserved;
} gamd_traj_params;
int32_t gamd_traj_configure(gamd_handle* h, const gamd_traj_params* p);
int32_t gamd_traj_reset(gamd_handle* h);
int32_t gamd_traj_read_frames(gamd_handle* h, void* stream, int64_t first, int64_t count, int64_t* steps,
                              float* x, float* v, float* f, int32_t* image, int64_t* n_frames, int64_t* dropped);
int32_t gamd_traj_read_dynamics(gamd_handle* h, void* stream, double* msd_sum, double* vacf_sum, int64_t elems,
                                int64_t* n_samples, uint64_t* ambiguous, int64_t* class_atoms, int32_t dims[3]);

typedef struct gamd_struct_params {
    int64_t interval;
    int32_t rdf_bins;
    float rdf_rmax;
    int32_t exclude_same_molecule;
    int32_t sk_n2max;
    int32_t reserved[2];
} gamd_struct_params;
int32_t gamd_struct_configure(gamd_handle* h, const gamd_struct_params* p);
int32_t gamd_struct_reset(gamd_handle* h);
int32_t gamd_struct_read(gamd_handle* h, void* stream, uint64_t* counts, int64_t count_elems, double* sk_sum, int64_t sk_elems,
                         int32_t* kvec, int64_t kvec_elems, int64_t* frames, int32_t dims[4]);

int32_t gamd_profile(gamd_handle* h, const float* pos_dev, const uint8_t* species_dev, const float* box,
                     float* out_norm_dev, void* stream, char* names, size_t names_bytes, float* ms, int32_t max_ms,
                     int32_t* n_out);

int32_t gamd_timing_enable(gamd_handle* h, int32_t enable);
int32_t gamd_timing_read(gamd_handle* h, void* stream, double* total_ms, int64_t* n_launches);
int32_t gamd_timing_read_stages(gamd_handle* h, void* stream, double total_ms[3], int64_t n_launches[3]);
int32_t gamd_timing_read_steps(gamd_handle* h, void* stream, float* step_ms, int64_t max_steps, int64_t* n_steps);

#ifdef __cplusplus
}
#endif
#endif
```

Before: 3.356 million atom-steps/s.

## Fold integrator halves and skin check into last node kernel; skip gated layer-0 launch

Moves the BAOAB second half, the next step's first half and the skin displacement check into the epilogue of the final node/decode kernel, so the next step's neighbor path can skip its separate skin-check kernel (check_done) and the integrator launches disappear. Next-step counters are zeroed inside the binning and cell kernels. Separately, the layer-0 node launch is skipped entirely when it would be gated off and the cached layer-0 tables are valid. This trades fewer kernel launches and passes over positions for extra register and argument pressure in k_node and more complex frozen-state handling.

```diff
diff --git a/gamd_amd/csrc/gamd_api.hip b/gamd_amd/csrc/gamd_api.hip
--- a/gamd_amd/csrc/gamd_api.hip
+++ b/gamd_amd/csrc/gamd_api.hip
@@ -303,7 +303,8 @@
 
 int enqueue_forward(gamd_handle* h, const float* pos_dev, const uint8_t* species_dev, float* out_norm_dev,
                     float* out_denorm_dev, hipStream_t st, hipEvent_t* evs, int* n_ev, std::vector<std::string>* labels,
-                    const EdgeList* el = nullptr, const MdFuse* fuse = nullptr, bool copy_counters = true, bool l0_reuse = false) {
+                    const EdgeList* el = nullptr, const MdFuse* fuse = nullptr, bool copy_counters = true, bool l0_reuse = false,
+                    NodeMdFuse* node_fuse = nullptr, bool check_done = false) {
     auto mark = [&](const char* label) {
         if (evs) { (void)hipEventRecord(evs[*n_ev], st); ++*n_ev; labels->push_back(label); }
     };
@@ -329,7 +330,15 @@
         na.force_rebuild = h->cand_valid ? 0 : 1;
         ++h->skin_calls;
         na.cells_one_wg = (h->skin_calls < 32 || 6ll * h->sticky_host[STICKY_REBUILDS] < h->skin_calls) ? 1 : 0;
-        if (fuse && !pingpong) return fail(-1, "internal: integrator halves can only be fused into the skin path");
+        if ((fuse || node_fuse || check_done) && !pingpong) return fail(-1, "internal: integrator halves can only be fused into the skin path");
+        na.check_done = check_done ? 1 : 0;
+        if (node_fuse) {
+            node_fuse->nbr = na;
+            node_fuse->nbr.counters = counters_next;
+            node_fuse->nbr.counters_next = nullptr;
+            node_fuse->nbr.force_rebuild = 0;
+            node_fuse->nbr.check_done = 0;
+        }
         if ((r = launch_neighbor_skin(na, st, fuse))) return fail(-1, "neighbor (skin) launch failed (%d)", r);
         h->cand_valid = true;
     } else if ((r = launch_neighbor_build(na, st))) return fail(-1, "neighbor build launch failed (%d)", r);
@@ -402,7 +411,9 @@
 
     const size_t nh = (size_t)h->n * (size_t)h->H;
     auto node = [&](const NodeArgs& na_) {
-        return h->DT > 1 ? launch_node_wide_d(na_, h->HT, h->DT, st) : h->wide_conv ? launch_node_wide(na_, h->HT, st) : launch_node(na_, st);
+        if (na_.md_fuse && (h->DT > 1 || h->wide_conv)) return -22;
+        return h->DT > 1 ? launch_node_wide_d(na_, h->HT, h->DT, st) : h->wide_conv ? launch_node_wide(na_, h->HT, st)
+                                                                                   : launch_node(na_, st, na_.md_fuse ? node_fuse : nullptr);
     };
     auto hptr = [&](int l) { return h->hbuf.as<float>() + (h->cfg.keep_stages ? (size_t)l * nh : (size_t)(l & 1) * nh); };
 
@@ -442,7 +453,12 @@
     no.h_out = h0;
     if (l0) { no.hn_out = h->l0_hn.as<float>(); no.S_out = h->l0_S.as<float>(); no.D_out = h->l0_D.as<float>(); no.P_out = h->l0_P.as<float>(); }
     no.l0_gate = (l0 && l0_reuse) ? 1 : 0;
-    if ((r = node(no))) return fail(-1, "node(0) launch failed (%d)", r);
+    const bool l0_skip = no.l0_gate && h->node_emb && h->l0_tables_ok && !h->cfg.keep_stages &&
+                         !(h->cfg.kernel_select & GAMD_KSEL_NO_L0_SKIP);
+    if (!l0_skip) {
+        if ((r = node(no))) return fail(-1, "node(0) launch failed (%d)", r);
+        if (l0 && !no.l0_gate) h->l0_tables_ok = true;
+    }
     no.l0_gate = 0;
     no.hn_out = h->hn.as<float>(); no.S_out = h->S.as<float>(); no.D_out = h->D.as<float>(); no.P_out = h->P.as<float>();
     mark("node_first");
@@ -504,6 +520,7 @@
         no.h_in = l == 0 ? h0 : hptr(l);
         no.P_in = (l0 && l == 0) ? h->l0_P.as<float>() : h->P.as<float>();
         no.h_out = hptr(l + 1);
+        no.md_fuse = (node_fuse && no.mode == 2) ? 1 : 0;
         if ((r = node(no))) return fail(-1, "node launch failed (%d)", r);
         mark(no.mode == 2 ? "node_last_decode" : "node_mid");
     }
@@ -559,12 +576,15 @@
     MdPending& p = h->pending;
     int r;
     if (p.kind == 0 && h->skin > 0.f) {
+        const bool fold_ok = !(h->cfg.kernel_select & GAMD_KSEL_NO_NODE_MD_FUSE) && !small_path(h) && h->n > 1024 && !p.m.use_rigid &&
+                             !p.m.com.enabled && !h->wide_conv && h->DT == 1 && !h->node_f16;
+        bool folded_prev = false;
         for (long long s = s_begin; s < p.n_steps; ++s) {
             if ((r = step_event(h, p.st))) return r;
             p.m.step = p.first_step + (unsigned long long)s;
             p.m.step_index = (int)s;
-            int do_second = (s > s_begin && !observers_sampled(h, s - 1)) ? 1 : 0;
-            const int do_first = (skip_first && s == s_begin) ? 0 : 1;
+            int do_second = (s > s_begin && !observers_sampled(h, s - 1) && !folded_prev) ? 1 : 0;
+            const int do_first = ((skip_first && s == s_begin) || folded_prev) ? 0 : 1;
             if (p.m.com.enabled) {
                 if (do_second && do_first) {
                     MdArgs prev = p.m;
@@ -584,9 +604,19 @@
                 }
             }
             const MdFuse fuse{&p.m, do_second, do_first};
-            if ((r = enqueue_forward(h, p.x, p.species, nullptr, p.f, p.st, nullptr, nullptr, nullptr, nullptr, &fuse,
-                                     s + 1 == p.n_steps, s > s_begin)))
+            const bool fold = fold_ok && !observers_sampled(h, s);
+            NodeMdFuse nf{};
+            if (fold) {
+                nf.do_first = s + 1 < p.n_steps ? 1 : 0;
+                nf.frozen_at = 2 * (int)s + 1;
+                nf.md = p.m;
+                nf.md.step = p.m.step + 1;
+                nf.md.step_index = (int)s + 1;
+            }
+            if ((r = enqueue_forward(h, p.x, p.species, nullptr, p.f, p.st, nullptr, nullptr, nullptr, nullptr, folded_prev ? nullptr : &fuse,
+                                     s + 1 == p.n_steps, s > s_begin, fold ? &nf : nullptr, folded_prev)))
                 return r;
+            folded_prev = fold;
             if (s + 1 < p.n_steps && observers_sampled(h, s)) {
                 if ((r = launch_baoab_second(p.m, p.st))) return fail(-1, "integrator launch failed (%d)", r);
                 if ((r = observers_enqueue(h, s))) return r;
@@ -594,7 +624,7 @@
         }
         if (p.n_steps > s_begin) {
             p.m.step_index = (int)(p.n_steps - 1);
-            if ((r = launch_baoab_second(p.m, p.st))) return fail(-1, "integrator launch failed (%d)", r);
+            if (!folded_prev && (r = launch_baoab_second(p.m, p.st))) return fail(-1, "integrator launch failed (%d)", r);
             if ((r = observers_enqueue(h, p.n_steps - 1))) return r;
         }
         return step_event(h, p.st, true);
@@ -669,7 +699,8 @@
         return fail(-22, "unknown self_loop_mode %d", cfg->self_loop_mode);
     if (cfg->self_loop_mode != GAMD_SELF_LOOP_DGL07_NOOP && cfg->edge_dtype != GAMD_EDGE_F32)
         return fail(-22, "self_loop_mode 1 is built for the fp32 edge dtype only");
-    if (cfg->kernel_select & ~(GAMD_KSEL_FORCE_GENERIC_WIDTH | GAMD_KSEL_FORCE_HALF_QUANTUM | GAMD_KSEL_NO_LAYER0_HOIST))
+    if (cfg->kernel_select & ~(GAMD_KSEL_FORCE_GENERIC_WIDTH | GAMD_KSEL_FORCE_HALF_QUANTUM | GAMD_KSEL_NO_LAYER0_HOIST |
+                               GAMD_KSEL_NO_L0_SKIP | GAMD_KSEL_NO_NODE_MD_FUSE))
         return fail(-22, "unknown kernel_select bits 0x%x", cfg->kernel_select);
     int ndev = 0;
     if (hipGetDeviceCount(&ndev) != hipSuccess || ndev <= 0)
@@ -694,6 +725,9 @@
     gamd_handle* h = new gamd_handle();
     h->obs = observers_new();
     h->cfg = *cfg;
+#ifdef GAMD_KSEL_OR
+    h->cfg.kernel_select |= GAMD_KSEL_OR;
+#endif
     h->dev = cfg->device;
     if (hipStreamCreateWithFlags(&h->init_stream, hipStreamNonBlocking) != hipSuccess) {
         h->init_stream = nullptr;
@@ -831,6 +865,7 @@
     t.data.assign(data, data + cnt);
     h->host_w[name] = std::move(t);
     h->finalized = false;
+    h->l0_tables_ok = false;
     return 0;
 }
 
@@ -839,6 +874,7 @@
     DeviceGuard guard(h->dev);
     InitStream init(h->init_stream);
     const int F = h->n_feat, L = h->L;
+    h->l0_tables_ok = false;
     const int64_t H = h->H, Eh = h->Eh, HT = h->HT, EHT = h->EHT;
     const int64_t Ht = h->H_true, Et = h->Eh_true, Dt = h->D_true;
     const int64_t Dp = h->Dp, DT = h->DT;
diff --git a/gamd_amd/csrc/gamd_host.h b/gamd_amd/csrc/gamd_host.h
--- a/gamd_amd/csrc/gamd_host.h
+++ b/gamd_amd/csrc/gamd_host.h
@@ -139,6 +139,7 @@
     DevBuf pos_w, pos_s, cell_of, perm, inv_perm, deg, row_ptr, na_excl, bond_nbr;
     DevBuf hbuf, hn, S, D, P, f_norm, f_den;
     DevBuf l0_h, l0_hn, l0_S, l0_D, l0_P;
+    bool l0_tables_ok = false;
     DevBuf cell_cnt, cell_fill, cell_start;
     int ncell_cap = 0;
     long long e_cap = 0;
diff --git a/gamd_amd/csrc/gamd_internal.h b/gamd_amd/csrc/gamd_internal.h
--- a/gamd_amd/csrc/gamd_internal.h
+++ b/gamd_amd/csrc/gamd_internal.h
@@ -129,6 +129,7 @@
     unsigned* chunk_mask;
     int* counters;
     int* counters_next;
+    int check_done;
     int* sticky;
     const int* gate;
     float skin_half2;
@@ -283,8 +284,8 @@
     float* forces_norm;
     float* forces;
     long long* tdbg;
-};
-int launch_node(const NodeArgs& a, hipStream_t st);
+    int md_fuse;
+};
 int launch_node_wide(const NodeArgs& a, int ht, hipStream_t st);
 int launch_node_wide_d(const NodeArgs& a, int ht, int dt, hipStream_t st);
 
@@ -312,6 +313,13 @@
     int step_index;
     MdCom com;
 };
+struct NodeMdFuse {
+    int do_first;
+    int frozen_at;
+    MdArgs md;
+    NbrArgs nbr;
+};
+int launch_node(const NodeArgs& a, hipStream_t st, const NodeMdFuse* mf = nullptr);
 int launch_baoab_first(const MdArgs& a, hipStream_t st);
 int launch_baoab_second(const MdArgs& a, hipStream_t st);
 int launch_baoab_second_com(const MdArgs& a, hipStream_t st);
diff --git a/gamd_amd/csrc/gamd_md_dev.h b/gamd_amd/csrc/gamd_md_dev.h
--- a/gamd_amd/csrc/gamd_md_dev.h
+++ b/gamd_amd/csrc/gamd_md_dev.h
@@ -204,3 +204,52 @@
 }
 
 #pragma clang fp contract(fast)
+
+__device__ __forceinline__ float node_feature(const NbrArgs& a, int v) {
+    return a.feat ? a.feat[v] : (a.species ? (float)a.species[v] : 0.f);
+}
+
+__device__ __forceinline__ int box_id(const NbrArgs& a, int i) { return a.bx.n_boxes > 1 ? gamd_box_of(a.bx, i) : 0; }
+__device__ __forceinline__ BoxDims box_dims(const NbrArgs& a, int b) {
+    if (a.bx.n_boxes <= 1) {
+        float bx = a.box[0], by = a.box[1], bz = a.box[2], hx = a.half[0], hy = a.half[1], hz = a.half[2];
+        asm volatile("" : "+r"(bx), "+r"(by), "+r"(bz), "+r"(hx), "+r"(hy), "+r"(hz));
+        return BoxDims{bx, by, bz, hx, hy, hz};
+    }
+    const float4 B = a.bx.boxes[3 * b], H = a.bx.boxes[3 * b + 1];
+    return BoxDims{B.x, B.y, B.z, H.x, H.y, H.z};
+}
+__device__ __forceinline__ bool d_moved_beyond(const float4& p, const float4& r, const BoxDims& B, float skin_half2) {
+#pragma clang fp contract(off)
+    const float dx = gamd_min_image_wrapped(p.x - r.x, B.bx, B.hx);
+    const float dy = gamd_min_image_wrapped(p.y - r.y, B.by, B.hy);
+    const float dz = gamd_min_image_wrapped(p.z - r.z, B.bz, B.hz);
+    return !(((dx * dx + dy * dy) + dz * dz) <= skin_half2);
+}
+
+__device__ __forceinline__ bool d_skin_check(const NbrArgs& a, int i) {
+    const BoxDims B = box_dims(a, box_id(a, i));
+    float4 p;
+    p.x = gamd_remainder(a.pos[3 * i + 0], B.bx);
+    p.y = gamd_remainder(a.pos[3 * i + 1], B.by);
+    p.z = gamd_remainder(a.pos[3 * i + 2], B.bz);
+    p.w = 0.f;
+    a.pos_w[i] = p;
+    bool moved = a.force_rebuild != 0;
+    if (!moved) {
+        moved = d_moved_beyond(p, a.ref_pos[i], B, a.skin_half2);
+    }
+    p.w = node_feature(a, i);
+    a.pos_s[a.inv_perm[i]] = p;
+    return moved;
+}
+
+
+__device__ __forceinline__ void d_node_md_atom(const NodeMdFuse& m, int i) {
+#pragma unroll
+    for (int d = 0; d < 3; ++d) d_baoab_second_dof(m.md, 3 * i + d);
+    if (m.do_first) {
+        d_baoab_first_atom(m.md, i);
+        if (d_skin_check(m.nbr, i)) m.nbr.counters[CNT_REBUILD] = 1;
+    }
+}
diff --git a/gamd_amd/csrc/neighbor.hip b/gamd_amd/csrc/neighbor.hip
--- a/gamd_amd/csrc/neighbor.hip
+++ b/gamd_amd/csrc/neighbor.hip
@@ -10,21 +10,8 @@
 }
 
 #define GAMD_GATE() do { if (a.gate && *a.gate == 0) return; } while (0)
-
-__device__ __forceinline__ float node_feature(const NbrArgs& a, int v) {
-    return a.feat ? a.feat[v] : (a.species ? (float)a.species[v] : 0.f);
-}
-
-__device__ __forceinline__ int box_id(const NbrArgs& a, int i) { return a.bx.n_boxes > 1 ? gamd_box_of(a.bx, i) : 0; }
-__device__ __forceinline__ BoxDims box_dims(const NbrArgs& a, int b) {
-    if (a.bx.n_boxes <= 1) {
-        float bx = a.box[0], by = a.box[1], bz = a.box[2], hx = a.half[0], hy = a.half[1], hz = a.half[2];
-        asm volatile("" : "+r"(bx), "+r"(by), "+r"(bz), "+r"(hx), "+r"(hy), "+r"(hz));
-        return BoxDims{bx, by, bz, hx, hy, hz};
-    }
-    const float4 B = a.bx.boxes[3 * b], H = a.bx.boxes[3 * b + 1];
-    return BoxDims{B.x, B.y, B.z, H.x, H.y, H.z};
-}
+#define GAMD_ZERO_NEXT(A) do { if ((A).check_done && blockIdx.x == 0 && threadIdx.x < CNT_COUNT) (A).counters_next[threadIdx.x] = 0; } while (0)
+
 struct BoxCells { int nx, ny, nz, base; };
 __device__ __forceinline__ BoxCells box_cells(const NbrArgs& a, int b) {
     if (a.bx.n_boxes <= 1) {
@@ -54,6 +41,7 @@
 }
 
 __global__ void k_bin(NbrArgs a) {
+    GAMD_ZERO_NEXT(a);
     GAMD_GATE();
     const int i = blockIdx.x * blockDim.x + threadIdx.x;
     if (i < a.n) d_bin(a, i);
@@ -592,31 +580,6 @@
     d_sort_gather_batch(c, tid >> 6, tid & 63, 0, c.ncell);
 }
 
-__device__ __forceinline__ bool d_moved_beyond(const float4& p, const float4& r, const BoxDims& B, float skin_half2) {
-#pragma clang fp contract(off)
-    const float dx = gamd_min_image_wrapped(p.x - r.x, B.bx, B.hx);
-    const float dy = gamd_min_image_wrapped(p.y - r.y, B.by, B.hy);
-    const float dz = gamd_min_image_wrapped(p.z - r.z, B.bz, B.hz);
-    return !(((dx * dx + dy * dy) + dz * dz) <= skin_half2);
-}
-
-__device__ __forceinline__ bool d_skin_check(const NbrArgs& a, int i) {
-    const BoxDims B = box_dims(a, box_id(a, i));
-    float4 p;
-    p.x = gamd_remainder(a.pos[3 * i + 0], B.bx);
-    p.y = gamd_remainder(a.pos[3 * i + 1], B.by);
-    p.z = gamd_remainder(a.pos[3 * i + 2], B.bz);
-    p.w = 0.f;
-    a.pos_w[i] = p;
-    bool moved = a.force_rebuild != 0;
-    if (!moved) {
-        moved = d_moved_beyond(p, a.ref_pos[i], B, a.skin_half2);
-    }
-    p.w = node_feature(a, i);
-    a.pos_s[a.inv_perm[i]] = p;
-    return moved;
-}
-
 __device__ __forceinline__ bool d_skin_check_mol(const NbrArgs& a, int i0) {
     float px[3][3];
     float4 r[3];
@@ -680,6 +643,7 @@
 }
 
 __global__ void __launch_bounds__(1024) k_cells_one_wg(NbrArgs a) {
+    GAMD_ZERO_NEXT(a);
     if (a.counters[CNT_REBUILD] == 0) return;
     d_cells_one_wg(cand_args(a));
 }
@@ -702,6 +666,7 @@
 }
 
 __global__ void __launch_bounds__(1024) k_cells_sliced(NbrArgs a0) {
+    GAMD_ZERO_NEXT(a0);
     if (a0.counters[CNT_REBUILD] == 0) return;
     __shared__ int s_cnt[CELLS_SL_MAXCELL];
     __shared__ int s_start[CELLS_SL_MAXCELL + 1];
@@ -1204,7 +1169,9 @@
         return 0;
     }
     if (!a.counters_next) { e = hipMemsetAsync(a.counters, 0, sizeof(int) * CNT_COUNT, st); if (e) return (int)e; }
-    {
+    if (a.check_done) {
+        if (!a.counters_next || fuse) return -22;
+    } else {
         MdArgs md{};
         if (fuse) md = *fuse->md;
         hipLaunchKernelGGL(k_skin_check, dim3(gb), dim3(tb), 0, st, a, md, fuse ? fuse->do_second : 0, fuse ? fuse->do_first : 0);
diff --git a/gamd_amd/csrc/node.hip b/gamd_amd/csrc/node.hip
--- a/gamd_amd/csrc/node.hip
+++ b/gamd_amd/csrc/node.hip
@@ -1,5 +1,6 @@
 #include "gamd_common.h"
 #include "gamd_internal.h"
+#include "gamd_md_dev.h"
 
 namespace {
 
@@ -117,12 +118,17 @@
 }
 
 template <bool F16>
-__global__ void __launch_bounds__(256, 3) k_node(NodeArgs a) {
+__global__ void __launch_bounds__(256, 3) k_node(NodeArgs a, NodeMdFuse mf) {
     __shared__ __attribute__((aligned(16))) float xbuf[NT * XLD];
     __shared__ float obuf[4][NT][3];
     __shared__ float red[2][4][NT];
 
-    if (a.counters[CNT_OVERFLOW] || a.devflags[DEVFLAG_FROZEN]) return;
+    if (a.counters[CNT_OVERFLOW] || a.devflags[DEVFLAG_FROZEN]) {
+        if constexpr (!F16)
+            if (a.md_fuse && blockIdx.x == 0 && threadIdx.x == 0 && mf.md.devflags[DEVFLAG_FROZEN_AT] < 0)
+                mf.md.devflags[DEVFLAG_FROZEN_AT] = mf.frozen_at;
+        return;
+    }
     if (a.mode == 0 && a.l0_gate && a.counters[CNT_REBUILD] == 0) return;
 
     const int lane = threadIdx.x & 63, la = lane & 15, g = lane >> 4;
@@ -331,6 +337,8 @@
                 if (a.forces) a.forces[3 * (size_t)orig + c] = v * a.scale + a.shift;
                 if (!(fabsf(v) <= 3.0e38f)) a.sticky[STICKY_NONFINITE] = 1;
             }
+            if constexpr (!F16)
+                if (a.md_fuse) d_node_md_atom(mf, orig);
         }
     }
 }
@@ -341,10 +349,12 @@
 
 }
 
-int launch_node(const NodeArgs& a, hipStream_t st) {
+int launch_node(const NodeArgs& a, hipStream_t st, const NodeMdFuse* mf) {
     const int nb = (a.n + NT - 1) / NT;
-    if (a.f16x3) hipLaunchKernelGGL((k_node<true>), dim3(nb), dim3(256), 0, st, a);
-    else hipLaunchKernelGGL((k_node<false>), dim3(nb), dim3(256), 0, st, a);
+    if (a.md_fuse && (!mf || a.f16x3 || a.mode != 2 || a.forces != mf->md.f)) return -22;
+    static const NodeMdFuse none{};
+    if (a.f16x3) hipLaunchKernelGGL((k_node<true>), dim3(nb), dim3(256), 0, st, a, none);
+    else hipLaunchKernelGGL((k_node<false>), dim3(nb), dim3(256), 0, st, a, mf ? *mf : none);
     GAMD_CHECK_LAUNCH();
     return 0;
 }
diff --git a/gamd_amd/engine.py b/gamd_amd/engine.py
--- a/gamd_amd/engine.py
+++ b/gamd_amd/engine.py
@@ -18,6 +18,8 @@
 SELF_LOOP = {"dgl07_noop": 0, "append_zero_feature_loops": 1}
 KSEL_FORCE_GENERIC_WIDTH = 1
 KSEL_NO_LAYER0_HOIST = 4
+KSEL_NO_L0_SKIP = 8
+KSEL_NO_NODE_MD_FUSE = 16
 
 
 def _box3(box) -> np.ndarray:
@@ -270,14 +272,7 @@
         self.edge_dtype = edge_dtype
         check(self._lib.gamd_create(C.byref(c), C.byref(self._h)), "gamd_create")
         self.keep_stages = keep_stages
-        for name, t in state_dict.items():
-            if name.endswith("num_batches_tracked"):
-                continue
-            a = np.ascontiguousarray(t.detach().cpu().numpy().astype(np.float32))
-            shape = (C.c_int64 * a.ndim)(*a.shape)
-            check(self._lib.gamd_load_weight(self._h, name.encode(), a.ctypes.data_as(C.c_void_p), shape, a.ndim),
-                  f"gamd_load_weight({name})")
-        check(self._lib.gamd_finalize_weights(self._h), "gamd_finalize_weights")
+        self.load_weights(state_dict)
         self.set_scaler(*scaler)
         if cfg.use_bond:
             if bond is None:
@@ -299,6 +294,16 @@
             self.close()
         except Exception:
             pass
+
+    def load_weights(self, state_dict: Dict[str, torch.Tensor]) -> None:
+        for name, t in state_dict.items():
+            if name.endswith("num_batches_tracked"):
+                continue
+            a = np.ascontiguousarray(t.detach().cpu().numpy().astype(np.float32))
+            shape = (C.c_int64 * a.ndim)(*a.shape)
+            check(self._lib.gamd_load_weight(self._h, name.encode(), a.ctypes.data_as(C.c_void_p), shape, a.ndim),
+                  f"gamd_load_weight({name})")
+        check(self._lib.gamd_finalize_weights(self._h), "gamd_finalize_weights")
 
     def set_scaler(self, mean, var):
         self.scaler_mean = np.asarray(mean, dtype=np.float64).reshape(-1)[:1]
diff --git a/include/gamd_hip.h b/include/gamd_hip.h
--- a/include/gamd_hip.h
+++ b/include/gamd_hip.h
@@ -38,7 +38,8 @@
     int32_t n_boxes;
 } gamd_config;
 enum { GAMD_SELF_LOOP_DGL07_NOOP = 0, GAMD_SELF_LOOP_APPEND_ZERO_FEATURE = 1 };
-enum { GAMD_KSEL_FORCE_GENERIC_WIDTH = 1, GAMD_KSEL_FORCE_HALF_QUANTUM = 2, GAMD_KSEL_NO_LAYER0_HOIST = 4 };
+enum { GAMD_KSEL_FORCE_GENERIC_WIDTH = 1, GAMD_KSEL_FORCE_HALF_QUANTUM = 2, GAMD_KSEL_NO_LAYER0_HOIST = 4,
+       GAMD_KSEL_NO_L0_SKIP = 8, GAMD_KSEL_NO_NODE_MD_FUSE = 16 };
 
 const char* gamd_version(void);
 const char* gamd_last_error(void);
```

Result: no change. 3.353 million atom-steps/s (-0.1%).
